# GestaltCogTeam/STEP

Hardware: AMD Instinct MI355X
Metric: training windows/sec on PEMS04, horizon-12 MAE parity, 1/2/4/8 MI355X (higher is better)
Workload: dtype f16 (TSFormer Q/K/weights) + bf16 (P, V, GraphWaveNet / graph-learner GEMMs) operands, f32 accumulate

## Files before the change

### include/step_hip.h

```cpp
#ifndef STEP_HIP_H
#define STEP_HIP_H

#include <stdint.h>

#ifdef __cplusplus
extern "C" {
#endif

const char* step_last_error(void);
int step_abi_version(void);

typedef struct StepGemm {
    int M, N, K, batch;
    const void* A; long sam, sak, sab; int a_bf16;
    const void* B; long sbk, sbn, sbb; int b_bf16;
    float* C; long ldc, scn, scb;
    float alpha;
    int accumulate;
    const float* bias; int relu;
    int splitk;
    int a_kblk; long a_kstride;
    int b_kblk; long b_kstride;
    int b_nblk; long b_nstride;
    int c_nblk; long c_nstride;
    const float* a_kscale; const float* a_kshift; int a_kperiod;
    int batch0; long sab1, sbb1, scb1;
    int compute_bf16;
    float* a_rowsum;
    const float *c_nscale, *c_nshift, *c_mvec;
    int c_nperiod;
    float* splitk_ws; long splitk_ws_floats;
} StepGemm;
int step_gemm(const StepGemm* g, void* stream);

#define STEP_ENC_F16 1
#define STEP_ENC_ALWAYS_RESHIFT 2
#define STEP_ENC_RANGE_FLAG 4
#define STEP_ENC_WORKGROUPS(n) (((n) & 0xffff) << 8)
int step_tsformer_encode(const float* series, int S, int L, const void* wpack, long wpack_bytes,
                         int depth, int flags, uint16_t* hidden_bf16, float* hidden_f32, float* last_f32,
                         float* sqnorm_part, float dropout_p, const uint64_t* drop_pool, long pool_words, uint64_t seed,
                         unsigned int* fallback_count, void* stream);
int step_dropout_pool_fill(uint64_t* pool, long words, float dropout_p, uint64_t seed, void* stream);
long step_tsformer_dropout_words(int L, int depth);

int step_pack_long_history(const float* x, int B, int L, int N, int C, int ch, float* out, void* stream);
int step_gather_windows(const float* data, int T, int N, int C, int ch, const long* t0, int B, int L, int H,
                        float* long_series, float* hist, float* fut, void* stream);

long step_knn_workspace_bytes(int B, int N, int F);
int step_knn_graph(const uint16_t* hidden, const float* sqnorm_part, int B, int N, int F, int k_total,
                   float* sim, float* adj, void* work, long work_bytes, void* stream);
int step_topk_mask(const float* sim, int B, int N, int k_total, float* adj, void* work, long work_bytes,
                   void* stream);

typedef struct StepDglParams {
    float *conv1_w, *conv1_b;
    float *conv2_w, *conv2_b;
    float *fc_w, *fc_b;
    float *bn1_w, *bn1_b, *bn1_rm, *bn1_rv;
    float *bn2_w, *bn2_b, *bn2_rm, *bn2_rv;
    float *bn3_w, *bn3_b, *bn3_rm, *bn3_rv;
    float *fc_out_w, *fc_out_b;
    float *fc_cat_w, *fc_cat_b;
    int gemm_bf16;
} StepDglParams;

long step_dgl_global_saved_floats(int N, int T);
long step_dgl_global_work_floats(int N, int T, int backward);
int step_dgl_global_forward(const float* series_nt, int N, int T, const StepDglParams* p, int training,
                            float momentum, float* saved, float* work, float* g, void* stream);
int step_dgl_global_backward(const float* series_nt, int N, int T, const StepDglParams* p, const float* saved,
                             const float* dg, float* work, const StepDglParams* grads, void* stream);
#define STEP_DGL_FRESH_FC_GRAD 16
int step_dgl_global_backward_phase(const float* series_nt, int N, int T, const StepDglParams* p, const float* saved,
                             const float* dg, float* work, const StepDglParams* grads, int phase, void* stream);

typedef struct StepDglShard { int own1; double count1, count2; } StepDglShard;
int step_dgl_global_forward_shard(const float* series_slice, int N, int Ts, const StepDglParams* p, int training, float momentum,
                                  float* saved, float* work, double* sums, float* g, const StepDglShard* shard, int phase,
                                  void* stream);
int step_dgl_global_backward_shard(const float* series_slice, int N, int Ts, const StepDglParams* p, const float* saved,
                                   const float* dg, float* work, const StepDglParams* grads, const StepDglShard* shard, int phase,
                                   void* stream);
// ... 162 lines not shown
```

### step_amd/_lib.py

```python
import ctypes
import os

import torch

_HERE = os.path.dirname(os.path.abspath(__file__))
LIB_PATH = os.environ.get("STEP_HIP_LIB") or os.path.join(_HERE, "libstep_hip.so")

_vp, _i, _l, _f, _u64 = ctypes.c_void_p, ctypes.c_int, ctypes.c_long, ctypes.c_float, ctypes.c_uint64


class StepGemm(ctypes.Structure):
    _fields_ = [("M", _i), ("N", _i), ("K", _i), ("batch", _i),
                ("A", _vp), ("sam", _l), ("sak", _l), ("sab", _l), ("a_bf16", _i),
                ("B", _vp), ("sbk", _l), ("sbn", _l), ("sbb", _l), ("b_bf16", _i),
                ("C", _vp), ("ldc", _l), ("scn", _l), ("scb", _l),
                ("alpha", _f), ("accumulate", _i), ("bias", _vp), ("relu", _i), ("splitk", _i),
                ("a_kblk", _i), ("a_kstride", _l), ("b_kblk", _i), ("b_kstride", _l),
                ("b_nblk", _i), ("b_nstride", _l), ("c_nblk", _i), ("c_nstride", _l),
                ("a_kscale", _vp), ("a_kshift", _vp), ("a_kperiod", _i),
                ("batch0", _i), ("sab1", _l), ("sbb1", _l), ("scb1", _l), ("compute_bf16", _i), ("a_rowsum", _vp), ("c_nscale", _vp), ("c_nshift", _vp), ("c_mvec", _vp),
                ("c_nperiod", _i), ("splitk_ws", _vp), ("splitk_ws_floats", _l)]


class StepDglParams(ctypes.Structure):
    NAMES = ["conv1_w", "conv1_b", "conv2_w", "conv2_b", "fc_w", "fc_b",
             "bn1_w", "bn1_b", "bn1_rm", "bn1_rv", "bn2_w", "bn2_b", "bn2_rm", "bn2_rv",
             "bn3_w", "bn3_b", "bn3_rm", "bn3_rv", "fc_out_w", "fc_out_b", "fc_cat_w", "fc_cat_b"]
    _fields_ = [(n, _vp) for n in NAMES] + [("gemm_bf16", _i)]


class StepGwnetParams(ctypes.Structure):
    _fields_ = [("nodevec1", _vp), ("nodevec2", _vp), ("start_w", _vp), ("start_b", _vp),
                ("filter_w", _vp * 8), ("filter_b", _vp * 8), ("gate_w", _vp * 8), ("gate_b", _vp * 8),
                ("skip_w", _vp * 8), ("skip_b", _vp * 8),
                ("bn_w", _vp * 8), ("bn_b", _vp * 8), ("bn_rm", _vp * 8), ("bn_rv", _vp * 8),
                ("gconv_w", _vp * 8), ("gconv_b", _vp * 8),
                ("fc_his0_w", _vp), ("fc_his0_b", _vp), ("fc_his2_w", _vp), ("fc_his2_b", _vp),
                ("end1_w", _vp), ("end1_b", _vp), ("end2_w", _vp), ("end2_b", _vp), ("gemm_bf16", _i)]


_PD = ctypes.POINTER(StepDglParams)


class StepDynState(ctypes.Structure):
    _fields_ = [("seed_xor", ctypes.c_uint64), ("adam_step", ctypes.c_int32), ("lr", _f), ("gsl_coef", _f), ("reserved", _f)]


class StepDglShard(ctypes.Structure):
    _fields_ = [("own1", ctypes.c_int), ("count1", ctypes.c_double), ("count2", ctypes.c_double)]


_PS = ctypes.POINTER(StepDglShard)
_PG = ctypes.POINTER(StepGwnetParams)

_SIGS = {
    "step_last_error": (ctypes.c_char_p, []),
    "step_abi_version": (_i, []),
    "step_gemm": (_i, [ctypes.POINTER(StepGemm), _vp]),
    "step_tsformer_encode": (_i, [_vp, _i, _i, _vp, _l, _i, _i, _vp, _vp, _vp, _vp, _f, _vp, _l, _u64, _vp, _vp]),
    "step_dropout_pool_fill": (_i, [_vp, _l, _f, _u64, _vp]),
    "step_tsformer_dropout_words": (_l, [_i, _i]),
    "step_gather_windows": (_i, [_vp, _i, _i, _i, _i, _vp, _i, _i, _i, _vp, _vp, _vp, _vp]),
    "step_pack_long_history": (_i, [_vp, _i, _i, _i, _i, _i, _vp, _vp]),
    "step_knn_workspace_bytes": (_l, [_i, _i, _i]),
    "step_knn_graph": (_i, [_vp, _vp, _i, _i, _i, _i, _vp, _vp, _vp, _l, _vp]),
    "step_topk_mask": (_i, [_vp, _i, _i, _i, _vp, _vp, _l, _vp]),
    "step_selftest_mfma": (_i, [_vp, _vp]),
    "step_streams_concurrent": (_i, [_vp, _vp, ctypes.POINTER(_i)]),
    "step_dgl_global_saved_floats": (_l, [_i, _i]),
    "step_dgl_global_work_floats": (_l, [_i, _i, _i]),
    "step_dgl_global_forward": (_i, [_vp, _i, _i, _PD, _i, _f, _vp, _vp, _vp, _vp]),
    "step_dgl_global_backward": (_i, [_vp, _i, _i, _PD, _vp, _vp, _vp, _PD, _vp]),
    "step_dgl_global_backward_phase": (_i, [_vp, _i, _i, _PD, _vp, _vp, _vp, _PD, _i, _vp]),
    "step_dgl_global_forward_shard": (_i, [_vp, _i, _i, _PD, _i, _f, _vp, _vp, _vp, _vp, _PS, _i, _vp]),
# ... 82 lines not shown

ABI_VERSION = 10
ENC_F16, ENC_ALWAYS_RESHIFT, ENC_RANGE_FLAG = 1, 2, 4
COMM_F32, COMM_F64, COMM_U8, COMM_ID_BYTES = 0, 1, 2, 128


def lib():
    global _lib
    if _lib is None:
        if not os.path.exists(LIB_PATH):
            raise RuntimeError(
                f"libstep_hip.so not found at {LIB_PATH}: build it with `python -m step_amd.build` "
                "(step_amd has no fallback path)")
        _lib = ctypes.CDLL(LIB_PATH)
        for name, (res, args) in _SIGS.items():
            fn = getattr(_lib, name)
            fn.restype = res
            fn.argtypes = args
        if _lib.step_abi_version() != ABI_VERSION:
            v = _lib.step_abi_version()
            _lib = None
            raise RuntimeError(f"libstep_hip.so has ABI version {v}, this package needs {ABI_VERSION}: rebuild with `python -m step_amd.build`")
    return _lib


def exported_symbols():
    return sorted(_SIGS)


def check(rc, what=""):
    if rc != 0:
        msg = lib().step_last_error().decode(errors="replace")
        raise RuntimeError(f"libstep_hip {what} failed (rc={rc}): {msg}")


def ptr(t):
    if t is None:
        return None
    assert t.is_cuda and t.is_contiguous(), "libstep_hip takes contiguous device tensors"
    return ctypes.c_void_p(t.data_ptr())


def stream():
    return ctypes.c_void_p(torch.cuda.current_stream().cuda_stream)


def call(name, *args):
    check(getattr(lib(), name)(*args), name)


def gemm(a, b, c, M, N, K, sam, sak, sbk, sbn, ldc, batch=1, sab=0, sbb=0, scb=0, scn=1, alpha=1.0,
         accumulate=0, bias=None, relu=False, splitk=1, a_off=0, b_off=0, c_off=0, a_k=(0, 0), b_k=(0, 0),
         b_n=(0, 0), c_n=(0, 0), a_kscale=None, a_kshift=None, a_kperiod=0, batch0=0, sab1=0, sbb1=0, scb1=0, compute_bf16=False, a_rowsum=None, c_nscale=None, c_nshift=None, c_mvec=None,
         c_nperiod=0, splitk_ws=None):
    g = StepGemm()
    g.M, g.N, g.K, g.batch = M, N, K, batch
    g.A = a.data_ptr() + a_off * a.element_size()
    g.sam, g.sak, g.sab, g.a_bf16 = sam, sak, sab, int(a.dtype == torch.bfloat16)
    g.B = b.data_ptr() + b_off * b.element_size()
    g.sbk, g.sbn, g.sbb, g.b_bf16 = sbk, sbn, sbb, int(b.dtype == torch.bfloat16)
    g.C = c.data_ptr() + c_off * 4
    g.ldc, g.scn, g.scb = ldc, scn, scb
    g.alpha, g.accumulate = alpha, accumulate
    g.bias = bias.data_ptr() if bias is not None else None
    g.relu, g.splitk = int(relu), splitk
    g.a_kblk, g.a_kstride = a_k
    g.b_kblk, g.b_kstride = b_k
    g.b_nblk, g.b_nstride = b_n
    g.c_nblk, g.c_nstride = c_n
    g.batch0, g.sab1, g.sbb1, g.scb1 = batch0, sab1, sbb1, scb1
    g.compute_bf16 = int(compute_bf16)
    g.a_rowsum = ptr(a_rowsum) if a_rowsum is not None else None
    g.c_nscale, g.c_nshift, g.c_mvec = (ptr(c_nscale) if c_nscale is not None else None, ptr(c_nshift) if c_nshift is not None else None,
                                         ptr(c_mvec) if c_mvec is not None else None)
    g.c_nperiod = c_nperiod
    if splitk_ws is not None:
        g.splitk_ws, g.splitk_ws_floats = ptr(splitk_ws), splitk_ws.numel()
    if a_kscale is not None:
        g.a_kscale, g.a_kshift, g.a_kperiod = a_kscale.data_ptr(), a_kshift.data_ptr(), a_kperiod
    check(lib().step_gemm(ctypes.byref(g), stream()), "step_gemm")
```

### step_amd/csrc/common.h

```cpp
#pragma once
#include "../../include/step_hip.h"
#include <hip/hip_runtime.h>
#include <stdint.h>
#include <stdio.h>
#include <string.h>

#define STEP_OK 0
#define STEP_ERR_ARG 1
#define STEP_ERR_HIP 2

void step_set_error(const char* fmt, ...);
int step_raise_lds_once(const void* kernel, int bytes, const char* what);

#define STEP_REQUIRE(cond, ...)                 \
    do {                                        \
        if (!(cond)) {                          \
            step_set_error(__VA_ARGS__);        \
            return STEP_ERR_ARG;                \
        }                                       \
    } while (0)

#define STEP_LAUNCH_CHECK(name)                                                   \
    do {                                                                          \
        hipError_t e_ = hipGetLastError();                                        \
// ... 26 lines not shown
    return f32_to_bf16_bits(lo) | (f32_to_bf16_bits(hi) << 16);
}
__device__ __forceinline__ float bf16_bits_to_f32(uint32_t b) { return __uint_as_float(b << 16); }

typedef __attribute__((ext_vector_type(8))) float f32x8;
__device__ __forceinline__ bf16x8 pack8(const float* v) {
    f32x8 t;
#pragma unroll
    for (int j = 0; j < 8; ++j) t[j] = v[j];
    return __builtin_convertvector(t, bf16x8);
}

__device__ __forceinline__ float wave_sum(float v) {
#pragma unroll
    for (int o = 32; o > 0; o >>= 1) v += __shfl_xor(v, o, 64);
    return v;
}
__device__ __forceinline__ float wave_max(float v) {
#pragma unroll
    for (int o = 32; o > 0; o >>= 1) v = fmaxf(v, __shfl_xor(v, o, 64));
    return v;
}

#ifndef STEP_PHILOX_MUL64
#define STEP_PHILOX_MUL64 1
#endif
__device__ __forceinline__ void philox4x32(uint32_t c0, uint32_t c1, uint32_t c2, uint32_t c3,
                                           uint32_t k0, uint32_t k1, uint32_t out[4]) {
#pragma unroll
    for (int r = 0; r < 10; ++r) {
#if STEP_PHILOX_MUL64
        const uint64_t p0 = (uint64_t)0xD2511F53u * c0, p1 = (uint64_t)0xCD9E8D57u * c2;
        const uint32_t hi0 = (uint32_t)(p0 >> 32), lo0 = (uint32_t)p0, hi1 = (uint32_t)(p1 >> 32), lo1 = (uint32_t)p1;
#else
        uint32_t hi0 = __umulhi(0xD2511F53u, c0), lo0 = 0xD2511F53u * c0;
        uint32_t hi1 = __umulhi(0xCD9E8D57u, c2), lo1 = 0xCD9E8D57u * c2;
#endif
        uint32_t n0 = hi1 ^ c1 ^ k0, n1 = lo1, n2 = hi0 ^ c3 ^ k1, n3 = lo0;
        c0 = n0; c1 = n1; c2 = n2; c3 = n3;
        k0 += 0x9E3779B9u; k1 += 0xBB67AE85u;
    }
    out[0] = c0; out[1] = c1; out[2] = c2; out[3] = c3;
}
__device__ __forceinline__ float u32_to_unit(uint32_t x) { return (float)(x >> 8) * (1.0f / 16777216.0f); }

struct GemmColAffine { float cs, csh; const float* mvec; };
__device__ __forceinline__ GemmColAffine gemm_col_affine(const StepGemm& g, int gn) {
    GemmColAffine a = {1.f, 0.f, nullptr};
    if (g.c_nscale) { const int c = gn / g.c_nperiod; a.cs = g.c_nscale[c]; a.csh = g.c_nshift[c]; a.mvec = g.c_mvec; }
    return a;
}

__device__ __forceinline__ void gemm_store_tile(const f32x16& acc, float* col, int mb, int M, long ldc, float alpha, int accumulate,
                                                float bv, int relu, GemmColAffine ca = GemmColAffine{1.f, 0.f, nullptr}) {
    float val[16];
#pragma unroll
    for (int e = 0; e < 16; ++e) {
        const int gm = mb + (e & 3) + 8 * (e >> 2);
        val[e] = alpha * acc[e] * ca.cs;
        if (ca.mvec) val[e] += ca.csh * (gm < M ? ca.mvec[gm] : 0.f);
    }
    if (accumulate == 2) {
#pragma unroll
        for (int e = 0; e < 16; ++e) {
            const int gm = mb + (e & 3) + 8 * (e >> 2);
            if (gm < M) atomicAdd(col + (long)gm * ldc, val[e]);
        }
    } else if (accumulate == 1) {
        float old[16];
#pragma unroll
        for (int e = 0; e < 16; ++e) {
            const int gm = mb + (e & 3) + 8 * (e >> 2);
            old[e] = gm < M ? col[(long)gm * ldc] : 0.f;
        }
#pragma unroll
        for (int e = 0; e < 16; ++e) {
            const int gm = mb + (e & 3) + 8 * (e >> 2);
            float v = val[e] + old[e] + bv;
            if (relu) v = fmaxf(v, 0.f);
            if (gm < M) col[(long)gm * ldc] = v;
        }
    } else {
#pragma unroll
        for (int e = 0; e < 16; ++e) {
            const int gm = mb + (e & 3) + 8 * (e >> 2);
            float v = val[e] + bv;
            if (relu) v = fmaxf(v, 0.f);
            if (gm < M) col[(long)gm * ldc] = v;
        }
    }
}
```

### step_amd/csrc/dgl.hip

```cpp
#include "common.h"
#include "step_internal.h"

namespace {

constexpr int KW = 10;
constexpr int EMB = 100;

template <int CI, int CO, int TPT>
__global__ __launch_bounds__(256) void conv_relu_fwd_kernel(const float* __restrict__ in, const float* __restrict__ w,
                                                            const float* __restrict__ b, const float* __restrict__ in_sc,
                                                            const float* __restrict__ in_sh, float* __restrict__ out,
                                                            float* __restrict__ partial, int Tin, int stat_limit) {
    __shared__ __attribute__((aligned(16))) float ws[CI * KW * CO];
    __shared__ float red[4][2 * CO];
    const int tid = threadIdx.x, n = blockIdx.y;
    const int Tout = Tin - (KW - 1);
    for (int e = tid; e < CI * KW * CO; e += 256) {
        int co = e % CO, k = (e / CO) % KW, ci = e / (CO * KW);
        ws[e] = w[(co * CI + ci) * KW + k];
    }
    __syncthreads();
    const int t0 = (blockIdx.x * 256 + tid) * TPT;
    float acc[CO][TPT];
#pragma unroll
    for (int co = 0; co < CO; ++co)
#pragma unroll
        for (int j = 0; j < TPT; ++j) acc[co][j] = b[co];
    if (t0 < Tout) {
#pragma unroll 1
        for (int ci = 0; ci < CI; ++ci) {
            const float* src = in + ((long)n * CI + ci) * Tin + t0;
            const float sc = in_sc ? in_sc[ci] : 1.f, sh = in_sh ? in_sh[ci] : 0.f;
            float x[TPT + KW - 1];
#pragma unroll
            for (int q = 0; q < TPT + KW - 1; ++q) x[q] = (t0 + q < Tin) ? src[q] * sc + sh : 0.f;
#pragma unroll
            for (int k = 0; k < KW; ++k) {
                const float* wk = ws + (ci * KW + k) * CO;
#pragma unroll
                for (int co = 0; co < CO; ++co) {
                    const float wv = wk[co];
#pragma unroll
                    for (int j = 0; j < TPT; ++j) acc[co][j] += wv * x[k + j];
                }
            }
        }
    }
    float s1[CO], s2[CO];
#pragma unroll
    for (int co = 0; co < CO; ++co) {
        s1[co] = 0.f; s2[co] = 0.f;
        float* dst = out + ((long)n * CO + co) * Tout + t0;
#pragma unroll
        for (int j = 0; j < TPT; ++j) {
            if (t0 + j < Tout) {
                float v = fmaxf(acc[co][j], 0.f);
                dst[j] = v;
                if (t0 + j < stat_limit) { s1[co] += v; s2[co] += v * v; }
            }
        }
    }
    const int lane = tid & 63, wave = tid >> 6;
#pragma unroll
    for (int co = 0; co < CO; ++co) {
        float a = wave_sum(s1[co]), q = wave_sum(s2[co]);
        if (lane == 0) { red[wave][co] = a; red[wave][CO + co] = q; }
    }
    __syncthreads();
    if (tid < 2 * CO)
        partial[((long)blockIdx.y * gridDim.x + blockIdx.x) * (2 * CO) + tid] = red[0][tid] + red[1][tid] + red[2][tid] + red[3][tid];
}

__global__ __launch_bounds__(256) void bn_finalize_kernel(const float* __restrict__ partial, int nblk, int C, double count,
                                                          const float* __restrict__ gamma, const float* __restrict__ beta,
                                                          float* __restrict__ rmean, float* __restrict__ rvar, int training,
                                                          float momentum, float* __restrict__ stat) {
    __shared__ double r1[256], r2[256];
    const int c = blockIdx.x, tid = threadIdx.x;
    double mean, var;
    if (training) {
        double a = 0.0, q = 0.0;
        for (int i = tid; i < nblk; i += 256) { a += partial[(long)i * 2 * C + c]; q += partial[(long)i * 2 * C + C + c]; }
        r1[tid] = a; r2[tid] = q;
        __syncthreads();
        for (int s = 128; s > 0; s >>= 1) {
            if (tid < s) { r1[tid] += r1[tid + s]; r2[tid] += r2[tid + s]; }
            __syncthreads();
        }
        mean = r1[0] / count;
        var = fmax(r2[0] / count - mean * mean, 0.0);
        if (tid == 0) {
            rmean[c] = (1.f - momentum) * rmean[c] + momentum * (float)mean;
            rvar[c] = (1.f - momentum) * rvar[c] + momentum * (float)(var * count / fmax(count - 1.0, 1.0));
        }
    } else {
        mean = rmean[c];
        var = rvar[c];
    }
    if (tid == 0) {
        float rstd = (float)(1.0 / sqrt(var + 1e-5));
        float sc = gamma[c] * rstd;
        stat[c] = sc;
        stat[C + c] = beta[c] - (float)mean * sc;
        stat[2 * C + c] = (float)mean;
        stat[3 * C + c] = rstd;
    }
}

__global__ __launch_bounds__(256) void bn_sums_kernel(const float* __restrict__ partial, int nblk, int C, double* __restrict__ sums) {
    __shared__ double r1[256], r2[256];
    const int c = blockIdx.x, tid = threadIdx.x;
    double a = 0.0, q = 0.0;
    for (int i = tid; i < nblk; i += 256) { a += partial[(long)i * 2 * C + c]; q += partial[(long)i * 2 * C + C + c]; }
    r1[tid] = a; r2[tid] = q;
    __syncthreads();
    for (int s = 128; s > 0; s >>= 1) {
        if (tid < s) { r1[tid] += r1[tid + s]; r2[tid] += r2[tid + s]; }
        __syncthreads();
    }
    if (tid == 0) { sums[c] = r1[0]; sums[C + c] = r2[0]; }
}
__global__ __launch_bounds__(256) void bn_sums_sliced_kernel(const float* __restrict__ partial, int nblk, int C, double* __restrict__ sums) {
    __shared__ double r1[256], r2[256];
    const int c = blockIdx.x, tid = threadIdx.x;
    const int per = (nblk + gridDim.y - 1) / gridDim.y, beg = blockIdx.y * per, end = min(nblk, beg + per);
    double a = 0.0, q = 0.0;
    for (int i = beg + tid; i < end; i += 256) { a += partial[(long)i * 2 * C + c]; q += partial[(long)i * 2 * C + C + c]; }
    r1[tid] = a; r2[tid] = q;
    __syncthreads();
    for (int s = 128; s > 0; s >>= 1) {
        if (tid < s) { r1[tid] += r1[tid + s]; r2[tid] += r2[tid + s]; }
        __syncthreads();
    }
    if (tid == 0) { unsafeAtomicAdd(sums + c, r1[0]); unsafeAtomicAdd(sums + C + c, r2[0]); }
}
__global__ void bn_finalize_sums_kernel(const double* __restrict__ sums, int C, double count, const float* __restrict__ gamma,
                                        const float* __restrict__ beta, float* __restrict__ rmean, float* __restrict__ rvar,
                                        int training, float momentum, float* __restrict__ stat) {
    const int c = threadIdx.x;
    if (c >= C) return;
    double mean, var;
    if (training) {
        mean = sums[c] / count;
        var = fmax(sums[C + c] / count - mean * mean, 0.0);
        rmean[c] = (1.f - momentum) * rmean[c] + momentum * (float)mean;
        rvar[c] = (1.f - momentum) * rvar[c] + momentum * (float)(var * count / fmax(count - 1.0, 1.0));
    } else {
        mean = rmean[c]; var = rvar[c];
    }
    const float rstd = (float)(1.0 / sqrt(var + 1e-5));
    const float sc = gamma[c] * rstd;
    stat[c] = sc; stat[C + c] = beta[c] - (float)mean * sc; stat[2 * C + c] = (float)mean; stat[3 * C + c] = rstd;
}

__global__ __launch_bounds__(256) void fc_post_bn3_kernel(float* __restrict__ gpre, const float* __restrict__ bias, int N,
                                                          const float* __restrict__ gamma, const float* __restrict__ beta,
                                                          float* __restrict__ rmean, float* __restrict__ rvar, int training,
                                                          float momentum, float* __restrict__ stat, float* __restrict__ g) {
    __shared__ double r1[256], r2[256];
    const int j = blockIdx.x, tid = threadIdx.x;
    const float bj = bias[j];
    double a = 0.0, q = 0.0;
    for (int n = tid; n < N; n += 256) {
        float v = gpre[(long)n * EMB + j] + bj;
        gpre[(long)n * EMB + j] = v;
        v = fmaxf(v, 0.f);
        a += v; q += (double)v * v;
    }
    r1[tid] = a; r2[tid] = q;
    __syncthreads();
    for (int s = 128; s > 0; s >>= 1) {
        if (tid < s) { r1[tid] += r1[tid + s]; r2[tid] += r2[tid + s]; }
        __syncthreads();
    }
    double mean, var;
    if (training) {
        mean = r1[0] / N;
        var = fmax(r2[0] / N - mean * mean, 0.0);
        if (tid == 0) {
            rmean[j] = (1.f - momentum) * rmean[j] + momentum * (float)mean;
            rvar[j] = (1.f - momentum) * rvar[j] + momentum * (float)(var * N / fmax((double)N - 1.0, 1.0));
        }
    } else {
        mean = rmean[j]; var = rvar[j];
    }
    const float rstd = (float)(1.0 / sqrt(var + 1e-5));
    if (tid == 0) { stat[2 * EMB + j] = (float)mean; stat[3 * EMB + j] = rstd; }
    const float sc = gamma[j] * rstd, sh = beta[j] - (float)mean * sc;
    for (int n = tid; n < N; n += 256) g[(long)n * EMB + j] = fmaxf(gpre[(long)n * EMB + j], 0.f) * sc + sh;
}

__global__ __launch_bounds__(256) void bn3_relu_bwd_kernel(const float* __restrict__ dg, const float* __restrict__ gpre, int N,
                                                           const float* __restrict__ gamma, const float* __restrict__ stat,
                                                           float* __restrict__ dgamma, float* __restrict__ dbeta,
                                                           float* __restrict__ dbias, float* __restrict__ dgpre,
                                                           float* __restrict__ dgpreT, float* __restrict__ colsum) {
    __shared__ double r1[256], r2[256];
    const int j = blockIdx.x, tid = threadIdx.x;
    const float mean = stat[2 * EMB + j], rstd = stat[3 * EMB + j];
    double a = 0.0, q = 0.0;
    for (int n = tid; n < N; n += 256) {
        float d = dg[(long)n * EMB + j];
        float xh = (fmaxf(gpre[(long)n * EMB + j], 0.f) - mean) * rstd;
        a += d; q += (double)d * xh;
    }
    r1[tid] = a; r2[tid] = q;
    __syncthreads();
    for (int s = 128; s > 0; s >>= 1) {
        if (tid < s) { r1[tid] += r1[tid + s]; r2[tid] += r2[tid + s]; }
        __syncthreads();
    }
    const float m1 = (float)(r1[0] / N), m2 = (float)(r2[0] / N);
    const float k = gamma[j] * rstd;
    __syncthreads();
    double sb = 0.0;
    for (int n = tid; n < N; n += 256) {
        float pre = gpre[(long)n * EMB + j];
        float xh = (fmaxf(pre, 0.f) - mean) * rstd;
        float dh = k * (dg[(long)n * EMB + j] - m1 - xh * m2);
        float v = pre > 0.f ? dh : 0.f;
        dgpre[(long)n * EMB + j] = v;
        dgpreT[(long)j * N + n] = v;
        sb += v;
    }
    if (tid == 0) { dgamma[j] += (float)r2[0]; dbeta[j] += (float)r1[0]; }
    __syncthreads();
    r1[tid] = sb;
    __syncthreads();
    for (int s = 128; s > 0; s >>= 1) {
        if (tid < s) r1[tid] += r1[tid + s];
        __syncthreads();
    }
    if (tid == 0) { dbias[j] += (float)r1[0]; colsum[j] = (float)r1[0]; }
}

template <int C>
__global__ __launch_bounds__(256) void bn_bwd_reduce_kernel(const float* __restrict__ dy, const float* __restrict__ x,
                                                            const float* __restrict__ stat, int Tlen, float* __restrict__ partial) {
    __shared__ float red[4][2];
    const int n = blockIdx.z, c = blockIdx.y, tid = threadIdx.x;
    const float mean = stat[2 * C + c], rstd = stat[3 * C + c];
    const long base = ((long)n * C + c) * Tlen;
    float a = 0.f, q = 0.f;
    for (int t = blockIdx.x * 1024 + tid; t < min(Tlen, (int)(blockIdx.x + 1) * 1024); t += 256) {
        float d = dy[base + t];
        a += d; q += d * ((x[base + t] - mean) * rstd);
    }
    a = wave_sum(a); q = wave_sum(q);
    if ((tid & 63) == 0) { red[tid >> 6][0] = a; red[tid >> 6][1] = q; }
    __syncthreads();
    if (tid < 2) {
// ... 377 lines not shown
#pragma unroll
        for (int c = 0; c < 16; ++c) { acc += v[c] * st2[16 + c]; v[c] *= st2[c]; }
        uint4* dst = wp + ((long)o * T2 + t) * 2;
        dst[0] = make_uint4(pack_bf16x2(v[0], v[1]), pack_bf16x2(v[2], v[3]), pack_bf16x2(v[4], v[5]), pack_bf16x2(v[6], v[7]));
        dst[1] = make_uint4(pack_bf16x2(v[8], v[9]), pack_bf16x2(v[10], v[11]), pack_bf16x2(v[12], v[13]), pack_bf16x2(v[14], v[15]));
    }
    acc = wave_sum(acc);
    if ((tid & 63) == 0) red[tid >> 6] = acc;
    __syncthreads();
    if (tid == 0) atomicAdd(&shiftdot[o], red[0] + red[1] + red[2] + red[3]);
}
__global__ void gpre_init_kernel(float* __restrict__ gpre, const float* __restrict__ shiftdot, long n) {
    const long i = (long)blockIdx.x * 256 + threadIdx.x;
    if (i < n) gpre[i] = shiftdot[i % EMB];
}
__global__ __launch_bounds__(256) void fc_unpermute_kernel(const float* __restrict__ graw, const float* __restrict__ fc_w,
                                                           const float* __restrict__ st2, const float* __restrict__ colsum,
                                                           float* __restrict__ dfc_w, float* __restrict__ dots_o, int T2, int overwrite) {
    __shared__ float red[4][32];
    const int o = blockIdx.y, t = blockIdx.x * 256 + threadIdx.x, tid = threadIdx.x;
    const float cso = colsum[o];
    float d[32];
#pragma unroll
    for (int i = 0; i < 32; ++i) d[i] = 0.f;
    if (t < T2) {
        const float4* src = (const float4*)(graw + ((long)o * T2 + t) * 16);
        const float4 g0 = src[0], g1 = src[1], g2 = src[2], g3 = src[3];
        const float g[16] = {g0.x, g0.y, g0.z, g0.w, g1.x, g1.y, g1.z, g1.w, g2.x, g2.y, g2.z, g2.w, g3.x, g3.y, g3.z, g3.w};
        float w[16], old[16];
#pragma unroll
        for (int c = 0; c < 16; ++c) { const long idx = ((long)o * 16 + c) * T2 + t; w[c] = fc_w[idx]; old[c] = overwrite ? 0.f : dfc_w[idx]; }
#pragma unroll
        for (int c = 0; c < 16; ++c) {
            dfc_w[((long)o * 16 + c) * T2 + t] = old[c] + st2[c] * g[c] + st2[16 + c] * cso;
            d[2 * c] = w[c] * g[c]; d[2 * c + 1] = w[c] * cso;
        }
    }
#pragma unroll
    for (int i = 0; i < 32; ++i) {
        const float v = wave_sum(d[i]);
        if ((tid & 63) == 0) red[tid >> 6][i] = v;
    }
    __syncthreads();
    if (tid < 32) atomicAdd(&dots_o[o * 32 + tid], red[0][tid] + red[1][tid] + red[2][tid] + red[3][tid]);
}
__global__ void dots_reduce_kernel(const float* __restrict__ dots_o, float* __restrict__ dots) {
    const int i = threadIdx.x;
    if (i >= 32) return;
    double a = 0.0;
    for (int o = 0; o < EMB; ++o) a += dots_o[o * 32 + i];
    dots[i] = (float)a;
}

static bool dgl_channels_last(const StepDglParams* p) {
    const char* e = getenv("STEP_DGL_F32_STORAGE");
    return p->gemm_bf16 && !(e && e[0] == '1');
}

static bool dgl_legacy_bn_backward() {
    const char* e = getenv("STEP_DGL_LEGACY_BN");
    return e && e[0] == '1';
}

extern "C" long step_dgl_global_saved_floats(int N, int T) {
    long T1 = T - 9, T2 = T - 18;
    return (long)N * 8 * T1 + (long)N * 16 * T2 + (long)N * EMB + 4 * 8 + 4 * 16 + 4 * EMB + (long)EMB * 16 * T2 + 128;
}
static long fc_splitk_ws_floats(int N, int T2) {
    const int splits = step_gemm_auto_splitk(N, EMB, 16 * T2, 1);
    return splits > 1 ? (long)splits * N * EMB + 4 : 0;
}
extern "C" long step_dgl_global_work_floats(int N, int T, int backward) {
    long T1 = T - 9, T2 = T - 18;
    long nb1 = (long)N * cdiv(T1, 1024), nb2 = (long)N * cdiv(T2, 1024);
    long part = (nb1 > nb2 ? nb1 : nb2) * 32 + 64;
    if (!backward) return part + dgl_conv2_pack_floats() + 64 + fc_splitk_ws_floats(N, (int)T2);
    return part + (long)N * 16 * T2 + (long)N * 8 * T1 + (long)EMB * 16 * T2 + 2L * N * EMB + DGL_SMALL + dgl_conv2_wgrad_scratch_floats(N, (int)T1);
}

static float* saved_wp(float* saved, int N, int T) {
    long T1 = T - 9, T2 = T - 18;
    return saved + (long)N * 8 * T1 + (long)N * 16 * T2 + (long)N * EMB + 4 * 8 + 4 * 16 + 4 * EMB;
}
static void carve_saved(float* saved, int N, int T, float** a1, float** a2, float** gpre, float** st1, float** st2, float** st3) {
    long T1 = T - 9, T2 = T - 18;
    *a1 = saved; saved += (long)N * 8 * T1;
    *a2 = saved; saved += (long)N * 16 * T2;
    *gpre = saved; saved += (long)N * EMB;
    *st1 = saved; saved += 4 * 8;
    *st2 = saved; saved += 4 * 16;
    *st3 = saved;
}

static int dgl_bn_stats(const float* partial, int nblk, int C, double count, const float* gamma, const float* beta, float* rm, float* rv,
                        int training, float momentum, float* stat, double* sums, hipStream_t st) {
    if (nblk < 8192) {
        bn_finalize_kernel<<<C, 256, 0, st>>>(partial, nblk, C, count, gamma, beta, rm, rv, training, momentum, stat);
    } else {
        if (hipMemsetAsync(sums, 0, 2 * C * sizeof(double), st) != hipSuccess) { step_set_error("memset failed"); return STEP_ERR_HIP; }
        bn_sums_sliced_kernel<<<dim3(C, 32), 256, 0, st>>>(partial, nblk, C, sums);
        bn_finalize_sums_kernel<<<1, 64, 0, st>>>(sums, C, count, gamma, beta, rm, rv, training, momentum, stat);
    }
    STEP_LAUNCH_CHECK("bn_stats");
    return STEP_OK;
}

static int dgl_global_forward_impl(const float* series_nt, int N, int T, const StepDglParams* p, int training, float momentum,
                                   float* saved, float* work, double* sums, float* g, const StepDglShard* shard, int phase,
                                   hipStream_t st) {
    const int T1 = T - 9, T2 = T - 18;
    float *a1, *a2, *gpre, *st1, *st2, *st3;
    carve_saved(saved, N, T, &a1, &a2, &gpre, &st1, &st2, &st3);
    float* partial = work;
    const bool all = phase == 0;
    const double count1 = shard ? shard->count1 : (double)N * T1, count2 = shard ? shard->count2 : (double)N * T2;
    const bool cl = dgl_channels_last(p);
    const long part_floats = ((long)N * cdiv(T1, 1024) > (long)N * cdiv(T2, 1024) ? (long)N * cdiv(T1, 1024) : (long)N * cdiv(T2, 1024)) * 32 + 64;
    double* own_sums = (double*)(work + part_floats + dgl_conv2_pack_floats());
    float* wp = saved_wp(saved, N, T);
    float* shiftdot = wp + (long)EMB * 16 * T2;
    if (all || phase == 1) {
        int nblk;
        if (cl) {
            STEP_TRY(dgl_conv1_fwd_cl(series_nt, p->conv1_w, p->conv1_b, a1, partial, N, T, shard ? shard->own1 : T1, &nblk, st));
        } else {
            dim3 grid(cdiv(T1, 256 * 4), N);
            conv_relu_fwd_kernel<1, 8, 4><<<grid, 256, 0, st>>>(series_nt, p->conv1_w, p->conv1_b, nullptr, nullptr, a1, partial, T,
                                                                shard ? shard->own1 : T1);
            STEP_LAUNCH_CHECK("conv1");
            nblk = grid.x * grid.y;
        }
        if (shard) bn_sums_kernel<<<8, 256, 0, st>>>(partial, nblk, 8, sums);
        else STEP_TRY(dgl_bn_stats(partial, nblk, 8, count1, p->bn1_w, p->bn1_b, p->bn1_rm, p->bn1_rv, training, momentum, st1, own_sums, st));
        STEP_LAUNCH_CHECK("bn1");
    }
    if (all || phase == 2) {
        if (shard) bn_finalize_sums_kernel<<<1, 64, 0, st>>>(sums, 8, count1, p->bn1_w, p->bn1_b, p->bn1_rm, p->bn1_rv, training, momentum, st1);
        int nblk;
        if (cl) {
            STEP_TRY(dgl_conv2_fwd_cl(a1, p->conv2_w, p->conv2_b, st1, st1 + 8, a2, partial, N, T1, &nblk,
                                      work + part_floats, st));
        } else if (p->gemm_bf16) {
            STEP_TRY(dgl_conv2_fwd_mfma(a1, p->conv2_w, p->conv2_b, st1, st1 + 8, a2, partial, N, T1, &nblk, st));
        } else {
            dim3 grid(cdiv(T2, 256 * 4), N);
            conv_relu_fwd_kernel<8, 16, 4><<<grid, 256, 0, st>>>(a1, p->conv2_w, p->conv2_b, st1, st1 + 8, a2, partial, T1, T2);
            STEP_LAUNCH_CHECK("conv2");
            nblk = grid.x * grid.y;
        }
        if (shard) bn_sums_kernel<<<16, 256, 0, st>>>(partial, nblk, 16, sums + 16);
        else STEP_TRY(dgl_bn_stats(partial, nblk, 16, count2, p->bn2_w, p->bn2_b, p->bn2_rm, p->bn2_rv, training, momentum, st2, own_sums, st));
        STEP_LAUNCH_CHECK("bn2");
    }
    if (all || phase == 3) {
        if (shard) bn_finalize_sums_kernel<<<1, 64, 0, st>>>(sums + 16, 16, count2, p->bn2_w, p->bn2_b, p->bn2_rm, p->bn2_rv, training, momentum, st2);
        const long K = 16L * T2;
        StepGemm gm = gemm_desc(N, EMB, (int)K, a2, K, 1, p->fc_w, 1, K, gpre, EMB);
        if (cl) {
            if (hipMemsetAsync(shiftdot, 0, 128 * sizeof(float), st) != hipSuccess) { step_set_error("memset failed"); return STEP_ERR_HIP; }
            fc_prep_kernel<<<dim3(cdiv(T2, 256), EMB), 256, 0, st>>>(p->fc_w, st2, (uint4*)wp, shiftdot, T2);
            gpre_init_kernel<<<cdiv((long)N * EMB, 256), 256, 0, st>>>(gpre, shiftdot, (long)N * EMB);
            STEP_LAUNCH_CHECK("fc_prep");
            gm.a_bf16 = 1;
            gm.B = wp; gm.b_bf16 = 1;
        } else {
            if (hipMemsetAsync(gpre, 0, (size_t)N * EMB * sizeof(float), st) != hipSuccess) { step_set_error("memset failed"); return STEP_ERR_HIP; }
            gm.a_kscale = st2; gm.a_kshift = st2 + 16; gm.a_kperiod = T2;
        }
        gm.accumulate = 2;
        gm.splitk = -1;
        gm.compute_bf16 = p->gemm_bf16;
        if (fc_splitk_ws_floats(N, T2) > 0) {
            float* ws = work + part_floats + dgl_conv2_pack_floats() + 64;
            gm.splitk_ws = (float*)(((uintptr_t)ws + 15) & ~(uintptr_t)15);
            gm.splitk_ws_floats = fc_splitk_ws_floats(N, T2) - 4;
        }
        STEP_TRY(step_gemm_launch(gm, st));
    }
    if (all || phase == 4) {
        fc_post_bn3_kernel<<<EMB, 256, 0, st>>>(gpre, p->fc_b, N, p->bn3_w, p->bn3_b, p->bn3_rm, p->bn3_rv, training, momentum, st3, g);
        STEP_LAUNCH_CHECK("fc_post_bn3");
    }
    return STEP_OK;
}

extern "C" int step_dgl_global_forward(const float* series_nt, int N, int T, const StepDglParams* p, int training,
                                       float momentum, float* saved, float* work, float* g, void* stream) {
    STEP_REQUIRE(series_nt && p && saved && work && g && N > 0 && T > 18, "dgl_global_forward: bad arguments");
    return dgl_global_forward_impl(series_nt, N, T, p, training, momentum, saved, work, nullptr, g, nullptr, 0, (hipStream_t)stream);
}

extern "C" int step_dgl_global_forward_shard(const float* series_slice, int N, int Ts, const StepDglParams* p, int training,
                                             float momentum, float* saved, float* work, double* sums, float* g,
                                             const StepDglShard* shard, int phase, void* stream) {
    STEP_REQUIRE(series_slice && p && saved && work && sums && g && shard && N > 0 && Ts > 18 && phase >= 1 && phase <= 4,
                 "dgl_global_forward_shard: bad arguments");
    STEP_REQUIRE(shard->own1 > 0 && shard->own1 <= Ts - 9 && shard->count1 > 0 && shard->count2 > 0, "dgl_global_forward_shard: bad shard");
    return dgl_global_forward_impl(series_slice, N, Ts, p, training, momentum, saved, work, sums, g, shard, phase, (hipStream_t)stream);
}

extern "C" long step_dgl_global_offset(int N, int T, int item) {
    const long T1 = T - 9, T2 = T - 18;
    if (item == 0) return 0;
    if (item == 1) return (long)N * 8 * T1;
    if (item == 2) return (long)N * 8 * T1 + (long)N * 16 * T2;
    const long nb1 = (long)N * cdiv(T1, 1024), nb2 = (long)N * cdiv(T2, 1024);
    const long coef = (nb1 > nb2 ? nb1 : nb2) * 32 + 64 + (long)N * 16 * T2 + (long)N * 8 * T1 + (long)EMB * 16 * T2 + 2L * N * EMB;
    if (item == 10) return coef + 256;
    if (item == 11) return coef + 320;
    return -1;
}

static int dgl_global_backward_impl(const float* series_nt, int N, int T, const StepDglParams* p, const float* saved, const float* dg,
                                    float* work, const StepDglParams* grads, const StepDglShard* shard, int phase, void* stream);

extern "C" int step_dgl_global_backward(const float* series_nt, int N, int T, const StepDglParams* p, const float* saved,
                                        const float* dg, float* work, const StepDglParams* grads, void* stream) {
    return step_dgl_global_backward_phase(series_nt, N, T, p, saved, dg, work, grads, 0, stream);
}

extern "C" int step_dgl_global_backward_phase(const float* series_nt, int N, int T, const StepDglParams* p, const float* saved,
                                              const float* dg, float* work, const StepDglParams* grads, int phase, void* stream) {
    STEP_REQUIRE(series_nt && p && saved && dg && work && grads && N > 0 && T > 18 && (phase & ~STEP_DGL_FRESH_FC_GRAD) >= 0 &&
                 (phase & ~STEP_DGL_FRESH_FC_GRAD) <= 2, "dgl_global_backward: bad arguments");
    return dgl_global_backward_impl(series_nt, N, T, p, saved, dg, work, grads, nullptr, phase, stream);
}

extern "C" int step_dgl_global_backward_shard(const float* series_slice, int N, int Ts, const StepDglParams* p, const float* saved,
                                              const float* dg, float* work, const StepDglParams* grads, const StepDglShard* shard,
                                              int phase, void* stream) {
    const int ph = phase & ~STEP_DGL_FRESH_FC_GRAD;
    STEP_REQUIRE(series_slice && p && saved && dg && work && grads && shard && N > 0 && Ts > 18 && (ph == 1 || ph == 3 || ph == 4),
                 "dgl_global_backward_shard: bad arguments");
    STEP_REQUIRE(p->gemm_bf16 && Ts - 18 >= 128, "dgl_global_backward_shard: needs the bf16 contraction mode and a slice of >= 128 conv2 columns");
    return dgl_global_backward_impl(series_slice, N, Ts, p, saved, dg, work, grads, shard, phase, stream);
}

static int dgl_global_backward_impl(const float* series_nt, int N, int T, const StepDglParams* p, const float* saved, const float* dg,
                                    float* work, const StepDglParams* grads, const StepDglShard* shard, int phase, void* stream) {
    const int fresh_fc = (phase & STEP_DGL_FRESH_FC_GRAD) ? 1 : 0;
    phase &= ~STEP_DGL_FRESH_FC_GRAD;
    const bool do_fc = phase == 0 || phase == 1, do_mid = phase == 0 || phase == 2 || phase == 3, do_tail = phase == 0 || phase == 2 || phase == 4;
    hipStream_t st = (hipStream_t)stream;
    const int T1 = T - 9, T2 = T - 18;
    const long K = 16L * T2;
    float *a1, *a2, *gpre, *st1, *st2, *st3;
    carve_saved((float*)saved, N, T, &a1, &a2, &gpre, &st1, &st2, &st3);
    long nb1 = (long)N * cdiv(T1, 1024), nb2 = (long)N * cdiv(T2, 1024);
    float* partial = work;
    float* d_a2 = work + (nb1 > nb2 ? nb1 : nb2) * 32 + 64;
    float* d_a1 = d_a2 + (long)N * 16 * T2;
    float* wraw = d_a1 + (long)N * 8 * T1;
    float* dgpre = wraw + (long)EMB * K;
    float* dgpreT = dgpre + (long)N * EMB;
    float* coef = dgpreT + (long)N * EMB;
    float* dots = coef + 256;
    float* graw = coef + 320;
    float* wg_scratch = coef + DGL_SMALL;
    const bool fuse2 = T2 >= 128 && (shard || !dgl_legacy_bn_backward());
    const double count1 = shard ? shard->count1 : (double)N * T1, count2 = shard ? shard->count2 : (double)N * T2;
    if (dgl_channels_last(p)) {
        const float* wp = saved_wp((float*)saved, N, T);
        float* dots_o = coef + 256 + 64 + 1344;
        float* colsum = coef + 128;
        if (do_fc) {
            bn3_relu_bwd_kernel<<<EMB, 256, 0, st>>>(dg, gpre, N, p->bn3_w, st3, grads->bn3_w, grads->bn3_b, grads->fc_b, dgpre, dgpreT, colsum);
            STEP_LAUNCH_CHECK("bn3_bwd");
            StepGemm gm = gemm_desc(EMB, (int)K, N, dgpre, 1, EMB, a2, K, 1, wraw, K);
            gm.b_bf16 = 1;
            gm.compute_bf16 = 1;
            STEP_TRY(step_gemm_launch(gm, st));
            if (hipMemsetAsync(dots_o, 0, EMB * 32 * sizeof(float), st) != hipSuccess) { step_set_error("memset failed"); return STEP_ERR_HIP; }
            fc_unpermute_kernel<<<dim3(cdiv(T2, 256), EMB), 256, 0, st>>>(wraw, p->fc_w, st2, colsum, grads->fc_w, dots_o, T2, fresh_fc);
            dots_reduce_kernel<<<1, 64, 0, st>>>(dots_o, dots);
            STEP_LAUNCH_CHECK("fc_unpermute");
        }
        if (do_mid) {
            bn2_fused_coef_kernel<<<1, 64, 0, st>>>(dots, st2, p->bn2_w, count2, grads->bn2_w, grads->bn2_b, coef);
            STEP_LAUNCH_CHECK("bn2_fused_coef");
            StepGemm gm = gemm_desc(N, (int)K, EMB, dgpre, EMB, 1, wp, K, 1, d_a2, K);
            gm.b_bf16 = 1;
            gm.compute_bf16 = 1;
            GemmFused fu = {nullptr, nullptr, a2, coef, st2, 16, T2, GEMM_FUSED_INTERLEAVED};
            STEP_TRY(step_gemm_launch_fused(gm, fu, st));
            STEP_TRY(dgl_conv2_wgrad_cl(d_a2, a1, wg_scratch, graw, N, T1, st));
        }
        if (do_tail) {
            STEP_TRY(dgl_conv2_wgrad_finish(graw, p->conv2_w, st1, p->bn1_w, p->bn1_b, count1, grads->conv2_w, grads->conv2_b, grads->bn1_w,
                                            grads->bn1_b, coef + 64, 1, st));
            STEP_TRY(dgl_conv2_dgrad_cl(d_a2, p->conv2_w, st1, d_a1, N, T1, a1, coef + 64, st1, shard ? shard->own1 : T1, wraw, st));
            STEP_TRY(dgl_conv1_wgrad_cl(d_a1, series_nt, wg_scratch, grads->conv1_w, grads->conv1_b, N, T, st));
        }
        return STEP_OK;
    }
    if (do_fc) {
        float* colsum = coef + 128;
        bn3_relu_bwd_kernel<<<EMB, 256, 0, st>>>(dg, gpre, N, p->bn3_w, st3, grads->bn3_w, grads->bn3_b, grads->fc_b, dgpre, dgpreT, colsum);
        STEP_LAUNCH_CHECK("bn3_bwd");
        {
            StepGemm gm = gemm_desc(EMB, (int)K, N, dgpre, 1, EMB, a2, K, 1, grads->fc_w, K);
            gm.accumulate = fresh_fc ? 0 : 1;
            gm.c_nscale = st2; gm.c_nshift = st2 + 16; gm.c_nperiod = T2; gm.c_mvec = colsum;
            gm.compute_bf16 = p->gemm_bf16;
            if (fuse2) {
                if (hipMemsetAsync(dots, 0, 32 * sizeof(float), st) != hipSuccess) { step_set_error("memset failed"); return STEP_ERR_HIP; }
                GemmFused fu = {p->fc_w, dots, nullptr, nullptr, nullptr, 16, T2};
                STEP_TRY(step_gemm_launch_fused(gm, fu, st));
            } else {
                STEP_TRY(step_gemm_launch(gm, st));
            }
        }
    }
    if (!do_mid && !do_tail) return STEP_OK;
    if (do_mid) {
        StepGemm gm = gemm_desc(N, (int)K, EMB, dgpreT, 1, N, p->fc_w, K, 1, d_a2, K);
        if (p->gemm_bf16 || fuse2) { gm.A = dgpre; gm.sam = EMB; gm.sak = 1; }
        gm.compute_bf16 = p->gemm_bf16;
        if (fuse2) {
            bn2_fused_coef_kernel<<<1, 64, 0, st>>>(dots, st2, p->bn2_w, count2, grads->bn2_w, grads->bn2_b, coef);
            STEP_LAUNCH_CHECK("bn2_fused_coef");
            GemmFused fu = {nullptr, nullptr, a2, coef, st2, 16, T2};
            STEP_TRY(step_gemm_launch_fused(gm, fu, st));
        } else {
            STEP_TRY(step_gemm_launch(gm, st));
        }
    }
    if (do_mid && !fuse2) {
        dim3 grid(cdiv(T2, 1024), 16, N);
        bn_bwd_reduce_kernel<16><<<grid, 256, 0, st>>>(d_a2, a2, st2, T2, partial);
        STEP_LAUNCH_CHECK("bn2_bwd_reduce");
        bn_bwd_finalize_kernel<<<16, 256, 0, st>>>(partial, (int)nb2, 16, (double)N * T2, p->bn2_w, st2, grads->bn2_w, grads->bn2_b, coef);
        STEP_LAUNCH_CHECK("bn2_bwd_finalize");
        bn_bwd_apply_kernel<16><<<grid, 256, 0, st>>>(d_a2, a2, st2, coef, T2);
        STEP_LAUNCH_CHECK("bn2_bwd_apply");
    }
    const bool fuse1 = p->gemm_bf16 && (shard || !dgl_legacy_bn_backward());
    if (fuse1) {
        if (do_mid) STEP_TRY(dgl_conv2_wgrad_xhat_mfma(d_a2, a1, st1, wg_scratch, graw, N, T1, st));
        if (!do_tail) return STEP_OK;
        STEP_TRY(dgl_conv2_wgrad_finish(graw, p->conv2_w, st1, p->bn1_w, p->bn1_b, count1, grads->conv2_w, grads->conv2_b, grads->bn1_w,
                                        grads->bn1_b, coef + 64, 0, st));
        STEP_TRY(dgl_conv2_dgrad_mfma(d_a2, p->conv2_w, d_a1, N, T1, a1, coef + 64, st1, shard ? shard->own1 : T1, st));
    } else if (p->gemm_bf16) {
        STEP_TRY(dgl_conv2_wgrad_mfma(d_a2, a1, st1, st1 + 8, wg_scratch, grads->conv2_w, grads->conv2_b, N, T1, st));
        STEP_TRY(dgl_conv2_dgrad_mfma(d_a2, p->conv2_w, d_a1, N, T1, nullptr, nullptr, nullptr, T1, st));
    } else {
        conv_bwd_weight_kernel<8, 16><<<N, 256, 0, st>>>(d_a2, a1, st1, st1 + 8, grads->conv2_w, grads->conv2_b, T1);
        STEP_LAUNCH_CHECK("conv2_bwd_weight");
        conv_bwd_data_kernel<8, 16, 4><<<dim3(cdiv(T1, 1024), N), 256, 0, st>>>(d_a2, p->conv2_w, d_a1, T1);
        STEP_LAUNCH_CHECK("conv2_bwd_data");
// ... 103 lines not shown
```

### step_amd/csrc/dgl_conv_mfma.hip

```cpp
#include "common.h"
#include "step_internal.h"

namespace {

constexpr int KW = 10, CI = 8, CO = 16, C1_ = 8;
constexpr int FW_TT = 1024;

__device__ __forceinline__ uint32_t cvt2(float a, float b) {
    uint32_t r;
    asm("v_cvt_pk_bf16_f32 %0, %1, %2" : "=v"(r) : "v"(a), "v"(b));
    return r;
}
__device__ __forceinline__ bf16x8 as_frag(uint4 v) { return __builtin_bit_cast(bf16x8, v); }

__global__ __launch_bounds__(256) void conv2_fwd_mfma_kernel(const float* __restrict__ a1, const float* __restrict__ w,
                                                             const float* __restrict__ b, const float* __restrict__ sc,
                                                             const float* __restrict__ sh, float* __restrict__ a2,
                                                             float* __restrict__ partial, int T1) {
    __shared__ uint4 xs[FW_TT + 16];
    __shared__ float red[4][2 * CO];
    const int tid = threadIdx.x, lane = tid & 63, wave = tid >> 6, n = blockIdx.y;
    const int T2 = T1 - (KW - 1), t0 = blockIdx.x * FW_TT;
    const int ln = lane & 15, q = lane >> 4;

// ... 376 lines not shown
    {
        const int tb = blockIdx.x * 1024;
        const float* xr = x + (long)n * T + tb;
        for (int i = tid; i < 1024 + 16; i += 256) xs[i] = tb + i < T ? xr[i] : 0.f;
    }
    __syncthreads();
    const int t0 = (blockIdx.x * 256 + tid) * 4;
    float s1[C1_], s2[C1_];
#pragma unroll
    for (int c = 0; c < C1_; ++c) { s1[c] = 0.f; s2[c] = 0.f; }
    if (t0 < T1) {
        float xv[16];
#pragma unroll
        for (int q4 = 0; q4 < 4; ++q4) {
            const float4 v4 = *(const float4*)(xs + 4 * tid + 4 * q4);
            xv[4 * q4] = v4.x; xv[4 * q4 + 1] = v4.y; xv[4 * q4 + 2] = v4.z; xv[4 * q4 + 3] = v4.w;
        }
        float acc[4][C1_];
#pragma unroll
        for (int j = 0; j < 4; ++j)
#pragma unroll
            for (int c = 0; c < C1_; ++c) acc[j][c] = b[c];
#pragma unroll
        for (int k = 0; k < KW; ++k)
#pragma unroll
            for (int c = 0; c < C1_; ++c) {
                const float wv = ws[k][c];
#pragma unroll
                for (int j = 0; j < 4; ++j) acc[j][c] += wv * xv[k + j];
            }
#pragma unroll
        for (int j = 0; j < 4; ++j) {
            if (t0 + j >= T1) break;
            float v[C1_];
#pragma unroll
            for (int c = 0; c < C1_; ++c) {
                v[c] = fmaxf(acc[j][c], 0.f);
                if (t0 + j < stat_limit) { s1[c] += v[c]; s2[c] += v[c] * v[c]; }
            }
            a1h[(long)n * T1 + t0 + j] = make_uint4(cvt2(v[0], v[1]), cvt2(v[2], v[3]), cvt2(v[4], v[5]), cvt2(v[6], v[7]));
        }
    }
    const int lane = tid & 63, wave = tid >> 6;
#pragma unroll
    for (int c = 0; c < C1_; ++c) {
        const float a = wave_sum(s1[c]), q = wave_sum(s2[c]);
        if (lane == 0) { red[wave][c] = a; red[wave][C1_ + c] = q; }
    }
    __syncthreads();
    if (tid < 2 * C1_)
        partial[((long)blockIdx.y * gridDim.x + blockIdx.x) * (2 * C1_) + tid] = red[0][tid] + red[1][tid] + red[2][tid] + red[3][tid];
}

__global__ void conv2_pack_kernel(const float* __restrict__ w, const float* __restrict__ b, const float* __restrict__ sc,
                                  const float* __restrict__ sh, uint4* __restrict__ pack) {
    const int lane = threadIdx.x & 63, s = threadIdx.x >> 6, ln = lane & 15, q = lane >> 4;
    float v[8];
    if (s < 3) {
        const int kk = 4 * s + q;
#pragma unroll
        for (int ci = 0; ci < CI; ++ci) v[ci] = kk < KW ? w[(ln * CI + ci) * KW + kk] * sc[ci] : 0.f;
    } else {
        const int kk = 2 * (s - 3) + (q >> 1), c0 = 8 * (q & 1);
#pragma unroll
        for (int j = 0; j < 8; ++j) v[j] = ln < CI ? w[((c0 + j) * CI + ln) * KW + kk] * sc[ln] : 0.f;
    }
    pack[s * 64 + lane] = make_uint4(cvt2(v[0], v[1]), cvt2(v[2], v[3]), cvt2(v[4], v[5]), cvt2(v[6], v[7]));
    if (threadIdx.x < CO) {
        float a = b[threadIdx.x];
        for (int ci = 0; ci < CI; ++ci) {
            float ws = 0.f;
            for (int kk = 0; kk < KW; ++kk) ws += w[(threadIdx.x * CI + ci) * KW + kk];
            a += ws * sh[ci];
        }
        ((float*)(pack + 8 * 64))[threadIdx.x] = a;
    }
}

__global__ __launch_bounds__(256) void conv2_fwd_cl_kernel(const uint4* __restrict__ a1h, const uint4* __restrict__ pack,
                                                           uint2* __restrict__ a2h, float* __restrict__ partial, int T1) {
    __shared__ uint4 xs[FW_TT + 16];
    __shared__ float red[4][2 * CO];
    const int tid = threadIdx.x, lane = tid & 63, wave = tid >> 6, n = blockIdx.y;
    const int T2 = T1 - (KW - 1), t0 = blockIdx.x * FW_TT;
    const int ln = lane & 15, q = lane >> 4;
    for (int tt = tid; tt < FW_TT + 16; tt += 256) {
        const int t = t0 + tt;
        xs[tt] = t < T1 ? a1h[(long)n * T1 + t] : make_uint4(0u, 0u, 0u, 0u);
    }
    bf16x8 wf[3];
#pragma unroll
    for (int s = 0; s < 3; ++s) wf[s] = as_frag(pack[s * 64 + lane]);
    float bias[4];
#pragma unroll
    for (int e = 0; e < 4; ++e) bias[e] = ((const float*)(pack + 8 * 64))[4 * q + e];
    __syncthreads();
    float s1[4] = {0.f, 0.f, 0.f, 0.f}, s2[4] = {0.f, 0.f, 0.f, 0.f};
    for (int tile = wave; tile < FW_TT / 16; tile += 4) {
        const int tb = tile * 16;
        if (t0 + tb >= T2) break;
        f32x4 acc = {0.f, 0.f, 0.f, 0.f};
#pragma unroll
        for (int s = 0; s < 3; ++s) acc = __builtin_amdgcn_mfma_f32_16x16x32_bf16(wf[s], as_frag(xs[tb + ln + 4 * s + q]), acc, 0, 0, 0);
        const int t = t0 + tb + ln;
        if (t < T2) {
            float v[4];
#pragma unroll
            for (int e = 0; e < 4; ++e) { v[e] = fmaxf(acc[e] + bias[e], 0.f); s1[e] += v[e]; s2[e] += v[e] * v[e]; }
            a2h[((long)n * T2 + t) * 4 + q] = make_uint2(cvt2(v[0], v[1]), cvt2(v[2], v[3]));
        }
    }
#pragma unroll
    for (int e = 0; e < 4; ++e) {
#pragma unroll
        for (int o = 1; o < 16; o <<= 1) { s1[e] += __shfl_xor(s1[e], o, 64); s2[e] += __shfl_xor(s2[e], o, 64); }
        if (ln == 0) { red[wave][4 * q + e] = s1[e]; red[wave][CO + 4 * q + e] = s2[e]; }
    }
    __syncthreads();
    if (tid < 2 * CO)
        partial[((long)blockIdx.y * gridDim.x + blockIdx.x) * (2 * CO) + tid] = red[0][tid] + red[1][tid] + red[2][tid] + red[3][tid];
}

__global__ __launch_bounds__(256) void conv2_dgrad_cl_kernel(const uint4* __restrict__ dz2h, const uint4* __restrict__ pack,
                                                             uint2* __restrict__ dz1h, int T1,
                                                             const uint2* __restrict__ a1h, const float* __restrict__ coef,
                                                             const float* __restrict__ stat, int own) {
    __shared__ uint4 zs[FW_TT + 16][2];
    const int tid = threadIdx.x, lane = tid & 63, wave = tid >> 6, n = blockIdx.y;
    const int T2 = T1 - (KW - 1), t0 = blockIdx.x * FW_TT;
// ... 249 lines not shown
    return (long)N * cdiv(T2, WG_SC * WG_PASSES) * WG_OUT;
}

int dgl_conv2_wgrad_mfma(const float* dz, const float* a1, const float* sc, const float* sh, float* scratch, float* dw, float* db, int N,
                         int T1, hipStream_t st) {
    const int T2 = T1 - (KW - 1);
    dim3 grid(cdiv(T2, WG_SC * WG_PASSES), N);
    conv2_wgrad_mfma_kernel<<<grid, 256, 0, st>>>(dz, a1, sc, sh, scratch, T1, 0);
    STEP_LAUNCH_CHECK("conv2_wgrad_mfma");
    conv_wgrad_reduce_kernel<<<dim3(cdiv(WG_OUT, 64), wgrad_slices(grid.x * grid.y)), 256, 0, st>>>(scratch, grid.x * grid.y, WG_OUT, CO * CI * KW, dw, db);
    STEP_LAUNCH_CHECK("conv2_wgrad_reduce");
    return STEP_OK;
}

int dgl_conv2_wgrad_xhat_mfma(const float* dz, const float* a1, const float* stat1, float* scratch, float* graw, int N, int T1,
                              hipStream_t st) {
    const int T2 = T1 - (KW - 1);
    dim3 grid(cdiv(T2, WG_SC * WG_PASSES), N);
    if (hipMemsetAsync(graw, 0, WG_OUT * sizeof(float), st) != hipSuccess) { step_set_error("memset failed"); return STEP_ERR_HIP; }
    conv2_wgrad_mfma_kernel<<<grid, 256, 0, st>>>(dz, a1, stat1, nullptr, scratch, T1, 1);
    STEP_LAUNCH_CHECK("conv2_wgrad_mfma(xhat)");
    conv_wgrad_reduce_kernel<<<dim3(cdiv(WG_OUT, 64), wgrad_slices(grid.x * grid.y)), 256, 0, st>>>(scratch, grid.x * grid.y, WG_OUT, CO * CI * KW, graw, graw + CO * CI * KW);
    STEP_LAUNCH_CHECK("conv2_wgrad_reduce");
    return STEP_OK;
}
int dgl_conv2_wgrad_finish(const float* graw, const float* w, const float* stat1, const float* gamma1, const float* beta1, double count,
                           float* dw, float* db, float* dgamma1, float* dbeta1, float* coef1, int raw, hipStream_t st) {
    conv2_wgrad_finish_kernel<<<1, 256, 0, st>>>(graw, w, stat1, gamma1, beta1, count, dw, db, dgamma1, dbeta1, coef1, raw);
    STEP_LAUNCH_CHECK("conv2_wgrad_finish");
    return STEP_OK;
}

int dgl_conv1_wgrad_mfma(const float* dz, const float* x, float* scratch, float* dw, float* db, int N, int T, hipStream_t st) {
    const int T1 = T - (KW - 1);
    dim3 grid(cdiv(T1, WG_SC * WG_PASSES), N);
    conv1_wgrad_mfma_kernel<<<grid, 256, 0, st>>>(dz, x, scratch, T);
    STEP_LAUNCH_CHECK("conv1_wgrad_mfma");
    conv_wgrad_reduce_kernel<<<dim3(cdiv(W1_OUT, 64), wgrad_slices(grid.x * grid.y)), 256, 0, st>>>(scratch, grid.x * grid.y, W1_OUT, C1 * KW, dw, db);
    STEP_LAUNCH_CHECK("conv1_wgrad_reduce");
    return STEP_OK;
}

int dgl_conv1_fwd_cl(const float* x, const float* w, const float* b, void* a1h, float* partial, int N, int T, int stat_limit, int* nblk,
                     hipStream_t st) {
    const int T1 = T - (KW - 1);
    dim3 grid(cdiv(T1, 1024), N);
    conv1_fwd_cl_kernel<<<grid, 256, 0, st>>>(x, w, b, (uint4*)a1h, partial, T, stat_limit);
    STEP_LAUNCH_CHECK("conv1_fwd_cl");
    *nblk = grid.x * grid.y;
    return STEP_OK;
}
long dgl_conv2_pack_floats() { return 8 * 64 * 4 + 16; }
int dgl_conv2_fwd_cl(const void* a1h, const float* w, const float* b, const float* sc, const float* sh, void* a2h, float* partial, int N,
                     int T1, int* nblk, float* pack, hipStream_t st) {
    const int T2 = T1 - (KW - 1);
    dim3 grid(cdiv(T2, FW_TT), N);
    conv2_pack_kernel<<<1, 512, 0, st>>>(w, b, sc, sh, (uint4*)pack);
    conv2_fwd_cl_kernel<<<grid, 256, 0, st>>>((const uint4*)a1h, (const uint4*)pack, (uint2*)a2h, partial, T1);
    STEP_LAUNCH_CHECK("conv2_fwd_cl");
    *nblk = grid.x * grid.y;
    return STEP_OK;
}
int dgl_conv2_dgrad_cl(const void* dz2h, const float* w, const float* sc, void* dz1h, int N, int T1, const void* a1h, const float* coef,
                       const float* stat, int own, float* pack, hipStream_t st) {
    conv2_pack_kernel<<<1, 512, 0, st>>>(w, w, sc, sc, (uint4*)pack);
    conv2_dgrad_cl_kernel<<<dim3(cdiv(T1, FW_TT), N), 256, 0, st>>>((const uint4*)dz2h, (const uint4*)pack, (uint2*)dz1h, T1, (const uint2*)a1h, coef, stat, own);
    STEP_LAUNCH_CHECK("conv2_dgrad_cl");
    return STEP_OK;
}
int dgl_conv2_wgrad_cl(const void* dz2h, const void* a1h, float* scratch, float* graw, int N, int T1, hipStream_t st) {
    const int T2 = T1 - (KW - 1);
    dim3 grid(cdiv(T2, WG_SC * WG_PASSES), N);
    if (hipMemsetAsync(graw, 0, WG_OUT * sizeof(float), st) != hipSuccess) { step_set_error("memset failed"); return STEP_ERR_HIP; }
    conv2_wgrad_cl_kernel<<<grid, 256, 0, st>>>((const uint4*)dz2h, (const uint4*)a1h, scratch, T1);
    STEP_LAUNCH_CHECK("conv2_wgrad_cl");
    conv_wgrad_reduce_kernel<<<dim3(cdiv(WG_OUT, 64), wgrad_slices(grid.x * grid.y)), 256, 0, st>>>(scratch, grid.x * grid.y, WG_OUT, CO * CI * KW, graw, graw + CO * CI * KW);
    STEP_LAUNCH_CHECK("conv2_wgrad_reduce");
    return STEP_OK;
}
int dgl_conv1_wgrad_cl(const void* dz1h, const float* x, float* scratch, float* dw, float* db, int N, int T, hipStream_t st) {
    const int T1 = T - (KW - 1);
    dim3 grid(cdiv(T1, WG_SC * WG_PASSES), N);
    conv1_wgrad_cl_kernel<<<grid, 256, 0, st>>>((const uint4*)dz1h, x, scratch, T);
    STEP_LAUNCH_CHECK("conv1_wgrad_cl");
    conv_wgrad_reduce_kernel<<<dim3(cdiv(W1_OUT, 64), wgrad_slices(grid.x * grid.y)), 256, 0, st>>>(scratch, grid.x * grid.y, W1_OUT, C1 * KW, dw, db);
    STEP_LAUNCH_CHECK("conv1_wgrad_reduce");
    return STEP_OK;
}
```

### step_amd/csrc/gemm.hip

```cpp
#include "common.h"
#include "step_internal.h"

namespace {

constexpr int BK = 32;

template <typename T>
__device__ __forceinline__ float ld_elem(const void* p, long idx) {
    if constexpr (sizeof(T) == 2) {
        return bf16_bits_to_f32(((const uint16_t*)p)[idx]);
    } else {
        return ((const float*)p)[idx];
    }
}

template <int BM, int BN, int WM, int WN, typename TA, typename TB>
__global__ __launch_bounds__(256) void gemm_f32mfma_kernel(StepGemm g) {
    constexpr int TM = BM / WM / 32;
    constexpr int TN = BN / WN / 32;
    constexpr int LDA = BM + 4;
    constexpr int LDB = BN + 4;
    __shared__ __attribute__((aligned(16))) float As[BK * LDA];
    __shared__ __attribute__((aligned(16))) float Bs[BK * LDB];

// ... 133 lines not shown
            const int e4 = tid + r * 256;
            if (b_kc) {
                const int kk = (e4 % (BK / 4)) * 4, nn = e4 / (BK / 4);
#pragma unroll
                for (int i = 0; i < 4; ++i) Bs[(kk + i) * LDB + nn] = rb[r][i];
            } else {
                const int nn = (e4 % (BN / 4)) * 4, kk = e4 / (BN / 4);
                *(float4*)&Bs[kk * LDB + nn] = make_float4(rb[r][0], rb[r][1], rb[r][2], rb[r][3]);
            }
        }
    };

    f32x16 acc[TM][TN];
#pragma unroll
    for (int i = 0; i < TM; ++i)
#pragma unroll
        for (int j = 0; j < TN; ++j)
#pragma unroll
            for (int e = 0; e < 16; ++e) acc[i][j][e] = 0.f;

    const int li = lane & 31, lk = lane >> 5;
    if (kbeg < kend) {
        load_tiles(kbeg);
        for (int k0 = kbeg; k0 < kend; k0 += BK) {
            __syncthreads();
            store_tiles();
            __syncthreads();
            if (k0 + BK < kend) load_tiles(k0 + BK);
#pragma unroll
            for (int kk = 0; kk < BK; kk += 2) {
                float a[TM], b[TN];
#pragma unroll
                for (int i = 0; i < TM; ++i) a[i] = As[(kk + lk) * LDA + wr * (TM * 32) + i * 32 + li];
#pragma unroll
                for (int j = 0; j < TN; ++j) b[j] = Bs[(kk + lk) * LDB + wc * (TN * 32) + j * 32 + li];
#pragma unroll
                for (int i = 0; i < TM; ++i)
#pragma unroll
                    for (int j = 0; j < TN; ++j)
                        acc[i][j] = __builtin_amdgcn_mfma_f32_32x32x2f32(a[i], b[j], acc[i][j], 0, 0, 0);
            }
        }
    }

    float* Cb = g.C + (long)i0 * g.scb + (long)i1 * g.scb1;
#pragma unroll
    for (int i = 0; i < TM; ++i)
#pragma unroll
        for (int j = 0; j < TN; ++j) {
            int gn = n0 + wc * (TN * 32) + j * 32 + li;
            if (gn >= g.N) continue;
            const float bv = (g.bias != nullptr) ? g.bias[gn] : 0.f;
            const long ni = g.c_nblk ? (long)(gn / g.c_nblk) * g.c_nstride + (gn % g.c_nblk) : (long)gn;
            gemm_store_tile(acc[i][j], Cb + ni * g.scn, m0 + wr * (TM * 32) + i * 32 + 4 * lk, g.M, g.ldc, g.alpha, g.accumulate, bv, g.relu, gemm_col_affine(g, gn));
        }
}

struct DirectArgs {
    int tiles_m, tiles_n;
    int a_sh, a_mask, b_sh, b_mask, bn_sh, bn_mask, cn_sh, cn_mask;
    int a_vec, b_vec;
};

template <typename TA, typename TB>
__global__ __launch_bounds__(256) void gemm_direct_kernel(StepGemm g, DirectArgs d) {
    const int lane = threadIdx.x & 63;
    const int wave = __builtin_amdgcn_readfirstlane(threadIdx.x >> 6);
    const long tile = (long)blockIdx.x * 4 + wave;
    const long per_batch = (long)d.tiles_m * d.tiles_n;
    if (tile >= per_batch * g.batch) return;
    const int zb = (int)(tile / per_batch);
    const int tr = (int)(tile % per_batch);
    const int m0 = (tr / d.tiles_n) * 32, n0 = (tr % d.tiles_n) * 32;
    const int li = lane & 31, lk = lane >> 5;
    const int i0 = g.batch0 ? zb % g.batch0 : zb, i1 = g.batch0 ? zb / g.batch0 : 0;
    const TA* Ab = (const TA*)g.A + (long)i0 * g.sab + (long)i1 * g.sab1;
    const TB* Bb = (const TB*)g.B + (long)i0 * g.sbb + (long)i1 * g.sbb1;
    const int gm = m0 + li, gn = n0 + li;
    const bool m_ok = gm < g.M, n_ok = gn < g.N;
    const int K = g.K;
    const int sak = (int)g.sak, sbk = (int)g.sbk;
    const int a_row = m_ok ? (int)((long)gm * g.sam) : 0;
    const int b_col = n_ok ? (int)((((long)(gn >> d.bn_sh)) * g.b_nstride + (gn & d.bn_mask)) * g.sbn) : 0;
    const int a_lane = a_row + 4 * lk * sak;
    const int b_lane = b_col + 4 * lk * sbk;

    auto ldA = [&](const TA* p, int off) -> float {
        if constexpr (sizeof(TA) == 2) return bf16_bits_to_f32(((const uint16_t*)p)[off]); else return p[off];
    };
    auto ldB = [&](const TB* p, int off) -> float {
        if constexpr (sizeof(TB) == 2) return bf16_bits_to_f32(((const uint16_t*)p)[off]); else return p[off];
    };
    auto load_a = [&](int k0, float (&v)[4]) {
        const TA* pu = Ab + (long)(((k0 >> d.a_sh) * (int)g.a_kstride + (k0 & d.a_mask)) * sak);
        if (sizeof(TA) == 4 && d.a_vec) {
            float4 t = *(const float4*)((const float*)pu + a_lane);
            v[0] = t.x; v[1] = t.y; v[2] = t.z; v[3] = t.w;
        } else {
#pragma unroll
            for (int j = 0; j < 4; ++j) v[j] = ldA(pu, a_lane + j * sak);
        }
    };
    auto load_b = [&](int k0, float (&v)[4]) {
        const TB* pu = Bb + (long)(((k0 >> d.b_sh) * (int)g.b_kstride + (k0 & d.b_mask)) * sbk);
        if (sizeof(TB) == 4 && d.b_vec) {
            float4 t = *(const float4*)((const float*)pu + b_lane);
            v[0] = t.x; v[1] = t.y; v[2] = t.z; v[3] = t.w;
// ... 19 lines not shown
            const int gkc = gk < K ? gk : 0;
            const long ki = (long)(gkc >> d.b_sh) * g.b_kstride + (gkc & d.b_mask);
            float x = ldB(Bb, b_col + (int)(ki * sbk));
            v[j] = gk < K ? x : 0.f;
        }
    };

    constexpr int G = 3, CH = 8 * G;
    f32x16 acc, acc2;
#pragma unroll
    for (int e = 0; e < 16; ++e) { acc[e] = 0.f; acc2[e] = 0.f; }
    const int kfull = K / CH * CH;
    if (kfull > 0) {
        float a[G][4], b[G][4], an[G][4], bn[G][4];
#pragma unroll
        for (int q = 0; q < G; ++q) { load_a(8 * q, a[q]); load_b(8 * q, b[q]); }
        for (int k0 = 0; k0 < kfull; k0 += CH) {
            const int kn = k0 + CH;
            if (kn < kfull) {
#pragma unroll
                for (int q = 0; q < G; ++q) { load_a(kn + 8 * q, an[q]); load_b(kn + 8 * q, bn[q]); }
            }
#pragma unroll
            for (int q = 0; q < G; ++q)
#pragma unroll
                for (int j = 0; j < 4; j += 2) {
                    acc = __builtin_amdgcn_mfma_f32_32x32x2f32(m_ok ? a[q][j] : 0.f, n_ok ? b[q][j] : 0.f, acc, 0, 0, 0);
                    acc2 = __builtin_amdgcn_mfma_f32_32x32x2f32(m_ok ? a[q][j + 1] : 0.f, n_ok ? b[q][j + 1] : 0.f, acc2, 0, 0, 0);
                }
            if (kn < kfull) {
#pragma unroll
                for (int q = 0; q < G; ++q)
#pragma unroll
                    for (int j = 0; j < 4; ++j) { a[q][j] = an[q][j]; b[q][j] = bn[q][j]; }
            }
        }
    }
    for (int k0 = kfull; k0 < K; k0 += 8) {
        float a[4], b[4];
        load_a_tail(k0, a); load_b_tail(k0, b);
#pragma unroll
        for (int j = 0; j < 4; j += 2) {
            acc = __builtin_amdgcn_mfma_f32_32x32x2f32(m_ok ? a[j] : 0.f, n_ok ? b[j] : 0.f, acc, 0, 0, 0);
            acc2 = __builtin_amdgcn_mfma_f32_32x32x2f32(m_ok ? a[j + 1] : 0.f, n_ok ? b[j + 1] : 0.f, acc2, 0, 0, 0);
        }
    }
#pragma unroll
    for (int e = 0; e < 16; ++e) acc[e] += acc2[e];

    float* Cb = g.C + (long)i0 * g.scb + (long)i1 * g.scb1;
    if (!n_ok) return;
    const float bv = (g.bias != nullptr) ? g.bias[gn] : 0.f;
    const long ni = (long)(gn >> d.cn_sh) * g.c_nstride + (gn & d.cn_mask);
    gemm_store_tile(acc, Cb + ni * g.scn, m0 + 4 * lk, g.M, g.ldc, g.alpha, g.accumulate, bv, g.relu, gemm_col_affine(g, gn));
}

static bool pow2(int x) { return x > 0 && (x & (x - 1)) == 0; }
static int ilog2(int x) { int s = 0; while ((1 << s) < x) ++s; return s; }

bool direct_eligible(const StepGemm& g) {
    if (g.K > 1024 || g.a_kscale) return false;
    if (g.sak == 1 || g.sbk == 1) return false;
    if ((g.a_kblk && (!pow2(g.a_kblk) || g.a_kblk < 8)) || (g.b_kblk && (!pow2(g.b_kblk) || g.b_kblk < 8))) return false;
    if ((g.b_nblk && !pow2(g.b_nblk)) || (g.c_nblk && !pow2(g.c_nblk))) return false;
    const long lim = 1L << 30;
    if ((long)g.M * (g.sam < 0 ? -g.sam : g.sam) + (long)g.K * g.sak >= lim) return false;
    if ((long)g.N * (g.sbn < 0 ? -g.sbn : g.sbn) * (g.b_nblk ? g.b_nstride / g.b_nblk + 1 : 1) + (long)g.K * g.sbk >= lim) return false;
    return true;
}

int launch_direct(const StepGemm& g, hipStream_t st) {
    DirectArgs d;
    d.tiles_m = cdiv(g.M, 32); d.tiles_n = cdiv(g.N, 32);
    auto sm = [](int blk, int& sh, int& mask) { if (blk) { sh = ilog2(blk); mask = blk - 1; } else { sh = 31; mask = 0x7fffffff; } };
    sm(g.a_kblk, d.a_sh, d.a_mask); sm(g.b_kblk, d.b_sh, d.b_mask); sm(g.b_nblk, d.bn_sh, d.bn_mask); sm(g.c_nblk, d.cn_sh, d.cn_mask);
    d.a_vec = !g.a_bf16 && g.sak == 1 && (g.sam % 4 == 0) && (g.sab % 4 == 0) && (((uintptr_t)g.A & 15) == 0) &&
              (g.a_kblk == 0 || g.a_kstride % 4 == 0) && (g.sab1 % 4 == 0);
    d.b_vec = !g.b_bf16 && g.sbk == 1 && (g.sbn % 4 == 0) && (g.sbb % 4 == 0) && (((uintptr_t)g.B & 15) == 0) &&
              (g.b_kblk == 0 || g.b_kstride % 4 == 0) && (g.b_nblk == 0 || g.b_nstride % 4 == 0) && (g.sbb1 % 4 == 0);
    const long waves = (long)d.tiles_m * d.tiles_n * g.batch;
    dim3 grid((unsigned)((waves + 3) / 4));
    if (g.a_bf16 && g.b_bf16) gemm_direct_kernel<uint16_t, uint16_t><<<grid, 256, 0, st>>>(g, d);
    else if (g.a_bf16) gemm_direct_kernel<uint16_t, float><<<grid, 256, 0, st>>>(g, d);
    else if (g.b_bf16) gemm_direct_kernel<float, uint16_t><<<grid, 256, 0, st>>>(g, d);
    else gemm_direct_kernel<float, float><<<grid, 256, 0, st>>>(g, d);
    STEP_LAUNCH_CHECK("step_gemm(direct)");
    return STEP_OK;
}

template <int BM, int BN, int WM, int WN>
int launch(const StepGemm& g, hipStream_t st) {
    dim3 grid(cdiv(g.N, BN), cdiv(g.M, BM), g.batch * g.splitk);
    if (g.a_bf16 && g.b_bf16)
        gemm_f32mfma_kernel<BM, BN, WM, WN, uint16_t, uint16_t><<<grid, 256, 0, st>>>(g);
    else if (g.a_bf16)
        gemm_f32mfma_kernel<BM, BN, WM, WN, uint16_t, float><<<grid, 256, 0, st>>>(g);
    else if (g.b_bf16)
        gemm_f32mfma_kernel<BM, BN, WM, WN, float, uint16_t><<<grid, 256, 0, st>>>(g);
    else
        gemm_f32mfma_kernel<BM, BN, WM, WN, float, float><<<grid, 256, 0, st>>>(g);
    STEP_LAUNCH_CHECK("step_gemm");
    return STEP_OK;
}

}

int step_gemm_rowsum_separate(StepGemm* g, hipStream_t st) {
    if (!g->a_rowsum) return STEP_OK;
    STEP_REQUIRE(g->sam == 1 && g->a_kblk == 0, "step_gemm: a_rowsum on the general kernels needs an m-contiguous A without k remap");
    STEP_TRY(step_colsum_launch((const float*)g->A, g->K, g->M, g->sak, g->a_rowsum, st));
    g->a_rowsum = nullptr;
    return STEP_OK;
}

int step_gemm_launch(StepGemm g, hipStream_t st) {
    STEP_REQUIRE(g.M > 0 && g.N > 0 && g.K >= 0 && g.batch > 0, "step_gemm: bad sizes M=%d N=%d K=%d batch=%d", g.M, g.N, g.K, g.batch);
    STEP_REQUIRE(g.A && g.B && g.C, "step_gemm: null operand");
    if (g.scn == 0) g.scn = 1;
    if (g.a_rowsum)
        STEP_REQUIRE(g.batch == 1 && g.alpha == 1.f && !g.a_bf16 && !g.a_kscale, "step_gemm: a_rowsum needs batch 1, alpha 1, f32 A without affine");
    if (g.c_nscale)
        STEP_REQUIRE(g.c_nshift && g.c_mvec && g.c_nperiod > 0, "step_gemm: c_nscale needs c_nshift, c_mvec and a positive c_nperiod");
    if (g.compute_bf16) return step_gemm_bf16_launch(g, st);
    {
        const int rc = step_gemm_f32_fast_launch(g, st);
        if (rc != -1) return rc;
    }
    STEP_TRY(step_gemm_rowsum_separate(&g, st));
    if (g.splitk < 0 && direct_eligible(g)) g.splitk = 1;
    if (g.splitk < 0) {
        STEP_REQUIRE(g.accumulate == 2, "step_gemm: automatic split-K needs accumulate==2");
        const int bm = (g.N <= 32 && g.M > 64) ? 128 : (g.M <= 32 && g.N > 64) ? 32 : (g.M <= 64 || g.N <= 64) ? 64 : 128;
        const int bn = (g.N <= 32 && g.M > 64) ? 32 : (g.M <= 32 && g.N > 64) ? 128 : (g.M <= 64 || g.N <= 64) ? 64 : 128;
        long tiles = (long)cdiv(g.M, bm) * cdiv(g.N, bn) * g.batch;
        long want = (768 + tiles - 1) / tiles;
        long maxs = cdiv(g.K, BK) / 2;
        g.splitk = (int)(want < 1 ? 1 : (want > maxs ? (maxs < 1 ? 1 : maxs) : want));
    }
    if (g.splitk < 1) g.splitk = 1;
    if (g.splitk == 1 && direct_eligible(g)) return launch_direct(g, st);
    if (g.splitk > 1) {
        STEP_REQUIRE(g.accumulate == 2, "step_gemm: split-K needs accumulate==2 (atomic) and a pre-zeroed/accumulating C");
    }
    STEP_REQUIRE(!(g.accumulate == 2 && (g.bias || g.relu)), "step_gemm: bias/relu epilogue not available with atomic accumulate");
    if (g.N <= 32 && g.M > 64) return launch<128, 32, 4, 1>(g, st);
    if (g.M <= 32 && g.N > 64) return launch<32, 128, 1, 4>(g, st);
    if (g.M <= 64 || g.N <= 64) return launch<64, 64, 2, 2>(g, st);
    long tiles128 = (long)cdiv(g.M, 128) * cdiv(g.N, 128) * g.batch * g.splitk;
    if (tiles128 < 256) return launch<64, 64, 2, 2>(g, st);
    return launch<128, 128, 2, 2>(g, st);
}

int step_gemm_launch_fused(StepGemm g, const GemmFused& fused, hipStream_t st) {
    STEP_REQUIRE(g.M > 0 && g.N > 0 && g.K >= 0 && g.batch == 1 && g.A && g.B && g.C, "step_gemm(fused): bad descriptor");
    STEP_REQUIRE(fused.channels > 0 && fused.period > 0 && (long)fused.channels * fused.period == g.N, "step_gemm(fused): N != channels * period");
    if (g.scn == 0) g.scn = 1;
    if (g.splitk < 1) g.splitk = 1;
    if (g.c_nscale) STEP_REQUIRE(g.c_nshift && g.c_mvec && g.c_nperiod == fused.period, "step_gemm(fused): column affine must use the same period");
    if (g.compute_bf16) return step_gemm_bf16_launch(g, st, &fused);
    const int rc = step_gemm_f32_fast_launch(g, st, &fused);
    if (rc == -1) { step_set_error("step_gemm(fused): operands do not qualify for the staged path"); return STEP_ERR_ARG; }
    return rc;
}

extern "C" int step_gemm(const StepGemm* g, void* stream) {
    STEP_REQUIRE(g != nullptr, "step_gemm: null descriptor");
    return step_gemm_launch(*g, (hipStream_t)stream);
}
```

### step_amd/csrc/gemm_bf16.hip

```cpp
#include "common.h"
#include "step_internal.h"

namespace {

constexpr int BK = 32;
constexpr int PITCH = BK * 2 + 16;

typedef __attribute__((ext_vector_type(4))) float f32x4v;
typedef __attribute__((ext_vector_type(4))) __bf16 bf16x4;

typedef __attribute__((ext_vector_type(2))) float f32x2v;
typedef __attribute__((ext_vector_type(2))) __bf16 bf16x2v;
__device__ __forceinline__ uint32_t pack2(float a, float b) {
    uint32_t r;
    asm("v_cvt_pk_bf16_f32 %0, %1, %2" : "=v"(r) : "v"(a), "v"(b));
    return r;
}
__device__ __forceinline__ uint2 pack4(float a, float b, float c, float d) { return make_uint2(pack2(a, b), pack2(c, d)); }
__device__ __forceinline__ uint2 pack4(const float (&v)[4]) { return pack4(v[0], v[1], v[2], v[3]); }
__device__ __forceinline__ uint16_t bf16_of(float x) {
    return __builtin_bit_cast(uint16_t, (__bf16)x);
}
template <typename T>
__device__ __forceinline__ float ld1(const void* p, long idx) {
// ... 132 lines not shown
            const int e4 = tid + r * 256;
            if (b_kc) {
                const int kk = (e4 % (BK / 4)) * 4, nn = e4 / (BK / 4);
                *(uint2*)(Bs + nn * PITCH + kk * 2) = pack4(rb[r]);
            } else {
                const int nn = (e4 % (BN / 4)) * 4, kk = e4 / (BN / 4);
#pragma unroll
                for (int i = 0; i < 4; ++i) *(uint16_t*)(Bs + (nn + i) * PITCH + kk * 2) = bf16_of(rb[r][i]);
            }
        }
    };

    f32x16 acc[TM][TN];
#pragma unroll
    for (int i = 0; i < TM; ++i)
#pragma unroll
        for (int j = 0; j < TN; ++j)
#pragma unroll
            for (int e = 0; e < 16; ++e) acc[i][j][e] = 0.f;

    const int r = lane & 31, h = lane >> 5;
    if (kbeg < kend) {
        load_tiles(kbeg);
        for (int k0 = kbeg; k0 < kend; k0 += BK) {
            __syncthreads();
            store_tiles();
            __syncthreads();
            if (k0 + BK < kend) load_tiles(k0 + BK);
#pragma unroll
            for (int ks = 0; ks < BK / 16; ++ks) {
                bf16x8 a[TM], b[TN];
#pragma unroll
                for (int i = 0; i < TM; ++i) a[i] = *(const bf16x8*)(As + (wr * (TM * 32) + i * 32 + r) * PITCH + ks * 32 + h * 16);
#pragma unroll
                for (int j = 0; j < TN; ++j) b[j] = *(const bf16x8*)(Bs + (wc * (TN * 32) + j * 32 + r) * PITCH + ks * 32 + h * 16);
#pragma unroll
                for (int i = 0; i < TM; ++i)
#pragma unroll
                    for (int j = 0; j < TN; ++j)
                        acc[i][j] = __builtin_amdgcn_mfma_f32_32x32x16_bf16(a[i], b[j], acc[i][j], 0, 0, 0);
            }
        }
    }

    float* Cb = g.C + (long)i0 * g.scb + (long)i1 * g.scb1;
#pragma unroll
    for (int i = 0; i < TM; ++i)
#pragma unroll
        for (int j = 0; j < TN; ++j) {
            const int gn = n0 + wc * (TN * 32) + j * 32 + r;
            if (gn >= g.N) continue;
            const float bv = (g.bias != nullptr) ? g.bias[gn] : 0.f;
            const long ni = g.c_nblk ? (long)(gn / g.c_nblk) * g.c_nstride + (gn % g.c_nblk) : (long)gn;
            gemm_store_tile(acc[i][j], Cb + ni * g.scn, m0 + wr * (TM * 32) + i * 32 + 4 * h, g.M, g.ldc, g.alpha, g.accumulate, bv, g.relu, gemm_col_affine(g, gn));
        }
}


enum { KC_F32 = 0, KC_BF16 = 1, MC_F32 = 2, MC_BF16 = 3 };
constexpr int FBK = 64;
constexpr int FPITCH = FBK * 2 + 8;
constexpr int FPITCH32 = FBK * 4 + 16;

struct FastArgs {
    const GemmKSeg* ktab;
    int ktab_per;
    int a_klog, b_klog, b_nlog;
    int xcd_swizzle;
    int wide_store;
    int m_fast;
    long split_stride;
    GemmFused fu;
};

static int wide_store_ok(const StepGemm& g, bool force = false) {
    return g.accumulate != 2 && !g.a_rowsum && g.c_nblk == 0 && g.scn == 1 && g.N % 4 == 0 && g.ldc % 4 == 0 && g.scb % 4 == 0 &&
           g.scb1 % 4 == 0 && ((uintptr_t)g.C & 15) == 0 && (force || (long)g.M * g.N * g.batch >= (4L << 20));
}

__device__ __forceinline__ long remap(int i, int lg, long stride) {
    return (long)(i >> lg) * stride + (i & ((1 << lg) - 1));
}

template <int MODE, int BR>
struct Stage {
    static constexpr int NV = MODE == KC_F32 ? BR * FBK / 4 / 256 : (MODE == KC_BF16 ? BR * FBK / 8 / 256 : (MODE == MC_F32 ? BR * FBK / 16 / 256 : (BR * FBK / 32 + 255) / 256));
    static constexpr int NR = (MODE == MC_F32 || MODE == MC_BF16) ? NV * 4 : NV;
    float f[NR][4];
};

template <int MODE, int BR>
__device__ __forceinline__ void stage_load(Stage<MODE, BR>& s, const char* base, int row0, int rows, long srow, long sk, int k0,
                                           int kend, int klog, long kstride, int rlog, long rstride, int tid) {
    if constexpr (MODE == KC_F32) {
#pragma unroll
        for (int r = 0; r < s.NV; ++r) {
            const int e = tid + r * 256;
            const int k = k0 + (e % (FBK / 4)) * 4, row = row0 + e / (FBK / 4);
            const bool ok = row < rows && k < kend;
            const long off = ok ? remap(row, rlog, rstride) * srow + remap(k, klog, kstride) : 0;
            const float4 t = *(const float4*)((const float*)base + off);
            s.f[r][0] = t.x; s.f[r][1] = t.y; s.f[r][2] = t.z; s.f[r][3] = t.w;
        }
    } else if constexpr (MODE == KC_BF16) {
#pragma unroll
        for (int r = 0; r < s.NV; ++r) {
            const int e = tid + r * 256;
            const int k = k0 + (e % (FBK / 8)) * 8, row = row0 + e / (FBK / 8);
            const bool ok = row < rows && k < kend;
            const long off = ok ? remap(row, rlog, rstride) * srow + remap(k, klog, kstride) : 0;
            const float4 t = *(const float4*)((const uint16_t*)base + off);
            s.f[r][0] = t.x; s.f[r][1] = t.y; s.f[r][2] = t.z; s.f[r][3] = t.w;
        }
    } else if constexpr (MODE == MC_BF16) {
#pragma unroll
        for (int r = 0; r < s.NV; ++r) {
            const int e = tid + r * 256;
            const int row = row0 + (e % (BR / 8)) * 8, kb = k0 + (e / (BR / 8)) * 4;
#pragma unroll
            for (int j = 0; j < 4; ++j) {
                const bool ok = row < rows && kb + j < kend && e < BR * FBK / 32;
                const long off = ok ? (long)row * srow + remap(kb + j, klog, kstride) * sk : 0;
                const float4 t = *(const float4*)((const uint16_t*)base + off);
                s.f[r * 4 + j][0] = t.x; s.f[r * 4 + j][1] = t.y; s.f[r * 4 + j][2] = t.z; s.f[r * 4 + j][3] = t.w;
            }
        }
    } else {
#pragma unroll
        for (int r = 0; r < s.NV; ++r) {
            const int e = tid + r * 256;
// ... 441 lines not shown
                        v[i] = x[i] > 0.f ? kk[j] * (v[i] - m1[j] - (x[i] - mu[j]) * m2r[j]) : 0.f;
                    }
                }
                float4 r4 = make_float4(v[0], v[1], v[2], v[3]);
                if (g.accumulate == 1) { r4.x += o4[u].x; r4.y += o4[u].y; r4.z += o4[u].z; r4.w += o4[u].w; }
                *(float4*)(Cb + off[u]) = r4;
            }
        }
        if (fu.dotw) {
            float q4[4] = {dw[0], dm[0], dw[1], dm[1]};
#pragma unroll
            for (int i = 0; i < 4; ++i) q4[i] = wave_sum(q4[i]);
            if (lane == 0) { fred[wave][0] = q4[0]; fred[wave][1] = q4[1]; fred[wave][2] = q4[2]; fred[wave][3] = q4[3]; }
            __syncthreads();
            if (tid < 4) {
                const int c = c_lo + (tid >> 1);
                if (c < C) atomicAdd(fu.dots + 2 * c + (tid & 1), fred[0][tid] + fred[1][tid] + fred[2][tid] + fred[3][tid]);
            }
        }
        return;
    }
    if constexpr (BM * (BN + 4) * 4 <= 2 * BUF)
    if (fa.wide_store) {
        constexpr int TP = BN + 4;
        static_assert(BM * TP * 4 <= 2 * BUF, "staging tile must fit in the operand buffers");
        float* tile = (float*)lds;
        __syncthreads();
#pragma unroll
        for (int i = 0; i < TM; ++i)
#pragma unroll
            for (int j = 0; j < TN; ++j) {
                const int cn = wc * (TN * 32) + j * 32 + r, gn = n0 + cn;
                const GemmColAffine ca = gemm_col_affine(g, gn < g.N ? gn : 0);
                const float bv = (g.bias != nullptr && gn < g.N) ? g.bias[gn] : 0.f;
#pragma unroll
                for (int e = 0; e < 16; ++e) {
                    const int rm = wr * (TM * 32) + i * 32 + 4 * h + (e & 3) + 8 * (e >> 2), gm = m0 + rm;
                    float v = g.alpha * acc[i][j][e] * ca.cs + bv;
                    if (ca.mvec) v += ca.csh * (gm < g.M ? ca.mvec[gm] : 0.f);
                    tile[rm * TP + cn] = v;
                }
            }
        __syncthreads();
        constexpr int PIECES = BM * BN / 4;
#pragma unroll 4
        for (int pc = tid; pc < PIECES; pc += 256) {
            const int rm = pc / (BN / 4), c4 = (pc % (BN / 4)) * 4;
            const int gm = m0 + rm, gn = n0 + c4;
            if (gm >= g.M || gn >= g.N) continue;
            float4 v = *(const float4*)(tile + rm * TP + c4);
            float4* dst = (float4*)(Cb + (long)gm * g.ldc + gn);
            if (g.accumulate == 1) { const float4 o = *dst; v.x += o.x; v.y += o.y; v.z += o.z; v.w += o.w; }
            if (g.relu) { v.x = fmaxf(v.x, 0.f); v.y = fmaxf(v.y, 0.f); v.z = fmaxf(v.z, 0.f); v.w = fmaxf(v.w, 0.f); }
            *dst = v;
        }
        return;
    }
#pragma unroll
    for (int i = 0; i < TM; ++i)
#pragma unroll
        for (int j = 0; j < TN; ++j) {
            const int gn = n0 + wc * (TN * 32) + j * 32 + r;
            const int mb = m0 + wr * (TM * 32) + i * 32 + 4 * h;
            if (gn == ones_row) gemm_store_tile(acc[i][j], g.a_rowsum, mb, g.M, 1, g.alpha, 2, 0.f, 0);
            if (gn >= g.N) continue;
            const float bv = (g.bias != nullptr) ? g.bias[gn] : 0.f;
            const long ni = g.c_nblk ? (long)(gn / g.c_nblk) * g.c_nstride + (gn % g.c_nblk) : (long)gn;
            gemm_store_tile(acc[i][j], Cb + ni * g.scn, mb, g.M, g.ldc, g.alpha, g.accumulate, bv, g.relu, gemm_col_affine(g, gn));
        }
}

static int ilog2_exact(int v) {
    for (int l = 2; l < 31; ++l) if ((1 << l) == v) return l;
    return -2;
}

static int fast_mode(const void* base, int is_bf16, long srow, long sk, long sb0, long sb1, int kblk, long kstride, int rblk,
                     long rstride, int* klog, int* rlog) {
    const int vec = is_bf16 ? 8 : 4;
    if (((uintptr_t)base & 15) || sb0 % vec || sb1 % vec) return -1;
    *klog = 30; *rlog = 30;
    if (sk == 1) {
        if (srow % vec) return -1;
        if (kblk) { *klog = ilog2_exact(kblk); if (*klog < 0 || kblk % vec || kstride % vec) return -1; }
        if (rblk) { *rlog = ilog2_exact(rblk); if (*rlog < 0) return -1; }
        return is_bf16 ? KC_BF16 : KC_F32;
    }
    if (srow == 1 && is_bf16) {
        if (sk % 8 || kblk || rblk) return -1;
        return MC_BF16;
    }
    if (srow == 1 && !is_bf16) {
        if (sk % 4) return -1;
        if (kblk) { *klog = ilog2_exact(kblk); if (*klog < 0) return -1; }
        if (rblk) { *rlog = ilog2_exact(rblk); if (*rlog < 0 || rstride % 4) return -1; }
        return MC_F32;
    }
    return -1;
}

template <int BM, int BN, int AMODE>
int launch_fast_b(const StepGemm& g, const FastArgs& fa, int bmode, dim3 grid, hipStream_t st) {
    if (bmode == KC_F32) gemm_fast_kernel<BM, BN, AMODE, KC_F32, false><<<grid, 256, 0, st>>>(g, fa);
    else if (bmode == KC_BF16) gemm_fast_kernel<BM, BN, AMODE, KC_BF16, false><<<grid, 256, 0, st>>>(g, fa);
    else if (bmode == MC_F32) gemm_fast_kernel<BM, BN, AMODE, MC_F32, false><<<grid, 256, 0, st>>>(g, fa);
    else {
        if constexpr (AMODE != KC_BF16) gemm_fast_kernel<BM, BN, AMODE, MC_BF16, false><<<grid, 256, 0, st>>>(g, fa);
        else { step_set_error("step_gemm: an n-contiguous bf16 B operand needs an f32 A operand"); return STEP_ERR_ARG; }
    }
    STEP_LAUNCH_CHECK("step_gemm(bf16 fast)");
    return STEP_OK;
}
template <int BM, int BN>
int launch_fast(const StepGemm& g, const FastArgs& fa_in, int amode, int bmode, hipStream_t st) {
    dim3 grid(cdiv(g.N + (g.a_rowsum ? 1 : 0), BN), cdiv(g.M, BM), g.batch * g.splitk);
    FastArgs fa = fa_in;
    fa.xcd_swizzle = grid.x >= 2 && (grid.y * grid.z) % 8 == 0 && (long)g.M * g.K * g.batch >= (8L << 20);
    if (amode == KC_F32) return launch_fast_b<BM, BN, KC_F32>(g, fa, bmode, grid, st);
    if (amode == KC_BF16) return launch_fast_b<BM, BN, KC_BF16>(g, fa, bmode, grid, st);
    return launch_fast_b<BM, BN, MC_F32>(g, fa, bmode, grid, st);
}
// ... 83 lines not shown
                            ((fused->flags & (GEMM_FUSED_FFN_FWD | GEMM_FUSED_MASKNZ | GEMM_FUSED_BF16OUT)) ? (g.accumulate == 0 && !fused->dotw && !fused->bnx && !g.c_nscale) :
                             (fused->flags & GEMM_FUSED_INTERLEAVED) ? (128 % fused->channels == 0 && fused->channels % 8 == 0 && g.N % 8 == 0 && g.ldc % 8 == 0 &&
                                                                       ((((uintptr_t)fused->bnx) | ((uintptr_t)g.C)) & 15) == 0 && !fused->dotw) : fused->period >= 128),
                            "step_gemm: the fused DGL epilogues need the staged path with a wide-store result (aligned dense C, period >= 128)");
    if (g.splitk < 0) {
        STEP_REQUIRE(g.accumulate == 2, "step_gemm: automatic split-K needs accumulate==2");
        g.splitk = auto_splitk(g.M, g.N, g.K, g.batch, fast);
    }
    if (g.splitk < 1) g.splitk = 1;
    if (g.splitk > 1) STEP_REQUIRE(g.accumulate == 2, "step_gemm: split-K needs accumulate==2");
    STEP_REQUIRE(!(g.accumulate == 2 && (g.bias || g.relu)), "step_gemm: bias/relu epilogue not available with atomic accumulate");
    long tiles128 = (long)cdiv(g.M, 128) * cdiv(g.N, 128) * g.batch * g.splitk;
    const bool big = g.M > 64 && g.N > 64 && tiles128 >= 512;
    static const bool use_ws = []() { const char* e = getenv("STEP_GEMM_SPLITK_WS"); return !e || atoi(e) != 0; }();
    const StepGemm orig = g;
    bool ws_reduce = false;
    if (use_ws && fast && !fused && g.splitk > 1 && g.splitk_ws && !g.c_nblk && !g.c_nscale && (((uintptr_t)g.splitk_ws) & 15) == 0 &&
        (long)g.M * g.N * g.batch * g.splitk <= g.splitk_ws_floats) {
        const long mn = (long)g.M * g.N;
        ws_reduce = true;
        fa.split_stride = mn * g.batch;
        g.C = g.splitk_ws; g.ldc = g.N; g.scn = 1; g.accumulate = 0;
        g.scb = mn; g.scb1 = (long)g.batch0 * mn;
        fa.wide_store = wide_store_ok(g, true);
    }
    auto finish = [&](int rc) -> int {
        if (rc != STEP_OK || !ws_reduce) return rc;
        const long total = (long)orig.M * orig.N * orig.batch;
        const int chunk = 16;
        dim3 grid((unsigned)((total + 255) / 256), (unsigned)cdiv(orig.splitk, chunk));
        splitk_reduce_kernel<<<grid, 256, 0, st>>>(orig.splitk_ws, orig.splitk, chunk, (long)orig.M * orig.N, orig.N, orig.batch, orig.batch0, orig.C,
                                                  orig.ldc, orig.scn ? orig.scn : 1, orig.scb, orig.scb1);
        STEP_LAUNCH_CHECK("step_gemm(split-K reduce)");
        return STEP_OK;
    };
    if (fast && fused) return big ? launch_fast_fused<128, 128>(g, fa, amode, bmode, st) : launch_fast_fused<64, 64>(g, fa, amode, bmode, st);
    static const bool hop128 = []() { const char* e = getenv("STEP_GEMM_HOP128"); return !e || atoi(e) != 0; }();
    if (hop128 && fast && !big && amode == KC_BF16 && bmode == KC_BF16 && g.M >= 2048 && g.N >= 256 && tiles128 >= 256)
        return finish(launch_fast<128, 128>(g, fa, amode, bmode, st));
    static const int tall_m = []() { const char* e = getenv("STEP_GEMM_TALL_M"); return e ? atoi(e) : 1024; }();
    if (fast && !big && bmode != MC_BF16 && g.M >= tall_m && g.N > 64) {
        const long t = (long)cdiv(g.M, 128) * cdiv(g.N, 64) * g.batch * g.splitk;
        if (t >= 256) return finish(launch_fast<128, 64>(g, fa, amode, bmode, st));
    }
    if (fast) return finish(big ? launch_fast<128, 128>(g, fa, amode, bmode, st) : launch_fast<64, 64>(g, fa, amode, bmode, st));
    STEP_TRY(step_gemm_rowsum_separate(&g, st));
    if (big) return launch_bf16<128, 128>(g, st);
    return launch_bf16<64, 64>(g, st);
}

int step_gemm_segmented_launch(StepGemm g, const GemmKSeg* ktab, int ktab_per, hipStream_t st) {
    STEP_REQUIRE(g.M > 0 && g.N > 0 && g.K > 0 && g.K % 32 == 0 && g.K / 32 <= GEMM_KSEG_MAX && ktab && g.A && g.B && g.C && g.batch >= 1,
                 "step_gemm(segmented): bad descriptor");
    STEP_REQUIRE(g.accumulate != 2 && !g.bias && !g.relu && !g.a_rowsum && !g.a_kscale && g.scn <= 1 && !g.c_nblk,
                 "step_gemm(segmented): plain store / += only");
    STEP_REQUIRE((((uintptr_t)g.A | (uintptr_t)g.B) & 15) == 0, "step_gemm(segmented): 16-byte aligned bases");
    g.scn = 1; g.splitk = 1;
    if (g.batch0 == 0) g.batch0 = g.batch;
    FastArgs fa;
    memset(&fa, 0, sizeof(fa));
    fa.ktab = ktab; fa.ktab_per = ktab_per;
    fa.a_klog = fa.b_klog = fa.b_nlog = 30;
    fa.wide_store = 0;
    const long tiles128 = (long)cdiv(g.M, 128) * cdiv(g.N, 128) * g.batch;
    if (g.M > 64 && g.N > 64 && tiles128 >= 256) {
        dim3 grid(cdiv(g.N, 128), cdiv(g.M, 128), g.batch);
        if (g.compute_bf16) gemm_fast_kernel<128, 128, KC_F32, KC_F32, false, true><<<grid, 256, 0, st>>>(g, fa);
        else { dim3 g64(cdiv(g.N, 64), cdiv(g.M, 64), g.batch); gemm_fast_kernel<64, 64, KC_F32, KC_F32, true, true><<<g64, 256, 0, st>>>(g, fa); }
    } else {
        dim3 grid(cdiv(g.N, 64), cdiv(g.M, 64), g.batch);
        if (g.compute_bf16) gemm_fast_kernel<64, 64, KC_F32, KC_F32, false, true><<<grid, 256, 0, st>>>(g, fa);
        else gemm_fast_kernel<64, 64, KC_F32, KC_F32, true, true><<<grid, 256, 0, st>>>(g, fa);
    }
    STEP_LAUNCH_CHECK("step_gemm(segmented)");
    return STEP_OK;
}

int step_gemm_f32_fast_launch(StepGemm g, hipStream_t st, const GemmFused* fused) {
    if (g.a_bf16 || g.b_bf16) return -1;
    FastArgs fa;
    memset(&fa, 0, sizeof(fa));
    if (fused) fa.fu = *fused;
    int dummy;
    const int amode = fast_mode(g.A, 0, g.sam, g.sak, g.sab, g.sab1, g.a_kblk, g.a_kstride, 0, 0, &fa.a_klog, &dummy);
    const int bmode = fast_mode(g.B, 0, g.sbn, g.sbk, g.sbb, g.sbb1, g.b_kblk, g.b_kstride, g.b_nblk, g.b_nstride, &fa.b_klog, &fa.b_nlog);
    if (amode < 0 || bmode < 0 || amode == MC_BF16 || bmode == MC_BF16 || (g.a_kscale && (amode != KC_F32 || g.a_kperiod < FBK))) return -1;
    fa.wide_store = wide_store_ok(g, fused != nullptr);
    if (fused && !(fa.wide_store && !g.bias && !g.relu && g.batch == 1 && g.splitk <= 1 && fused->period >= 128)) return -1;
    if (g.splitk < 0) {
        STEP_REQUIRE(g.accumulate == 2, "step_gemm: automatic split-K needs accumulate==2");
        long tiles = (long)cdiv(g.M, 64) * cdiv(g.N, 64) * g.batch;
        long want = (512 + tiles - 1) / tiles;
        long maxs = cdiv(g.K, FBK) / 2;
        g.splitk = (int)(want < 1 ? 1 : (want > maxs ? (maxs < 1 ? 1 : maxs) : want));
    }
    if (g.splitk < 1) g.splitk = 1;
    if (g.splitk > 1) STEP_REQUIRE(g.accumulate == 2, "step_gemm: split-K needs accumulate==2");
    STEP_REQUIRE(!(g.accumulate == 2 && (g.bias || g.relu)), "step_gemm: bias/relu epilogue not available with atomic accumulate");
    if (fused) return launch_fast_f32_fused(g, fa, amode, bmode, st);
    return launch_fast_f32(g, fa, amode, bmode, st);
}
```

### step_amd/csrc/gwnet.hip

```cpp
#include "common.h"
#include "step_internal.h"
#include <vector>

namespace {

constexpr int C = 32, CAT = 224, CS = 256, CE = 512, OUT = 12, NL = 8, HID = 96;
constexpr int TIN[NL] = {13, 12, 10, 9, 7, 6, 4, 3};
constexpr int DIL[NL] = {1, 2, 1, 2, 1, 2, 1, 2};
constexpr int TOUT[NL] = {12, 10, 9, 7, 6, 4, 3, 1};

__global__ void start_conv_kernel(const float* __restrict__ hist, int B, int N, int Cin, const float* __restrict__ w,
                                  const float* __restrict__ b, float* __restrict__ x0) {
    long idx = (long)blockIdx.x * 256 + threadIdx.x;
    long total = (long)B * N * 13 * C;
    if (idx >= total) return;
    int c = idx % C, t = (idx / C) % 13;
    long bn = idx / (C * 13);
    int n = bn % N, bb = bn / N;
    float v = b[c];
    if (t >= 1) {
        const float* src = hist + (((long)bb * 12 + (t - 1)) * N + n) * Cin;
        v += w[c * 2] * src[0] + w[c * 2 + 1] * src[1];
    }
    x0[idx] = v;
}
__global__ __launch_bounds__(256) void start_conv_bwd_kernel(const float* __restrict__ hist, int B, int N, int Cin,
                                                             const float* __restrict__ dx0, float* __restrict__ dw,
                                                             float* __restrict__ db) {
    __shared__ float red[8][96];
    const int c = threadIdx.x & 31;
    const int sub = threadIdx.x >> 5;
    long npos = (long)B * N * 13;
    float a0 = 0.f, a1 = 0.f, ab = 0.f;
    for (long p = (long)blockIdx.x * 8 + sub; p < npos; p += (long)gridDim.x * 8) {
        int t = p % 13;
        long bn = p / 13;
        int n = bn % N, bb = bn / N;
        float d = dx0[p * C + c];
        ab += d;
        if (t >= 1) {
            const float* src = hist + (((long)bb * 12 + (t - 1)) * N + n) * Cin;
            a0 += d * src[0]; a1 += d * src[1];
        }
    }
    red[sub][c] = a0; red[sub][32 + c] = a1; red[sub][64 + c] = ab;
    __syncthreads();
    if (threadIdx.x < 96) {
        float s = 0.f;
#pragma unroll
        for (int r = 0; r < 8; ++r) s += red[r][threadIdx.x];
        const int cc = threadIdx.x & 31, kind = threadIdx.x >> 5;
        if (kind == 2) atomicAdd(&db[cc], s); else atomicAdd(&dw[cc * 2 + kind], s);
    }
}

__global__ __launch_bounds__(256) void row_sums_kernel(const float* __restrict__ A, int N, float* __restrict__ rs, float* __restrict__ cs_init) {
    __shared__ float red[4];
    const long row = blockIdx.x;
    float s = 0.f;
    for (int j = threadIdx.x; j < N; j += 256) s += A[row * N + j];
    s = wave_sum(s);
    if ((threadIdx.x & 63) == 0) red[threadIdx.x >> 6] = s;
    __syncthreads();
    if (threadIdx.x == 0) { rs[row] = 1.f + red[0] + red[1] + red[2] + red[3]; cs_init[row] = 1.f; }
}
__global__ __launch_bounds__(256) void col_sums_kernel(const float* __restrict__ A, int N, float* __restrict__ cs) {
    __shared__ float red[4][64];
    const int b = blockIdx.z;
    const int j = blockIdx.x * 64 + (threadIdx.x & 63), w = threadIdx.x >> 6;
    const int per = (N + gridDim.y - 1) / gridDim.y, ibeg = blockIdx.y * per, iend = min(N, ibeg + per);
    float s = 0.f;
    if (j < N)
        for (int i = ibeg + w; i < iend; i += 4) s += A[((long)b * N + i) * N + j];
    red[w][threadIdx.x & 63] = s;
    __syncthreads();
    if (w == 0 && j < N) atomicAdd(&cs[(long)b * N + j], red[0][threadIdx.x] + red[1][threadIdx.x] + red[2][threadIdx.x] + red[3][threadIdx.x]);
}
__global__ __launch_bounds__(256) void rw_build_kernel(const float* __restrict__ A, int N, const float* __restrict__ rs,
                                                       const float* __restrict__ cs, float* __restrict__ Pf, float* __restrict__ Pb,
                                                       float* __restrict__ PfT, float* __restrict__ PbT) {
    __shared__ float tile[32][33];
    const int b = blockIdx.z, i0 = blockIdx.y * 32, j0 = blockIdx.x * 32;
    const int tx = threadIdx.x & 31, ty = threadIdx.x >> 5;
    const long base = (long)b * N * N;
    for (int r = ty; r < 32; r += 8) {
        int i = i0 + r, j = j0 + tx;
        float a = (i < N && j < N) ? A[base + (long)i * N + j] : 0.f;
        tile[r][tx] = a;
        if (i < N && j < N) {
            const float v = a + (i == j ? 1.f : 0.f);
            Pf[base + (long)i * N + j] = v / rs[(long)b * N + i];
            PbT[base + (long)i * N + j] = v / cs[(long)b * N + j];
        }
    }
    __syncthreads();
    for (int r = ty; r < 32; r += 8) {
        int j = j0 + r, i = i0 + tx;
        if (i < N && j < N) {
            const float v = tile[tx][r] + (i == j ? 1.f : 0.f);
            Pb[base + (long)j * N + i] = v / cs[(long)b * N + j];
            PfT[base + (long)j * N + i] = v / rs[(long)b * N + i];
        }
    }
}
__global__ void replicate_adp_kernel(const float* __restrict__ Pa, int N, int B, float* __restrict__ P2, float* __restrict__ PT2) {
    long idx = (long)blockIdx.x * 256 + threadIdx.x;
    if (idx >= (long)N * N) return;
    int i = idx / N, j = idx % N;
    float v = Pa[idx], vt = Pa[(long)j * N + i];
    for (int b = 0; b < B; ++b) { P2[(long)b * N * N + idx] = v; PT2[(long)b * N * N + idx] = vt; }
}
__global__ void stacks_to_bf16_kernel(const float* __restrict__ P, const float* __restrict__ PT, long rows, int N, int N8,
                                      uint16_t* __restrict__ P16, uint16_t* __restrict__ PT16) {
    long idx = (long)blockIdx.x * 256 + threadIdx.x;
    if (idx >= rows * (N8 / 2)) return;
    const long row = idx / (N8 / 2);
    const int j = (int)(idx % (N8 / 2)) * 2;
    const float* src = blockIdx.y ? PT : P;
    uint16_t* dst = blockIdx.y ? PT16 : P16;
    const float a = j < N ? src[row * N + j] : 0.f, b = j + 1 < N ? src[row * N + j + 1] : 0.f;
    typedef __attribute__((ext_vector_type(2))) float f2;
    typedef __attribute__((ext_vector_type(2))) __bf16 b2;
    f2 t = {a, b};
    *(uint32_t*)(dst + row * N8 + j) = __builtin_bit_cast(uint32_t, __builtin_convertvector(t, b2));
}
__global__ __launch_bounds__(256) void slots_to_bf16T_kernel(const float* __restrict__ cat, int slot0, int sstep, int B, int N, int T, int N8,
                                                             uint16_t* __restrict__ XT) {
    __shared__ float tile[64][33];
    const int v0 = blockIdx.x * 64, t = blockIdx.y, src = blockIdx.z / B, b = blockIdx.z % B;
    const int slot = slot0 + sstep * src;
    const int c = threadIdx.x & 31, r = threadIdx.x >> 5;
    for (int i = r; i < 64; i += 8) {
        const int v = v0 + i;
        tile[i][c] = v < N ? cat[(((long)b * N + v) * T + t) * CAT + slot * C + c] : 0.f;
    }
    __syncthreads();
    const int cc = threadIdx.x >> 3, g8 = (threadIdx.x & 7) * 8;
    if (v0 + g8 < N8) {
        float v8[8];
#pragma unroll
        for (int j = 0; j < 8; ++j) v8[j] = tile[g8 + j][cc];
        *(bf16x8*)(XT + (((long)blockIdx.z * T + t) * C + cc) * N8 + v0 + g8) = pack8(v8);
    }
}
__global__ void sum_batches_kernel(const float* __restrict__ x, long n, int B, float* __restrict__ out) {
    long idx = (long)blockIdx.x * 256 + threadIdx.x;
    if (idx >= n) return;
    float s = 0.f;
    for (int b = 0; b < B; ++b) s += x[(long)b * n + idx];
    out[idx] = s;
}
__global__ __launch_bounds__(256) void row_dot_kernel(const float* __restrict__ dP, const float* __restrict__ P, int N,
                                                      float* __restrict__ out) {
    __shared__ float red[4];
    const long row = blockIdx.x;
    float s = 0.f;
    for (int j = threadIdx.x; j < N; j += 256) s += dP[row * N + j] * P[row * N + j];
    s = wave_sum(s);
    if ((threadIdx.x & 63) == 0) red[threadIdx.x >> 6] = s;
    __syncthreads();
    if (threadIdx.x == 0) out[row] = red[0] + red[1] + red[2] + red[3];
}
__global__ __launch_bounds__(256) void rw_bwd_kernel(const float* __restrict__ dPf, const float* __restrict__ dPb, int N,
                                                     const float* __restrict__ rs, const float* __restrict__ cs,
                                                     const float* __restrict__ rf, const float* __restrict__ rb, float* __restrict__ dA) {
    __shared__ float tile[32][33];
    const int b = blockIdx.z, i0 = blockIdx.y * 32, j0 = blockIdx.x * 32;
    const int tx = threadIdx.x & 31, ty = threadIdx.x >> 5;
    const long base = (long)b * N * N;
    for (int r = ty; r < 32; r += 8) {
        int j = j0 + r, i = i0 + tx;
        tile[r][tx] = (i < N && j < N) ? (dPb[base + (long)j * N + i] - rb[(long)b * N + j]) / cs[(long)b * N + j] : 0.f;
    }
    __syncthreads();
    for (int r = ty; r < 32; r += 8) {
        int i = i0 + r, j = j0 + tx;
        if (i < N && j < N)
            dA[base + (long)i * N + j] = (dPf[base + (long)i * N + j] - rf[(long)b * N + i]) / rs[(long)b * N + i] + tile[tx][r];
    }
}
__global__ __launch_bounds__(256) void softmax_relu_rows_kernel(const float* __restrict__ M, int N, float* __restrict__ P) {
    __shared__ float red[4];
    const long row = blockIdx.x;
    float mx = 0.f;
    for (int j = threadIdx.x; j < N; j += 256) mx = fmaxf(mx, M[row * N + j]);
    mx = wave_max(mx);
    if ((threadIdx.x & 63) == 0) red[threadIdx.x >> 6] = mx;
    __syncthreads();
    mx = fmaxf(fmaxf(red[0], red[1]), fmaxf(red[2], red[3]));
    __syncthreads();
    float s = 0.f;
    for (int j = threadIdx.x; j < N; j += 256) s += __expf(fmaxf(M[row * N + j], 0.f) - mx);
    s = wave_sum(s);
    if ((threadIdx.x & 63) == 0) red[threadIdx.x >> 6] = s;
    __syncthreads();
    const float inv = 1.f / (red[0] + red[1] + red[2] + red[3]);
    for (int j = threadIdx.x; j < N; j += 256) P[row * N + j] = __expf(fmaxf(M[row * N + j], 0.f) - mx) * inv;
}
__global__ void softmax_relu_bwd_kernel(const float* __restrict__ M, const float* __restrict__ P, const float* __restrict__ dP,
                                        const float* __restrict__ rdot, int N, float* __restrict__ dM) {
    long idx = (long)blockIdx.x * 256 + threadIdx.x;
    if (idx >= (long)N * N) return;
    int i = idx / N;
    dM[idx] = M[idx] > 0.f ? P[idx] * (dP[idx] - rdot[i]) : 0.f;
}

struct GatePtrs { float *wf[8], *bf[8], *wg[8], *bg[8]; };
struct SkipPtrs { float *w[8], *b[8]; };
struct MixPtrs { const float* w[7]; };
__global__ __launch_bounds__(256) void pack_weights_kernel(GatePtrs P, SkipPtrs K, MixPtrs M, float* __restrict__ wcat_all,
                                                           float* __restrict__ wcatT_all, float* __restrict__ bcat_all,
                                                           float* __restrict__ wskip, float* __restrict__ bsum, float* __restrict__ wmixT) {
    const int blk = blockIdx.x, tid = threadIdx.x;
    if (blk < 128) {
        const int L = blk >> 4;
        const int idx = (blk & 15) * 256 + tid;
        const int o = idx / 64, k = idx % 64;
        const float v = (o < 32 ? P.wf[L] : P.wg[L])[(((o & 31) * 32) + (k & 31)) * 2 + (k >> 5)];
        wcat_all[L * 4096 + idx] = v;
        wcatT_all[L * 4096 + k * 64 + o] = v;
        if (idx < 64) bcat_all[L * 64 + idx] = idx < 32 ? P.bf[L][idx] : P.bg[L][idx - 32];
    } else if (blk < 384) {
        const int o = blk - 128, k = tid;
        wskip[o * CS + k] = K.w[k >> 5][o * C + (k & 31)];
        if (o == 0) {
            float sum = 0.f;
#pragma unroll
            for (int i = 0; i < 8; ++i) sum += K.b[i][k];
            bsum[k] = sum;
        }
    } else {
        const int L = (blk - 384) / 28;
        const int idx = ((blk - 384) % 28) * 256 + tid;
        const int c = idx / CAT, j = idx % CAT;
        wmixT[L * (C * CAT) + j * C + c] = M.w[L][idx];
    }
}
__global__ void unpack_gate_grad_kernel(const float* __restrict__ dwcat_all, const float* __restrict__ dbcat_all, GatePtrs G) {
    const int L = blockIdx.y;
    const float* dwcat = dwcat_all + L * 4096;
    const float* dbcat = dbcat_all + L * 64;
    float *dwf = G.wf[L], *dbf = G.bf[L], *dwg = G.wg[L], *dbg = G.bg[L];
    int idx = blockIdx.x * 256 + threadIdx.x;
    if (idx < 64 * 64) {
        int o = idx / 64, k = idx % 64;
        float* dst = o < 32 ? dwf : dwg;
        dst[(((o & 31) * 32) + (k & 31)) * 2 + (k >> 5)] += dwcat[idx];
    }
    if (idx < 64) { if (idx < 32) dbf[idx] += dbcat[idx]; else dbg[idx - 32] += dbcat[idx]; }
}
struct XIn { const float* src; const float* stat; };

__device__ __forceinline__ void load8h(const float* chunk, int h, float* v) {
    const float4 a = *(const float4*)(chunk + 4 * h), b = *(const float4*)(chunk + 8 + 4 * h);
    v[0] = a.x; v[1] = a.y; v[2] = a.z; v[3] = a.w; v[4] = b.x; v[5] = b.y; v[6] = b.z; v[7] = b.w;
}
__device__ __forceinline__ void load8q(const float* chunk, int g, float* v) {
    const float4 a = *(const float4*)(chunk + 4 * g), b = *(const float4*)(chunk + 16 + 4 * g);
    v[0] = a.x; v[1] = a.y; v[2] = a.z; v[3] = a.w; v[4] = b.x; v[5] = b.y; v[6] = b.z; v[7] = b.w;
}
__device__ __forceinline__ void store8h(float* chunk, int h, const float* v) {
    *(float4*)(chunk + 4 * h) = make_float4(v[0], v[1], v[2], v[3]);
    *(float4*)(chunk + 8 + 4 * h) = make_float4(v[4], v[5], v[6], v[7]);
}
__device__ __forceinline__ int chan8h(int q, int h, int j) { return 16 * q + 4 * h + (j & 3) + 8 * (j >> 2); }

// ... 327 lines not shown
    if (!yprev) return;
    red[jg][c] = s1; red[jg][32 + c] = s2;
    __syncthreads();
    if (threadIdx.x < 64) {
        float a = 0.f;
#pragma unroll
        for (int r = 0; r < 8; ++r) a += red[r][threadIdx.x];
        bsum[threadIdx.x] = a;
    }
    __syncthreads();
    add_block_sums(sums, bsum);
}

__global__ void im2col_kernel(XIn x, long BN, int Tin, int Tout, int dil, float* __restrict__ xcat) {
    long idx = (long)blockIdx.x * 256 + threadIdx.x;
    if (idx >= BN * Tout * 64) return;
    int k = idx % 64, t = (idx / 64) % Tout;
    long bn = idx / (64L * Tout);
    float v = x.src[(bn * Tin + t + (k >> 5) * dil) * C + (k & 31)];
    if (x.stat) v = v * x.stat[k & 31] + x.stat[32 + (k & 31)];
    xcat[idx] = v;
}
__global__ void unpack_skip_grad_kernel(const float* __restrict__ dwskip, SkipPtrs G) {
    const int o = blockIdx.x, k = threadIdx.x;
    G.w[k >> 5][o * C + (k & 31)] += dwskip[o * CS + k];
}
__global__ void head_combine_kernel(const float* __restrict__ skip, const float* __restrict__ h2, long n, float* __restrict__ xh) {
    long idx = (long)blockIdx.x * 256 + threadIdx.x;
    if (idx >= n) return;
    xh[idx] = fmaxf(skip[idx] + h2[idx], 0.f);
}
struct MPtr8 { float* p[8]; };
__global__ void add_to8_kernel(MPtr8 dst, const float* __restrict__ v, int n) {
    int i = blockIdx.x * 256 + threadIdx.x;
    if (i >= n) return;
    const float x = v[i];
#pragma unroll
    for (int k = 0; k < 8; ++k) dst.p[k][i] += x;
}
__global__ void relu_bwd_kernel(float* __restrict__ d, const float* __restrict__ y, long n) {
    long idx = (long)blockIdx.x * 256 + threadIdx.x;
    if (idx < n && !(y[idx] > 0.f)) d[idx] = 0.f;
}

__global__ __launch_bounds__(256) void rowsum_mod_kernel(const float* __restrict__ x, int cols, int mod, float* __restrict__ out) {
    __shared__ float red[4];
    const long row = blockIdx.x;
    float s = 0.f;
    for (int j = threadIdx.x; j < cols; j += 256) s += x[row * cols + j];
    s = wave_sum(s);
    if ((threadIdx.x & 63) == 0) red[threadIdx.x >> 6] = s;
    __syncthreads();
    if (threadIdx.x == 0) atomicAdd(&out[row % mod], red[0] + red[1] + red[2] + red[3]);
}

constexpr int ADJ_NSEG = 2 * (12 + 10 + 9 + 7 + 6 + 4 + 3);
struct AdjOffsets { long cat[NL - 1], dcat[NL - 1]; };
__global__ void adj_ktab_kernel(AdjOffsets o, int N, GemmKSeg* __restrict__ tab) {
    const int j = threadIdx.x, s = blockIdx.x;
    if (j >= ADJ_NSEG) return;
    constexpr int tout[NL - 1] = {12, 10, 9, 7, 6, 4, 3};
    int i = 0, rem = j >> 1;
    while (rem >= tout[i]) { rem -= tout[i]; ++i; }
    const int t = rem, pair = j & 1, T = tout[i];
    GemmKSeg g;
    g.a_off = o.cat[i] + (long)t * CAT + (pair == 0 ? (1 + 2 * s) * C : 0);
    g.b_off = o.dcat[i] + (long)t * CAT + (pair == 0 ? (2 + 2 * s) * C : (1 + 2 * s) * C);
    g.a_rs = g.b_rs = T * CAT;
    g.a_bs = g.b_bs = (long)N * T * CAT;
    tab[s * ADJ_NSEG + j] = g;
}

inline dim3 g1(long n) { return dim3((unsigned)((n + 255) / 256)); }

struct Carver {
    float* base;
    long used = 0;
    explicit Carver(float* b) : base(b) {}
    float* take(long n) {
        float* p = base ? base + used : nullptr;
        used += (n + 3) & ~3L;
        return p;
    }
};

static inline int n8(int N) { return (N + 7) & ~7; }
static inline bool hop_transposed_operand(int N) {
    static const int min_n = []() { const char* e = getenv("STEP_HOP_XT_MIN_N"); return e ? atoi(e) : 768; }();
    return N >= min_n;
}

struct Saved {
    float *x0, *cat[NL], *tf[NL], *sg[NL], *y[NL], *mask[NL], *bnstat[NL], *zlast;
    float *Pstk, *PTstk, *Pa, *Madp, *rs, *cs;
    uint16_t *P16, *PT16;
    float *skip, *h1, *h2, *xh, *e1;
    long total;
};
Saved carve_saved(float* base, int B, int N, bool dropout) {
    Carver cv(base);
    Saved s;
    const long BN = (long)B * N;
    s.x0 = cv.take(BN * TIN[0] * C);
    s.zlast = cv.take(BN * CS);
    for (int i = 0; i < NL; ++i) {
        s.cat[i] = cv.take(BN * TOUT[i] * CAT);
        s.tf[i] = cv.take(BN * TOUT[i] * C);
        s.sg[i] = cv.take(BN * TOUT[i] * C);
        s.y[i] = i < NL - 1 ? cv.take(BN * TOUT[i] * C) : nullptr;
        s.mask[i] = (i < NL - 1 && dropout) ? cv.take(BN * TOUT[i] * C) : nullptr;
        s.bnstat[i] = cv.take(128);
    }
    s.Pstk = cv.take(3L * B * N * N);
    s.PTstk = cv.take(3L * B * N * N);
    s.P16 = (uint16_t*)cv.take(3L * B * N * n8(N) / 2);
    s.PT16 = (uint16_t*)cv.take(3L * B * N * n8(N) / 2);
    s.Pa = cv.take((long)N * N);
    s.Madp = cv.take((long)N * N);
    s.rs = cv.take(BN);
    s.cs = cv.take(BN);
    s.skip = cv.take(BN * CS);
    s.h1 = cv.take(BN * CE);
    s.h2 = cv.take(BN * CS);
// ... 107 lines not shown
    g.scb = (long)N * T * CAT; g.scb1 = (long)dstep * C;
    g.b_nblk = C; g.b_nstride = CAT; g.c_nblk = C; g.c_nstride = CAT;
    g.accumulate = dstep == 0 ? 2 : 1;
    g.compute_bf16 = bf16;
    return step_gemm_launch(g, st);
}
}

extern "C" long step_gwnet_saved_floats(int B, int N, int dropout) { return carve_saved(nullptr, B, N, dropout != 0).total; }
extern "C" long step_gwnet_work_floats(int B, int N, int backward) { return carve_work(nullptr, B, N, backward != 0).total; }
extern "C" long step_gwnet_saved_offset(int B, int N, int dropout, int item, int layer) {
    Saved s = carve_saved((float*)16, B, N, dropout != 0);
    float* p = item == 0 ? s.mask[layer] : item == 1 ? s.y[layer] : s.bnstat[layer];
    return p ? (long)(p - (float*)16) : -1;
}

template <bool BF16>
static int gwnet_layers_forward(const StepGwnetParams* p, const Saved& S, const Work& W, int B, int N, bool training, float drop_p,
                                uint64_t seed, float momentum, bool dead_bn7, const StepDynState* dyn, hipStream_t st,
                                bool first_tcn_only = false, bool skip_first_tcn = false) {
    const long BN = (long)B * N;
    for (int i = 0; i < (first_tcn_only ? 1 : NL); ++i) {
        const int Tin = TIN[i], Tout = TOUT[i], dil = DIL[i];
        const long npos = BN * Tout;
        BnFwd bn = {nullptr, nullptr, nullptr, nullptr, training ? 1 : 0, momentum, nullptr, (double)BN * Tin, nullptr};
        if (i > 0) {
            bn.gamma = p->bn_w[i - 1]; bn.beta = p->bn_b[i - 1]; bn.rm = p->bn_rm[i - 1]; bn.rv = p->bn_rv[i - 1];
            bn.stat = S.bnstat[i - 1]; bn.sums = W.acc64 + (long)(i - 1) * NCOPY * 64;
        }
        if (!(i == 0 && skip_first_tcn)) {
            tcn_fwd_kernel<BF16><<<(unsigned)cdiv(npos, 128), 256, 0, st>>>(i == 0 ? S.x0 : S.y[i - 1], bn, npos, Tin, Tout, dil, W.wcat + i * 4096,
                                                                            W.bcat + i * 64, S.tf[i], S.sg[i], S.cat[i], S.zlast, i);
            STEP_LAUNCH_CHECK("tcn_fwd");
        }
        if (first_tcn_only) break;
        if (i == NL - 1 && !(dead_bn7 && training)) break;
        STEP_TRY(nconv_fwd3(S.Pstk, S.PT16, S.cat[i], 0, 0, 1, B, N, Tout, BF16, W.xT, st));
        STEP_TRY(nconv_fwd3(S.Pstk, S.PT16, S.cat[i], 1, 2, 2, B, N, Tout, BF16, W.xT, st));
        const XIn xin = {i == 0 ? S.x0 : S.y[i - 1], i == 0 ? nullptr : S.bnstat[i - 1]};
        const bool dead = i == NL - 1;
        mix_fwd_kernel<BF16><<<(unsigned)cdiv(npos, 64), 256, 0, st>>>(S.cat[i], p->gconv_w[i], p->gconv_b[i], xin, npos, Tin, Tout, dil, drop_p,
                                                                       (uint32_t)seed, (uint32_t)(seed >> 32), (uint32_t)i, dead ? W.m7 : S.mask[i],
                                                                       dead ? W.y7 : S.y[i], W.acc64 + (long)i * NCOPY * 64, dyn);
        STEP_LAUNCH_CHECK("mix_fwd");
        if (dead) {
            const BnFwd b7 = {p->bn_w[i], p->bn_b[i], p->bn_rm[i], p->bn_rv[i], 1, momentum, S.bnstat[i], (double)npos, W.acc64 + (long)i * NCOPY * 64};
            bn_stats_only_kernel<<<1, 64, 0, st>>>(b7);
            STEP_LAUNCH_CHECK("bn7_stats");
        }
    }
    return STEP_OK;
}

static int pack_weights(const StepGwnetParams* p, const Work& W, hipStream_t st) {
    GatePtrs gp;
    SkipPtrs sp;
    MixPtrs mp;
    for (int i = 0; i < NL; ++i) {
        gp.wf[i] = p->filter_w[i]; gp.bf[i] = p->filter_b[i]; gp.wg[i] = p->gate_w[i]; gp.bg[i] = p->gate_b[i];
        sp.w[i] = p->skip_w[i]; sp.b[i] = p->skip_b[i];
        if (i < NL - 1) mp.w[i] = p->gconv_w[i];
    }
    pack_weights_kernel<<<384 + 7 * 28, 256, 0, st>>>(gp, sp, mp, W.wcat, W.wcatT, W.bcat, W.wskip, W.bsum, W.wmixT);
    STEP_LAUNCH_CHECK("pack_weights");
    return STEP_OK;
}

extern "C" int step_gwnet_forward(const float* hist, int B, int N, int Cin, const float* hidden_last, const float* adj,
                                  const StepGwnetParams* p, int training, float dropout_p, uint64_t seed, float momentum,
                                  float* saved, float* work, float* pred, void* stream) {
    return step_gwnet_forward_phase(hist, B, N, Cin, hidden_last, adj, p, training, dropout_p, seed, momentum, saved, work, pred, 0, stream);
}

extern "C" int step_gwnet_forward_phase(const float* hist, int B, int N, int Cin, const float* hidden_last, const float* adj,
                                        const StepGwnetParams* p, int training, float dropout_p, uint64_t seed, float momentum,
                                        float* saved, float* work, float* pred, int phase, void* stream) {
    return step_gwnet_forward_phase_dyn(hist, B, N, Cin, hidden_last, adj, p, training, dropout_p, seed, momentum, saved, work, pred, phase, nullptr,
                                        stream);
}
extern "C" int step_gwnet_forward_phase_dyn(const float* hist, int B, int N, int Cin, const float* hidden_last, const float* adj,
                                            const StepGwnetParams* p, int training, float dropout_p, uint64_t seed, float momentum,
                                            float* saved, float* work, float* pred, int phase, const StepDynState* dyn, void* stream) {
    STEP_REQUIRE(p && saved && work && phase >= 0 && phase <= 6, "gwnet_forward: null argument / bad phase");
    const bool do_prep = phase == 0 || phase == 1 || phase == 5, do_layers = phase == 0 || phase == 1 || phase == 6;
    const bool do_his = phase == 0 || phase == 2 || phase == 3, do_head = phase == 0 || phase == 2 || phase == 4;
    STEP_REQUIRE(!do_prep || hist, "gwnet_forward: the layer phase needs hist");
    STEP_REQUIRE(!do_layers || adj, "gwnet_forward: the layer phase needs adj");
    STEP_REQUIRE(!do_his || hidden_last, "gwnet_forward: the fc_his phase needs hidden_last");
    STEP_REQUIRE(!do_head || pred, "gwnet_forward: the head phase needs pred");
    STEP_REQUIRE(B > 0 && N > 0 && Cin >= 2, "gwnet_forward: bad sizes B=%d N=%d C=%d", B, N, Cin);
    hipStream_t st = (hipStream_t)stream;
    const bool train = (training & 1) != 0;
    const bool use_drop = train && dropout_p > 0.f;
    Saved S = carve_saved(saved, B, N, use_drop);
    Work W = carve_work(work, B, N, false);
    const long BN = (long)B * N;
    const int allbf16 = p->gemm_bf16;

    const long NN = (long)N * N;
    const bool dead_bn7 = (training & 2) != 0;
    if (do_prep) {
        STEP_TRY(zero((float*)W.acc64, 2L * NL * NCOPY * 64, st));
        start_conv_kernel<<<g1(BN * 13 * C), 256, 0, st>>>(hist, B, N, Cin, p->start_w, p->start_b, S.x0);
        STEP_LAUNCH_CHECK("start_conv");
        {
            StepGemm g = gemm_desc(N, N, 10, p->nodevec1, 10, 1, p->nodevec2, N, 1, S.Madp, N);
            STEP_TRY(step_gemm_launch(g, st));
            softmax_relu_rows_kernel<<<N, 256, 0, st>>>(S.Madp, N, S.Pa);
            replicate_adp_kernel<<<g1(NN), 256, 0, st>>>(S.Pa, N, B, S.Pstk + 2 * B * NN, S.PTstk + 2 * B * NN);
            STEP_LAUNCH_CHECK("adp_softmax");
        }
        STEP_TRY(pack_weights(p, W, st));
        if (allbf16) STEP_TRY(gwnet_layers_forward<true>(p, S, W, B, N, train, use_drop ? dropout_p : 0.f, seed, momentum, dead_bn7, dyn, st, true, false));
        else STEP_TRY(gwnet_layers_forward<false>(p, S, W, B, N, train, use_drop ? dropout_p : 0.f, seed, momentum, dead_bn7, dyn, st, true, false));
    }
    if (do_layers) {
        row_sums_kernel<<<(unsigned)BN, 256, 0, st>>>(adj, N, S.rs, S.cs);
        {
            int slices = cdiv(512, cdiv(N, 64) * B);
            if (slices > cdiv(N, 64)) slices = cdiv(N, 64);
            if (slices < 1) slices = 1;
            col_sums_kernel<<<dim3(cdiv(N, 64), slices, B), 256, 0, st>>>(adj, N, S.cs);
        }
        rw_build_kernel<<<dim3(cdiv(N, 32), cdiv(N, 32), B), 256, 0, st>>>(adj, N, S.rs, S.cs, S.Pstk, S.Pstk + B * NN, S.PTstk,
                                                                           S.PTstk + B * NN);
        STEP_LAUNCH_CHECK("rw_build");
        if (p->gemm_bf16) {
            const long rows = 3L * B * N;
            stacks_to_bf16_kernel<<<dim3((unsigned)cdiv(rows * (n8(N) / 2), 256), 2), 256, 0, st>>>(S.Pstk, S.PTstk, rows, N, n8(N), S.P16,
                                                                                                   S.PT16);
            STEP_LAUNCH_CHECK("stacks_to_bf16");
        }
        if (allbf16) STEP_TRY(gwnet_layers_forward<true>(p, S, W, B, N, train, use_drop ? dropout_p : 0.f, seed, momentum, dead_bn7, dyn, st, false, true));
        else STEP_TRY(gwnet_layers_forward<false>(p, S, W, B, N, train, use_drop ? dropout_p : 0.f, seed, momentum, dead_bn7, dyn, st, false, true));
    }

    if (do_his) {
        StepGemm g = gemm_desc((int)BN, CE, HID, hidden_last, HID, 1, p->fc_his0_w, 1, HID, S.h1, CE);
        g.bias = p->fc_his0_b; g.relu = 1;
        g.compute_bf16 = allbf16; STEP_TRY(step_gemm_launch(g, st));
        StepGemm g2 = gemm_desc((int)BN, CS, CE, S.h1, CE, 1, p->fc_his2_w, 1, CE, S.h2, CS);
        g2.bias = p->fc_his2_b; g2.relu = 1;
        g2.compute_bf16 = allbf16; STEP_TRY(step_gemm_launch(g2, st));
    }
    if (do_head) {
        StepGemm gs = gemm_desc((int)BN, CS, CS, S.zlast, CS, 1, W.wskip, 1, CS, S.skip, CS);
        gs.bias = W.bsum;
        gs.compute_bf16 = allbf16; STEP_TRY(step_gemm_launch(gs, st));
        head_combine_kernel<<<g1(BN * CS), 256, 0, st>>>(S.skip, S.h2, BN * CS, S.xh);
        STEP_LAUNCH_CHECK("head_combine");
        StepGemm g3 = gemm_desc((int)BN, CE, CS, S.xh, CS, 1, p->end1_w, 1, CS, S.e1, CE);
        g3.bias = p->end1_b; g3.relu = 1;
        g3.compute_bf16 = allbf16; STEP_TRY(step_gemm_launch(g3, st));
        StepGemm g4 = gemm_desc(N, OUT, CE, S.e1, CE, 1, p->end2_w, 1, CE, pred, 1);
        g4.batch = B; g4.sab = (long)N * CE; g4.scb = (long)OUT * N; g4.scn = N;
        g4.bias = p->end2_b;
        g4.compute_bf16 = allbf16; STEP_TRY(step_gemm_launch(g4, st));
    }
    return STEP_OK;
}

template <bool BF16>
static int gwnet_layers_backward(const StepGwnetParams* p, const StepGwnetParams* grads, const Saved& S, const Work& W, int B, int N,
                                 float** dx0, hipStream_t st, AuxLane& lane, AuxLane& leaves, hipEvent_t* adj_done) {
    const long BN = (long)B * N;
    float* dx_next = nullptr;
    float* dxbuf[2] = {W.dxa, W.dxb};
    {
        AdjOffsets o;
        for (int i = 0; i < NL - 1; ++i) { o.cat[i] = S.cat[i] - S.cat[0]; o.dcat[i] = W.dcat[i] - W.dcat[0]; }
        adj_ktab_kernel<<<3, 128, 0, st>>>(o, N, W.ktab);
        STEP_LAUNCH_CHECK("adj_ktab");
    }
    static const bool adj_pieces = []() { const char* e = getenv("STEP_ADJ_PIECES"); return !(e && e[0] == '0'); }();
    bool adj_first = true;
    auto adj_piece = [&](int lo, int hi, hipStream_t on_stream) -> int {
        int seg0 = 0, nseg = 0;
        for (int i = 0; i < lo; ++i) seg0 += 2 * TOUT[i];
        for (int i = lo; i <= hi; ++i) nseg += 2 * TOUT[i];
        StepGemm g = gemm_desc(N, N, 32 * nseg, S.cat[0], 0, 1, W.dcat[0], 1, 0, W.dPstk, N);
        g.batch = 3 * B; g.batch0 = B;
        g.scb = (long)N * N; g.scb1 = (long)B * N * N;
        g.compute_bf16 = BF16;
        g.accumulate = adj_first ? 0 : 1;
        adj_first = false;
        return step_gemm_segmented_launch(g, W.ktab + seg0, ADJ_NSEG, on_stream);
    };
    for (int i = NL - 1; i >= 0; --i) {
        const int Tin = TIN[i], Tout = TOUT[i], dil = DIL[i];
        const long npos = BN * Tout;
        const float* cat = S.cat[i];
        if (i < NL - 1) {
            const BnBwd bn = {p->bn_w[i], S.bnstat[i], grads->bn_w[i], grads->bn_b[i], (double)npos, W.acc64 + (long)i * NCOPY * 64};
            mix_bwd_kernel<BF16><<<(unsigned)cdiv(npos, 128), 256, 0, st>>>(dx_next, S.y[i], bn, S.mask[i], W.wmixT + i * (C * CAT), npos, W.dres, W.dh[i],
                                                                            W.dcat[i]);
            STEP_LAUNCH_CHECK("mix_bwd");
            STEP_TRY(nconv_bwd_data3(S.PTstk, S.P16, W.dcat[i], 2, 1, 2, B, N, Tout, BF16, W.xT, st));
            STEP_TRY(nconv_bwd_data3(S.PTstk, S.P16, W.dcat[i], 1, 0, 0, B, N, Tout, BF16, W.xT, st));
            if (adj_pieces && i == 0) { STEP_TRY(adj_piece(0, 0, lane.fork())); *adj_done = lane.done(); }
        }
        float* dx = dxbuf[i & 1];
        tcn_bwd_kernel<BF16><<<(unsigned)cdiv(BN, TB_ROWS / Tout), 256, 0, st>>>(i < NL - 1 ? W.dcat[i] : nullptr, W.dskip, i, S.tf[i], S.sg[i],
                                                                                W.wcatT + i * 4096, i < NL - 1 ? W.dres : nullptr, BN, Tin, Tout, dil,
                                                                                W.dpre[i], dx, i > 0 ? S.y[i - 1] : nullptr,
                                                                                i > 0 ? S.bnstat[i - 1] : nullptr,
                                                                                i > 0 ? W.acc64 + (long)(i - 1) * NCOPY * 64 : nullptr);
        STEP_LAUNCH_CHECK("tcn_bwd");
        const XIn xin = {i == 0 ? S.x0 : S.y[i - 1], i == 0 ? nullptr : S.bnstat[i - 1]};
        hipEvent_t ev = leaves.on ? leaves.mark() : lane.mark();
        if (adj_pieces && i == 4) STEP_TRY(adj_piece(4, 6, lane.after(ev)));
        if (adj_pieces && i == 2) STEP_TRY(adj_piece(2, 3, lane.after(ev)));
        if (adj_pieces && i == 1) STEP_TRY(adj_piece(1, 1, lane.after(ev)));
        hipStream_t leaf = leaves.after(ev);
        if (i < NL - 1) {
            StepGemm gw = gemm_desc(C, CAT, (int)npos, W.dh[i], 1, C, cat, CAT, 1, grads->gconv_w[i], CAT);
            gw.accumulate = 2; gw.splitk = -1;
            gw.a_rowsum = grads->gconv_b[i];
            gw.compute_bf16 = BF16; STEP_TRY(step_gemm_launch(gw, leaf));
        }
        im2col_kernel<<<g1(npos * 64), 256, 0, leaf>>>(xin, BN, Tin, Tout, dil, W.xcat[i]);
        STEP_LAUNCH_CHECK("im2col");
        StepGemm gw = gemm_desc(64, 64, (int)npos, W.dpre[i], 1, 64, W.xcat[i], 64, 1, W.dwcat + i * 4096, 64);
        gw.accumulate = 2; gw.splitk = -1;
        gw.a_rowsum = W.dbcat + i * 64;
        gw.compute_bf16 = BF16; STEP_TRY(step_gemm_launch(gw, leaf));
        dx_next = dx;
    }
    *dx0 = dx_next;
    if (!adj_pieces) STEP_TRY(adj_piece(0, NL - 2, lane.fork()));
    return STEP_OK;
}

extern "C" int step_gwnet_backward(const float* hist, int B, int N, int Cin, const float* hidden_last, const StepGwnetParams* p,
                                   const float* saved, float* work, const float* dpred, const StepGwnetParams* grads,
                                   float* dadj, int dropout, void* aux_stream, void* leaf_stream, void* stream) {
    STEP_REQUIRE(hist && hidden_last && p && saved && work && dpred && grads && dadj, "gwnet_backward: null argument");
    STEP_REQUIRE(B > 0 && N > 0 && Cin >= 2, "gwnet_backward: bad sizes");
    hipStream_t st = (hipStream_t)stream;
    AuxLane lane(st, (hipStream_t)aux_stream);
    AuxLane leaves(st, leaf_stream ? (hipStream_t)leaf_stream : (hipStream_t)aux_stream, 64);
    Saved S = carve_saved((float*)saved, B, N, dropout != 0);
    Work W = carve_work(work, B, N, true);
    const long BN = (long)B * N;
    const int allbf16 = p->gemm_bf16;
    auto split_for = [](long) { return -1; };

    STEP_TRY(pack_weights(p, W, st));
    STEP_TRY(zero(W.dwcat, (long)((float*)W.acc64 - W.dwcat) + 2L * NL * NCOPY * 64, st));
    const long NN = (long)N * N;

    {
        StepGemm g = gemm_desc(N, CE, OUT, dpred, 1, N, p->end2_w, CE, 1, W.d_e1, CE);
        g.batch = B; g.sab = (long)OUT * N; g.scb = (long)N * CE;
        STEP_TRY(step_gemm_launch(g, st));
        relu_bwd_kernel<<<g1(BN * CE), 256, 0, st>>>(W.d_e1, S.e1, BN * CE);
        StepGemm gx = gemm_desc((int)BN, CS, CE, W.d_e1, CE, 1, p->end1_w, CS, 1, W.d_xh, CS);
        gx.compute_bf16 = allbf16; STEP_TRY(step_gemm_launch(gx, st));
        relu_bwd_kernel<<<g1(BN * CS), 256, 0, st>>>(W.d_xh, S.xh, BN * CS);
        {
            hipStream_t leaf = leaves.fork();
            StepGemm gz = gemm_desc((int)BN, CS, CS, W.d_xh, CS, 1, W.wskip, CS, 1, W.dskip, CS);
            gz.compute_bf16 = allbf16; STEP_TRY(step_gemm_launch(gz, st));
            {
                StepGemm gw = gemm_desc(OUT, CE, N, dpred, N, 1, S.e1, CE, 1, grads->end2_w, CE);
                gw.batch = B; gw.sab = (long)OUT * N; gw.sbb = (long)N * CE; gw.scb = 0; gw.accumulate = 2;
                STEP_TRY(step_gemm_launch(gw, leaf));
                rowsum_mod_kernel<<<B * OUT, 256, 0, leaf>>>(dpred, N, OUT, grads->end2_b);
                STEP_LAUNCH_CHECK("end2_bias_grad");
                StepGemm gw1 = gemm_desc(CE, CS, (int)BN, W.d_e1, 1, CE, S.xh, CS, 1, grads->end1_w, CS);
                gw1.accumulate = 2; gw1.splitk = split_for(BN);
                gw1.a_rowsum = grads->end1_b;
                gw1.compute_bf16 = allbf16; STEP_TRY(step_gemm_launch(gw1, leaf));
            }
            STEP_TRY(zero(W.bsum, CS, leaf));
            STEP_TRY(step_colsum_launch(W.d_xh, BN, CS, CS, W.bsum, leaf));
            MPtr8 gb;
            for (int i = 0; i < NL; ++i) gb.p[i] = grads->skip_b[i];
            add_to8_kernel<<<1, 256, 0, leaf>>>(gb, W.bsum, CS);
            StepGemm gws = gemm_desc(CS, CS, (int)BN, W.d_xh, 1, CS, S.zlast, CS, 1, W.dwskip, CS);
            gws.accumulate = 2; gws.splitk = split_for(BN);
            gws.compute_bf16 = allbf16; STEP_TRY(step_gemm_launch(gws, leaf));
            if (hipMemcpyAsync(W.d_h2, W.d_xh, (size_t)BN * CS * sizeof(float), hipMemcpyDeviceToDevice, leaf) != hipSuccess) {
                step_set_error("gwnet_backward: copy failed");
                return STEP_ERR_HIP;
            }
            relu_bwd_kernel<<<g1(BN * CS), 256, 0, leaf>>>(W.d_h2, S.h2, BN * CS);
            StepGemm gw2 = gemm_desc(CS, CE, (int)BN, W.d_h2, 1, CS, S.h1, CE, 1, grads->fc_his2_w, CE);
            gw2.accumulate = 2; gw2.splitk = split_for(BN);
            gw2.a_rowsum = grads->fc_his2_b;
            gw2.compute_bf16 = allbf16; STEP_TRY(step_gemm_launch(gw2, leaf));
            StepGemm gh1 = gemm_desc((int)BN, CE, CS, W.d_h2, CS, 1, p->fc_his2_w, CE, 1, W.d_h1, CE);
            gh1.compute_bf16 = allbf16; STEP_TRY(step_gemm_launch(gh1, leaf));
            relu_bwd_kernel<<<g1(BN * CE), 256, 0, leaf>>>(W.d_h1, S.h1, BN * CE);
            StepGemm gw0 = gemm_desc(CE, HID, (int)BN, W.d_h1, 1, CE, hidden_last, HID, 1, grads->fc_his0_w, HID);
            gw0.accumulate = 2; gw0.splitk = split_for(BN);
            gw0.a_rowsum = grads->fc_his0_b;
            gw0.compute_bf16 = allbf16; STEP_TRY(step_gemm_launch(gw0, leaf));
        }
    }

    float* dx0 = nullptr;
    hipEvent_t adj_done = nullptr;
    if (allbf16) STEP_TRY(gwnet_layers_backward<true>(p, grads, S, W, B, N, &dx0, st, lane, leaves, &adj_done));
    else STEP_TRY(gwnet_layers_backward<false>(p, grads, S, W, B, N, &dx0, st, lane, leaves, &adj_done));
    STEP_TRY(lane.wait_done(adj_done));
    static const bool tail_leaves = []() { const char* e = getenv("STEP_TAIL_LEAVES"); return !(e && e[0] == '0'); }();
    if (!tail_leaves) STEP_TRY(leaves.join());
    hipStream_t leaf = tail_leaves ? leaves.fork() : st;
    row_dot_kernel<<<(unsigned)BN, 256, 0, st>>>(W.dPstk, S.Pstk, N, W.rf);
    row_dot_kernel<<<(unsigned)BN, 256, 0, st>>>(W.dPstk + B * NN, S.Pstk + B * NN, N, W.rb);
    rw_bwd_kernel<<<dim3(cdiv(N, 32), cdiv(N, 32), B), 256, 0, st>>>(W.dPstk, W.dPstk + B * NN, N, S.rs, S.cs, W.rf, W.rb, dadj);
    STEP_LAUNCH_CHECK("rw_bwd");
    {
        GatePtrs gg;
        SkipPtrs sg;
        for (int i = 0; i < NL; ++i) {
            gg.wf[i] = grads->filter_w[i]; gg.bf[i] = grads->filter_b[i]; gg.wg[i] = grads->gate_w[i]; gg.bg[i] = grads->gate_b[i];
            sg.w[i] = grads->skip_w[i]; sg.b[i] = nullptr;
        }
        start_conv_bwd_kernel<<<128, 256, 0, leaf>>>(hist, B, N, Cin, dx0, grads->start_w, grads->start_b);
        STEP_LAUNCH_CHECK("start_conv_bwd");
        unpack_gate_grad_kernel<<<dim3(16, NL), 256, 0, leaf>>>(W.dwcat, W.dbcat, gg);
        unpack_skip_grad_kernel<<<CS, CS, 0, leaf>>>(W.dwskip, sg);
    }
    {
        float* rdot = W.y7;
        sum_batches_kernel<<<g1(NN), 256, 0, leaf>>>(W.dPstk + 2 * B * NN, NN, B, W.dPa);
        row_dot_kernel<<<N, 256, 0, leaf>>>(W.dPa, S.Pa, N, rdot);
        softmax_relu_bwd_kernel<<<g1(NN), 256, 0, leaf>>>(S.Madp, S.Pa, W.dPa, rdot, N, W.dM);
        STEP_LAUNCH_CHECK("adp_bwd");
        StepGemm g1_ = gemm_desc(N, 10, N, W.dM, N, 1, p->nodevec2, 1, N, grads->nodevec1, 10);
        g1_.accumulate = 1;
        STEP_TRY(step_gemm_launch(g1_, leaf));
        StepGemm g2_ = gemm_desc(10, N, N, p->nodevec1, 1, 10, W.dM, N, 1, grads->nodevec2, N);
        g2_.accumulate = 1;
        STEP_TRY(step_gemm_launch(g2_, leaf));
    }
    STEP_LAUNCH_CHECK("rw_bwd");
    return STEP_OK;
}
```

### step_amd/csrc/step_internal.h

```cpp
#pragma once
#include <hip/hip_runtime.h>
#include <vector>
#include "../../include/step_hip.h"

enum { GEMM_FUSED_INTERLEAVED = 1, GEMM_FUSED_FFN_FWD = 2, GEMM_FUSED_MASKNZ = 4, GEMM_FUSED_BF16OUT = 8 };
struct GemmFused {
    const float* dotw; float* dots;
    const float* bnx; const float* bncoef; const float* bnstat;
    int channels, period;
    int flags;
    const float* ffn_bias; const void* maskx; float p; unsigned seed_lo, seed_hi, site;
};

struct GemmKSeg { long a_off, b_off, a_bs, b_bs; int a_rs, b_rs; };
constexpr int GEMM_KSEG_MAX = 128;
int step_gemm_segmented_launch(StepGemm g, const GemmKSeg* ktab, int ktab_per, hipStream_t st);

int step_gemm_launch(StepGemm g, hipStream_t st);
int step_gemm_auto_splitk(int M, int N, int K, int batch);
int step_gemm_launch_fused(StepGemm g, const GemmFused& fused, hipStream_t st);
int step_gemm_bf16_launch(StepGemm g, hipStream_t st, const GemmFused* fused = nullptr);
int step_gemm_f32_fast_launch(StepGemm g, hipStream_t st, const GemmFused* fused = nullptr);

static inline StepGemm gemm_desc(int M, int N, int K, const float* A, long sam, long sak, const float* B, long sbk,
                                 long sbn, float* C, long ldc) {
    StepGemm g;
    memset(&g, 0, sizeof(g));
    g.M = M; g.N = N; g.K = K; g.batch = 1;
    g.A = A; g.sam = sam; g.sak = sak;
    g.B = B; g.sbk = sbk; g.sbn = sbn;
    g.C = C; g.ldc = ldc; g.scn = 1;
    g.alpha = 1.f; g.splitk = 1;
    return g;
}

int step_gemm_rowsum_separate(StepGemm* g, hipStream_t st);
int dgl_conv2_fwd_mfma(const float* a1, const float* w, const float* b, const float* sc, const float* sh, float* a2, float* partial,
                       int N, int T1, int* nblk, hipStream_t st);
int dgl_conv2_dgrad_mfma(const float* dz, const float* w, float* din, int N, int T1, const float* bnx, const float* coef, const float* stat,
                         int own, hipStream_t st);
int dgl_conv2_wgrad_xhat_mfma(const float* dz, const float* a1, const float* stat1, float* scratch, float* graw, int N, int T1, hipStream_t st);
int dgl_conv2_wgrad_finish(const float* graw, const float* w, const float* stat1, const float* gamma1, const float* beta1, double count,
                           float* dw, float* db, float* dgamma1, float* dbeta1, float* coef1, int raw, hipStream_t st);
int dgl_conv1_fwd_cl(const float* x, const float* w, const float* b, void* a1h, float* partial, int N, int T, int stat_limit, int* nblk,
                     hipStream_t st);
long dgl_conv2_pack_floats();
int dgl_conv2_fwd_cl(const void* a1h, const float* w, const float* b, const float* sc, const float* sh, void* a2h, float* partial, int N,
                     int T1, int* nblk, float* pack, hipStream_t st);
int dgl_conv2_dgrad_cl(const void* dz2h, const float* w, const float* sc, void* dz1h, int N, int T1, const void* a1h, const float* coef,
                       const float* stat, int own, float* pack, hipStream_t st);
int dgl_conv2_wgrad_cl(const void* dz2h, const void* a1h, float* scratch, float* graw, int N, int T1, hipStream_t st);
int dgl_conv1_wgrad_cl(const void* dz1h, const float* x, float* scratch, float* dw, float* db, int N, int T, hipStream_t st);
long dgl_conv2_wgrad_scratch_floats(int N, int T1);
int dgl_conv2_wgrad_mfma(const float* dz, const float* a1, const float* sc, const float* sh, float* scratch, float* dw, float* db, int N,
                         int T1, hipStream_t st);
int dgl_conv1_wgrad_mfma(const float* dz, const float* x, float* scratch, float* dw, float* db, int N, int T, hipStream_t st);
int step_colsum_launch(const float* x, long rows, int cols, long ld, float* out, hipStream_t st);

struct AuxLane {
    hipStream_t main, aux;
    bool on;
    int next = 0, base = 0;
    AuxLane(hipStream_t m, hipStream_t a, int base_ = 0) : main(m), aux(a), on(a != nullptr && a != m), base(base_) {}
    static hipEvent_t event(int k) {
        thread_local std::vector<hipEvent_t> pool[16];
        int dev = 0;
        (void)hipGetDevice(&dev);
        std::vector<hipEvent_t>& v = pool[dev & 15];
        while ((int)v.size() <= k) {
            hipEvent_t e;
            if (hipEventCreateWithFlags(&e, hipEventDisableTiming) != hipSuccess) return nullptr;
            v.push_back(e);
        }
        return v[k];
    }
    hipStream_t fork() {
        if (!on) return main;
        hipEvent_t e = event(base + (next++ & 63));
        if (!e || hipEventRecord(e, main) != hipSuccess || hipStreamWaitEvent(aux, e, 0) != hipSuccess) { on = false; return main; }
        return aux;
    }
    hipEvent_t mark() {
        if (!on) return nullptr;
        hipEvent_t e = event(base + (next++ & 63));
        if (!e || hipEventRecord(e, main) != hipSuccess) { on = false; return nullptr; }
        return e;
    }
    hipStream_t after(hipEvent_t e) {
        if (!on || !e) return main;
        if (hipStreamWaitEvent(aux, e, 0) != hipSuccess) { on = false; return main; }
        return aux;
    }
    hipEvent_t done() {
        if (!on) return nullptr;
        hipEvent_t e = event(base + (next++ & 63));
        if (!e || hipEventRecord(e, aux) != hipSuccess) return nullptr;
        return e;
    }
    int wait_done(hipEvent_t e) {
        if (!on) return STEP_OK;
        if (!e) return join();
        if (hipStreamWaitEvent(main, e, 0) != hipSuccess) { step_set_error("backward: stream join failed"); return STEP_ERR_HIP; }
        return STEP_OK;
    }
// ... 11 lines not shown
```

Baseline: 2378.

## Fold small kernels and memsets into neighbouring kernels across DGL and GWNet passes

Removes many small launches by merging them into adjacent kernels. Memsets move into BN finalize, bn3 backward and weight packing. ReLU backward becomes a mask applied in the GEMM store epilogue, and row and column sums plus the two row-dot kernels are merged. The bf16 stack conversion is folded into rw_build, and the BN1 finalize and dots/coef reductions are folded into conv2 and packing. An environment variable restores the old unfused path, and the change adds interface and buffer-layout complexity with some risk of subtle ordering bugs.

```diff
diff --git a/include/step_hip.h b/include/step_hip.h
--- a/include/step_hip.h
+++ b/include/step_hip.h
@@ -30,6 +30,7 @@
     const float *c_nscale, *c_nshift, *c_mvec;
     int c_nperiod;
     float* splitk_ws; long splitk_ws_floats;
+    const float* c_relu_mask;
 } StepGemm;
 int step_gemm(const StepGemm* g, void* stream);
 
diff --git a/step_amd/_lib.py b/step_amd/_lib.py
--- a/step_amd/_lib.py
+++ b/step_amd/_lib.py
@@ -19,7 +19,7 @@
                 ("b_nblk", _i), ("b_nstride", _l), ("c_nblk", _i), ("c_nstride", _l),
                 ("a_kscale", _vp), ("a_kshift", _vp), ("a_kperiod", _i),
                 ("batch0", _i), ("sab1", _l), ("sbb1", _l), ("scb1", _l), ("compute_bf16", _i), ("a_rowsum", _vp), ("c_nscale", _vp), ("c_nshift", _vp), ("c_mvec", _vp),
-                ("c_nperiod", _i), ("splitk_ws", _vp), ("splitk_ws_floats", _l)]
+                ("c_nperiod", _i), ("splitk_ws", _vp), ("splitk_ws_floats", _l), ("c_relu_mask", _vp)]
 
 
 class StepDglParams(ctypes.Structure):
@@ -208,7 +208,7 @@
 def gemm(a, b, c, M, N, K, sam, sak, sbk, sbn, ldc, batch=1, sab=0, sbb=0, scb=0, scn=1, alpha=1.0,
          accumulate=0, bias=None, relu=False, splitk=1, a_off=0, b_off=0, c_off=0, a_k=(0, 0), b_k=(0, 0),
          b_n=(0, 0), c_n=(0, 0), a_kscale=None, a_kshift=None, a_kperiod=0, batch0=0, sab1=0, sbb1=0, scb1=0, compute_bf16=False, a_rowsum=None, c_nscale=None, c_nshift=None, c_mvec=None,
-         c_nperiod=0, splitk_ws=None):
+         c_nperiod=0, splitk_ws=None, c_relu_mask=None):
     g = StepGemm()
     g.M, g.N, g.K, g.batch = M, N, K, batch
     g.A = a.data_ptr() + a_off * a.element_size()
@@ -234,4 +234,6 @@
         g.splitk_ws, g.splitk_ws_floats = ptr(splitk_ws), splitk_ws.numel()
     if a_kscale is not None:
         g.a_kscale, g.a_kshift, g.a_kperiod = a_kscale.data_ptr(), a_kshift.data_ptr(), a_kperiod
+    if c_relu_mask is not None:
+        g.c_relu_mask = c_relu_mask.data_ptr() + c_off * 4
     check(lib().step_gemm(ctypes.byref(g), stream()), "step_gemm")
diff --git a/step_amd/csrc/common.h b/step_amd/csrc/common.h
--- a/step_amd/csrc/common.h
+++ b/step_amd/csrc/common.h
@@ -102,8 +102,15 @@
 }
 
 __device__ __forceinline__ void gemm_store_tile(const f32x16& acc, float* col, int mb, int M, long ldc, float alpha, int accumulate,
-                                                float bv, int relu, GemmColAffine ca = GemmColAffine{1.f, 0.f, nullptr}) {
+                                                float bv, int relu, GemmColAffine ca = GemmColAffine{1.f, 0.f, nullptr},
+                                                const float* mcol = nullptr) {
     float val[16];
+    bool open[16];
+#pragma unroll
+    for (int e = 0; e < 16; ++e) {
+        const int gm = mb + (e & 3) + 8 * (e >> 2);
+        open[e] = mcol == nullptr || (gm < M && mcol[(long)gm * ldc] > 0.f);
+    }
 #pragma unroll
     for (int e = 0; e < 16; ++e) {
         const int gm = mb + (e & 3) + 8 * (e >> 2);
@@ -128,6 +135,7 @@
             const int gm = mb + (e & 3) + 8 * (e >> 2);
             float v = val[e] + old[e] + bv;
             if (relu) v = fmaxf(v, 0.f);
+            if (!open[e]) v = 0.f;
             if (gm < M) col[(long)gm * ldc] = v;
         }
     } else {
@@ -136,6 +144,7 @@
             const int gm = mb + (e & 3) + 8 * (e >> 2);
             float v = val[e] + bv;
             if (relu) v = fmaxf(v, 0.f);
+            if (!open[e]) v = 0.f;
             if (gm < M) col[(long)gm * ldc] = v;
         }
     }
diff --git a/step_amd/csrc/dgl.hip b/step_amd/csrc/dgl.hip
--- a/step_amd/csrc/dgl.hip
+++ b/step_amd/csrc/dgl.hip
@@ -74,9 +74,11 @@
 __global__ __launch_bounds__(256) void bn_finalize_kernel(const float* __restrict__ partial, int nblk, int C, double count,
                                                           const float* __restrict__ gamma, const float* __restrict__ beta,
                                                           float* __restrict__ rmean, float* __restrict__ rvar, int training,
-                                                          float momentum, float* __restrict__ stat) {
+                                                          float momentum, float* __restrict__ stat, float* __restrict__ zero_p, int zero_n) {
     __shared__ double r1[256], r2[256];
     const int c = blockIdx.x, tid = threadIdx.x;
+    if (zero_p && c == 0)
+        for (int i = tid; i < zero_n; i += 256) zero_p[i] = 0.f;
     double mean, var;
     if (training) {
         double a = 0.0, q = 0.0;
@@ -136,8 +138,10 @@
 }
 __global__ void bn_finalize_sums_kernel(const double* __restrict__ sums, int C, double count, const float* __restrict__ gamma,
                                         const float* __restrict__ beta, float* __restrict__ rmean, float* __restrict__ rvar,
-                                        int training, float momentum, float* __restrict__ stat) {
+                                        int training, float momentum, float* __restrict__ stat, float* __restrict__ zero_p, int zero_n) {
     const int c = threadIdx.x;
+    if (zero_p)
+        for (int i = c; i < zero_n; i += blockDim.x) zero_p[i] = 0.f;
     if (c >= C) return;
     double mean, var;
     if (training) {
@@ -194,9 +198,11 @@
                                                            const float* __restrict__ gamma, const float* __restrict__ stat,
                                                            float* __restrict__ dgamma, float* __restrict__ dbeta,
                                                            float* __restrict__ dbias, float* __restrict__ dgpre,
-                                                           float* __restrict__ dgpreT, float* __restrict__ colsum) {
+                                                           float* __restrict__ dgpreT, float* __restrict__ colsum,
+                                                           float* __restrict__ dots_o) {
     __shared__ double r1[256], r2[256];
     const int j = blockIdx.x, tid = threadIdx.x;
+    if (dots_o && tid < 32) dots_o[j * 32 + tid] = 0.f;
     const float mean = stat[2 * EMB + j], rstd = stat[3 * EMB + j];
     double a = 0.0, q = 0.0;
     for (int n = tid; n < N; n += 256) {
@@ -680,6 +686,32 @@
     dots[i] = (float)a;
 }
 
+__global__ __launch_bounds__(256) void dots_coef_kernel(const float* __restrict__ dots_o, float* __restrict__ dots, const float* __restrict__ stat,
+                                                        const float* __restrict__ gamma, double count, float* __restrict__ dgamma,
+                                                        float* __restrict__ dbeta, float* __restrict__ coef, float* __restrict__ graw, int nraw) {
+    constexpr int C = 16;
+    __shared__ float sd[32];
+    const int i = threadIdx.x;
+    if (i < 32) {
+        double a = 0.0;
+        for (int o = 0; o < EMB; ++o) a += dots_o[o * 32 + i];
+        sd[i] = (float)a;
+        dots[i] = sd[i];
+    }
+    for (int k = i; k < nraw; k += 256) graw[k] = 0.f;
+    __syncthreads();
+    if (i < C) {
+        const int c = i;
+        const float S1 = sd[2 * c + 1];
+        const float S2 = stat[3 * C + c] * (sd[2 * c] - stat[2 * C + c] * S1);
+        dgamma[c] += S2;
+        dbeta[c] += S1;
+        coef[c] = (float)(S1 / count);
+        coef[C + c] = (float)(S2 / count);
+        coef[2 * C + c] = gamma[c] * stat[3 * C + c];
+    }
+}
+
 static bool dgl_channels_last(const StepDglParams* p) {
     const char* e = getenv("STEP_DGL_F32_STORAGE");
     return p->gemm_bf16 && !(e && e[0] == '1');
@@ -692,7 +724,7 @@
 
 extern "C" long step_dgl_global_saved_floats(int N, int T) {
     long T1 = T - 9, T2 = T - 18;
-    return (long)N * 8 * T1 + (long)N * 16 * T2 + (long)N * EMB + 4 * 8 + 4 * 16 + 4 * EMB + (long)EMB * 16 * T2 + 128;
+    return (long)N * 8 * T1 + (long)N * 16 * T2 + (long)N * EMB + 4 * 8 + 4 * 16 + 4 * EMB + (long)EMB * 16 * T2 + 128 + dgl_conv2_pack_floats();
 }
 static long fc_splitk_ws_floats(int N, int T2) {
     const int splits = step_gemm_auto_splitk(N, EMB, 16 * T2, 1);
@@ -710,6 +742,7 @@
     long T1 = T - 9, T2 = T - 18;
     return saved + (long)N * 8 * T1 + (long)N * 16 * T2 + (long)N * EMB + 4 * 8 + 4 * 16 + 4 * EMB;
 }
+static float* saved_pack(float* saved, int N, int T) { return saved_wp(saved, N, T) + (long)EMB * 16 * (T - 18) + 128; }
 static void carve_saved(float* saved, int N, int T, float** a1, float** a2, float** gpre, float** st1, float** st2, float** st3) {
     long T1 = T - 9, T2 = T - 18;
     *a1 = saved; saved += (long)N * 8 * T1;
@@ -721,13 +754,13 @@
 }
 
 static int dgl_bn_stats(const float* partial, int nblk, int C, double count, const float* gamma, const float* beta, float* rm, float* rv,
-                        int training, float momentum, float* stat, double* sums, hipStream_t st) {
+                        int training, float momentum, float* stat, double* sums, hipStream_t st, float* zero_p = nullptr, int zero_n = 0) {
     if (nblk < 8192) {
-        bn_finalize_kernel<<<C, 256, 0, st>>>(partial, nblk, C, count, gamma, beta, rm, rv, training, momentum, stat);
+        bn_finalize_kernel<<<C, 256, 0, st>>>(partial, nblk, C, count, gamma, beta, rm, rv, training, momentum, stat, zero_p, zero_n);
     } else {
         if (hipMemsetAsync(sums, 0, 2 * C * sizeof(double), st) != hipSuccess) { step_set_error("memset failed"); return STEP_ERR_HIP; }
         bn_sums_sliced_kernel<<<dim3(C, 32), 256, 0, st>>>(partial, nblk, C, sums);
-        bn_finalize_sums_kernel<<<1, 64, 0, st>>>(sums, C, count, gamma, beta, rm, rv, training, momentum, stat);
+        bn_finalize_sums_kernel<<<1, 64, 0, st>>>(sums, C, count, gamma, beta, rm, rv, training, momentum, stat, zero_p, zero_n);
     }
     STEP_LAUNCH_CHECK("bn_stats");
     return STEP_OK;
@@ -747,6 +780,9 @@
     double* own_sums = (double*)(work + part_floats + dgl_conv2_pack_floats());
     float* wp = saved_wp(saved, N, T);
     float* shiftdot = wp + (long)EMB * 16 * T2;
+    const bool fold = cl && all && !shard && !step_chain_unfused();
+    DglBn1Finalize bn1 = {};
+    bool bn1_in_pack = false;
     if (all || phase == 1) {
         int nblk;
         if (cl) {
@@ -759,15 +795,19 @@
             nblk = grid.x * grid.y;
         }
         if (shard) bn_sums_kernel<<<8, 256, 0, st>>>(partial, nblk, 8, sums);
+        else if (fold && nblk < 8192) {
+            bn1 = DglBn1Finalize{partial, nblk, count1, p->bn1_w, p->bn1_b, p->bn1_rm, p->bn1_rv, training, momentum, st1};
+            bn1_in_pack = true;
+        }
         else STEP_TRY(dgl_bn_stats(partial, nblk, 8, count1, p->bn1_w, p->bn1_b, p->bn1_rm, p->bn1_rv, training, momentum, st1, own_sums, st));
         STEP_LAUNCH_CHECK("bn1");
     }
     if (all || phase == 2) {
-        if (shard) bn_finalize_sums_kernel<<<1, 64, 0, st>>>(sums, 8, count1, p->bn1_w, p->bn1_b, p->bn1_rm, p->bn1_rv, training, momentum, st1);
+        if (shard) bn_finalize_sums_kernel<<<1, 64, 0, st>>>(sums, 8, count1, p->bn1_w, p->bn1_b, p->bn1_rm, p->bn1_rv, training, momentum, st1, nullptr, 0);
         int nblk;
         if (cl) {
             STEP_TRY(dgl_conv2_fwd_cl(a1, p->conv2_w, p->conv2_b, st1, st1 + 8, a2, partial, N, T1, &nblk,
-                                      work + part_floats, st));
+                                      fold ? saved_pack(saved, N, T) : work + part_floats, bn1_in_pack ? &bn1 : nullptr, st));
         } else if (p->gemm_bf16) {
             STEP_TRY(dgl_conv2_fwd_mfma(a1, p->conv2_w, p->conv2_b, st1, st1 + 8, a2, partial, N, T1, &nblk, st));
         } else {
@@ -777,15 +817,16 @@
             nblk = grid.x * grid.y;
         }
         if (shard) bn_sums_kernel<<<16, 256, 0, st>>>(partial, nblk, 16, sums + 16);
-        else STEP_TRY(dgl_bn_stats(partial, nblk, 16, count2, p->bn2_w, p->bn2_b, p->bn2_rm, p->bn2_rv, training, momentum, st2, own_sums, st));
+        else STEP_TRY(dgl_bn_stats(partial, nblk, 16, count2, p->bn2_w, p->bn2_b, p->bn2_rm, p->bn2_rv, training, momentum, st2, own_sums, st,
+                                   fold ? shiftdot : nullptr, 128));
         STEP_LAUNCH_CHECK("bn2");
     }
     if (all || phase == 3) {
-        if (shard) bn_finalize_sums_kernel<<<1, 64, 0, st>>>(sums + 16, 16, count2, p->bn2_w, p->bn2_b, p->bn2_rm, p->bn2_rv, training, momentum, st2);
+        if (shard) bn_finalize_sums_kernel<<<1, 64, 0, st>>>(sums + 16, 16, count2, p->bn2_w, p->bn2_b, p->bn2_rm, p->bn2_rv, training, momentum, st2, nullptr, 0);
         const long K = 16L * T2;
         StepGemm gm = gemm_desc(N, EMB, (int)K, a2, K, 1, p->fc_w, 1, K, gpre, EMB);
         if (cl) {
-            if (hipMemsetAsync(shiftdot, 0, 128 * sizeof(float), st) != hipSuccess) { step_set_error("memset failed"); return STEP_ERR_HIP; }
+            if (!fold && hipMemsetAsync(shiftdot, 0, 128 * sizeof(float), st) != hipSuccess) { step_set_error("memset failed"); return STEP_ERR_HIP; }
             fc_prep_kernel<<<dim3(cdiv(T2, 256), EMB), 256, 0, st>>>(p->fc_w, st2, (uint4*)wp, shiftdot, T2);
             gpre_init_kernel<<<cdiv((long)N * EMB, 256), 256, 0, st>>>(gpre, shiftdot, (long)N * EMB);
             STEP_LAUNCH_CHECK("fc_prep");
@@ -891,39 +932,46 @@
         const float* wp = saved_wp((float*)saved, N, T);
         float* dots_o = coef + 256 + 64 + 1344;
         float* colsum = coef + 128;
+        const bool unfused = step_chain_unfused();
+        const bool fold_coef = phase == 0 && !shard && !unfused;
         if (do_fc) {
-            bn3_relu_bwd_kernel<<<EMB, 256, 0, st>>>(dg, gpre, N, p->bn3_w, st3, grads->bn3_w, grads->bn3_b, grads->fc_b, dgpre, dgpreT, colsum);
+            bn3_relu_bwd_kernel<<<EMB, 256, 0, st>>>(dg, gpre, N, p->bn3_w, st3, grads->bn3_w, grads->bn3_b, grads->fc_b, dgpre, dgpreT, colsum,
+                                                     unfused ? nullptr : dots_o);
             STEP_LAUNCH_CHECK("bn3_bwd");
             StepGemm gm = gemm_desc(EMB, (int)K, N, dgpre, 1, EMB, a2, K, 1, wraw, K);
             gm.b_bf16 = 1;
             gm.compute_bf16 = 1;
             STEP_TRY(step_gemm_launch(gm, st));
-            if (hipMemsetAsync(dots_o, 0, EMB * 32 * sizeof(float), st) != hipSuccess) { step_set_error("memset failed"); return STEP_ERR_HIP; }
+            if (unfused && hipMemsetAsync(dots_o, 0, EMB * 32 * sizeof(float), st) != hipSuccess) { step_set_error("memset failed"); return STEP_ERR_HIP; }
             fc_unpermute_kernel<<<dim3(cdiv(T2, 256), EMB), 256, 0, st>>>(wraw, p->fc_w, st2, colsum, grads->fc_w, dots_o, T2, fresh_fc);
-            dots_reduce_kernel<<<1, 64, 0, st>>>(dots_o, dots);
+            if (fold_coef) dots_coef_kernel<<<1, 256, 0, st>>>(dots_o, dots, st2, p->bn2_w, count2, grads->bn2_w, grads->bn2_b, coef, graw, dgl_conv2_wgrad_out_floats());
+            else dots_reduce_kernel<<<1, 64, 0, st>>>(dots_o, dots);
             STEP_LAUNCH_CHECK("fc_unpermute");
         }
         if (do_mid) {
-            bn2_fused_coef_kernel<<<1, 64, 0, st>>>(dots, st2, p->bn2_w, count2, grads->bn2_w, grads->bn2_b, coef);
+            if (!fold_coef) bn2_fused_coef_kernel<<<1, 64, 0, st>>>(dots, st2, p->bn2_w, count2, grads->bn2_w, grads->bn2_b, coef);
             STEP_LAUNCH_CHECK("bn2_fused_coef");
             StepGemm gm = gemm_desc(N, (int)K, EMB, dgpre, EMB, 1, wp, K, 1, d_a2, K);
             gm.b_bf16 = 1;
             gm.compute_bf16 = 1;
             GemmFused fu = {nullptr, nullptr, a2, coef, st2, 16, T2, GEMM_FUSED_INTERLEAVED};
             STEP_TRY(step_gemm_launch_fused(gm, fu, st));
-            STEP_TRY(dgl_conv2_wgrad_cl(d_a2, a1, wg_scratch, graw, N, T1, st));
+            STEP_TRY(dgl_conv2_wgrad_cl(d_a2, a1, wg_scratch, graw, N, T1, fold_coef ? 0 : 1, st));
         }
         if (do_tail) {
             STEP_TRY(dgl_conv2_wgrad_finish(graw, p->conv2_w, st1, p->bn1_w, p->bn1_b, count1, grads->conv2_w, grads->conv2_b, grads->bn1_w,
                                             grads->bn1_b, coef + 64, 1, st));
-            STEP_TRY(dgl_conv2_dgrad_cl(d_a2, p->conv2_w, st1, d_a1, N, T1, a1, coef + 64, st1, shard ? shard->own1 : T1, wraw, st));
+            if (!shard && !unfused)
+                STEP_TRY(dgl_conv2_dgrad_cl(d_a2, p->conv2_w, st1, d_a1, N, T1, a1, coef + 64, st1, T1, saved_pack((float*)saved, N, T), 0, st));
+            else
+                STEP_TRY(dgl_conv2_dgrad_cl(d_a2, p->conv2_w, st1, d_a1, N, T1, a1, coef + 64, st1, shard ? shard->own1 : T1, wraw, 1, st));
             STEP_TRY(dgl_conv1_wgrad_cl(d_a1, series_nt, wg_scratch, grads->conv1_w, grads->conv1_b, N, T, st));
         }
         return STEP_OK;
     }
     if (do_fc) {
         float* colsum = coef + 128;
-        bn3_relu_bwd_kernel<<<EMB, 256, 0, st>>>(dg, gpre, N, p->bn3_w, st3, grads->bn3_w, grads->bn3_b, grads->fc_b, dgpre, dgpreT, colsum);
+        bn3_relu_bwd_kernel<<<EMB, 256, 0, st>>>(dg, gpre, N, p->bn3_w, st3, grads->bn3_w, grads->bn3_b, grads->fc_b, dgpre, dgpreT, colsum, nullptr);
         STEP_LAUNCH_CHECK("bn3_bwd");
         {
             StepGemm gm = gemm_desc(EMB, (int)K, N, dgpre, 1, EMB, a2, K, 1, grads->fc_w, K);
diff --git a/step_amd/csrc/dgl_conv_mfma.hip b/step_amd/csrc/dgl_conv_mfma.hip
--- a/step_amd/csrc/dgl_conv_mfma.hip
+++ b/step_amd/csrc/dgl_conv_mfma.hip
@@ -452,8 +452,8 @@
         partial[((long)blockIdx.y * gridDim.x + blockIdx.x) * (2 * C1_) + tid] = red[0][tid] + red[1][tid] + red[2][tid] + red[3][tid];
 }
 
-__global__ void conv2_pack_kernel(const float* __restrict__ w, const float* __restrict__ b, const float* __restrict__ sc,
-                                  const float* __restrict__ sh, uint4* __restrict__ pack) {
+__device__ __forceinline__ void conv2_pack_body(const float* __restrict__ w, const float* __restrict__ b, const float* sc, const float* sh,
+                                                uint4* __restrict__ pack) {
     const int lane = threadIdx.x & 63, s = threadIdx.x >> 6, ln = lane & 15, q = lane >> 4;
     float v[8];
     if (s < 3) {
@@ -475,6 +475,52 @@
         }
         ((float*)(pack + 8 * 64))[threadIdx.x] = a;
     }
+}
+__global__ void conv2_pack_kernel(const float* __restrict__ w, const float* __restrict__ b, const float* __restrict__ sc,
+                                  const float* __restrict__ sh, uint4* __restrict__ pack) {
+    conv2_pack_body(w, b, sc, sh, pack);
+}
+__global__ __launch_bounds__(512) void conv2_pack_bn1_kernel(const float* __restrict__ w, const float* __restrict__ b, uint4* __restrict__ pack,
+                                                             DglBn1Finalize f) {
+    constexpr int C = C1_;
+    __shared__ double r1[2][256], r2[2][256];
+    __shared__ float scs[C], shs[C];
+    const int half = threadIdx.x >> 8, tid = threadIdx.x & 255;
+    for (int round = 0; round < C / 2; ++round) {
+        const int c = 2 * round + half;
+        double mean, var;
+        if (f.training) {
+            double a = 0.0, q = 0.0;
+            for (int i = tid; i < f.nblk; i += 256) { a += f.partial[(long)i * 2 * C + c]; q += f.partial[(long)i * 2 * C + C + c]; }
+            r1[half][tid] = a; r2[half][tid] = q;
+            __syncthreads();
+            for (int s = 128; s > 0; s >>= 1) {
+                if (tid < s) { r1[half][tid] += r1[half][tid + s]; r2[half][tid] += r2[half][tid + s]; }
+                __syncthreads();
+            }
+            mean = r1[half][0] / f.count;
+            var = fmax(r2[half][0] / f.count - mean * mean, 0.0);
+            if (tid == 0) {
+                f.rmean[c] = (1.f - f.momentum) * f.rmean[c] + f.momentum * (float)mean;
+                f.rvar[c] = (1.f - f.momentum) * f.rvar[c] + f.momentum * (float)(var * f.count / fmax(f.count - 1.0, 1.0));
+            }
+        } else {
+            mean = f.rmean[c];
+            var = f.rvar[c];
+        }
+        if (tid == 0) {
+            float rstd = (float)(1.0 / sqrt(var + 1e-5));
+            float sc = f.gamma[c] * rstd;
+            float sh = f.beta[c] - (float)mean * sc;
+            f.stat[c] = sc;
+            f.stat[C + c] = sh;
+            f.stat[2 * C + c] = (float)mean;
+            f.stat[3 * C + c] = rstd;
+            scs[c] = sc; shs[c] = sh;
+        }
+        __syncthreads();
+    }
+    conv2_pack_body(w, b, scs, shs, pack);
 }
 
 __global__ __launch_bounds__(256) void conv2_fwd_cl_kernel(const uint4* __restrict__ a1h, const uint4* __restrict__ pack,
@@ -830,26 +876,28 @@
 }
 long dgl_conv2_pack_floats() { return 8 * 64 * 4 + 16; }
 int dgl_conv2_fwd_cl(const void* a1h, const float* w, const float* b, const float* sc, const float* sh, void* a2h, float* partial, int N,
-                     int T1, int* nblk, float* pack, hipStream_t st) {
+                     int T1, int* nblk, float* pack, const DglBn1Finalize* bn1, hipStream_t st) {
     const int T2 = T1 - (KW - 1);
     dim3 grid(cdiv(T2, FW_TT), N);
-    conv2_pack_kernel<<<1, 512, 0, st>>>(w, b, sc, sh, (uint4*)pack);
+    if (bn1) conv2_pack_bn1_kernel<<<1, 512, 0, st>>>(w, b, (uint4*)pack, *bn1);
+    else conv2_pack_kernel<<<1, 512, 0, st>>>(w, b, sc, sh, (uint4*)pack);
     conv2_fwd_cl_kernel<<<grid, 256, 0, st>>>((const uint4*)a1h, (const uint4*)pack, (uint2*)a2h, partial, T1);
     STEP_LAUNCH_CHECK("conv2_fwd_cl");
     *nblk = grid.x * grid.y;
     return STEP_OK;
 }
 int dgl_conv2_dgrad_cl(const void* dz2h, const float* w, const float* sc, void* dz1h, int N, int T1, const void* a1h, const float* coef,
-                       const float* stat, int own, float* pack, hipStream_t st) {
-    conv2_pack_kernel<<<1, 512, 0, st>>>(w, w, sc, sc, (uint4*)pack);
+                       const float* stat, int own, float* pack, int build_pack, hipStream_t st) {
+    if (build_pack) conv2_pack_kernel<<<1, 512, 0, st>>>(w, w, sc, sc, (uint4*)pack);
     conv2_dgrad_cl_kernel<<<dim3(cdiv(T1, FW_TT), N), 256, 0, st>>>((const uint4*)dz2h, (const uint4*)pack, (uint2*)dz1h, T1, (const uint2*)a1h, coef, stat, own);
     STEP_LAUNCH_CHECK("conv2_dgrad_cl");
     return STEP_OK;
 }
-int dgl_conv2_wgrad_cl(const void* dz2h, const void* a1h, float* scratch, float* graw, int N, int T1, hipStream_t st) {
+long dgl_conv2_wgrad_out_floats() { return WG_OUT; }
+int dgl_conv2_wgrad_cl(const void* dz2h, const void* a1h, float* scratch, float* graw, int N, int T1, int clear_graw, hipStream_t st) {
     const int T2 = T1 - (KW - 1);
     dim3 grid(cdiv(T2, WG_SC * WG_PASSES), N);
-    if (hipMemsetAsync(graw, 0, WG_OUT * sizeof(float), st) != hipSuccess) { step_set_error("memset failed"); return STEP_ERR_HIP; }
+    if (clear_graw && hipMemsetAsync(graw, 0, WG_OUT * sizeof(float), st) != hipSuccess) { step_set_error("memset failed"); return STEP_ERR_HIP; }
     conv2_wgrad_cl_kernel<<<grid, 256, 0, st>>>((const uint4*)dz2h, (const uint4*)a1h, scratch, T1);
     STEP_LAUNCH_CHECK("conv2_wgrad_cl");
     conv_wgrad_reduce_kernel<<<dim3(cdiv(WG_OUT, 64), wgrad_slices(grid.x * grid.y)), 256, 0, st>>>(scratch, grid.x * grid.y, WG_OUT, CO * CI * KW, graw, graw + CO * CI * KW);
diff --git a/step_amd/csrc/gemm.hip b/step_amd/csrc/gemm.hip
--- a/step_amd/csrc/gemm.hip
+++ b/step_amd/csrc/gemm.hip
@@ -209,7 +209,8 @@
             if (gn >= g.N) continue;
             const float bv = (g.bias != nullptr) ? g.bias[gn] : 0.f;
             const long ni = g.c_nblk ? (long)(gn / g.c_nblk) * g.c_nstride + (gn % g.c_nblk) : (long)gn;
-            gemm_store_tile(acc[i][j], Cb + ni * g.scn, m0 + wr * (TM * 32) + i * 32 + 4 * lk, g.M, g.ldc, g.alpha, g.accumulate, bv, g.relu, gemm_col_affine(g, gn));
+            gemm_store_tile(acc[i][j], Cb + ni * g.scn, m0 + wr * (TM * 32) + i * 32 + 4 * lk, g.M, g.ldc, g.alpha, g.accumulate, bv, g.relu, gemm_col_affine(g, gn),
+                            g.c_relu_mask ? g.c_relu_mask + ((Cb - g.C) + ni * g.scn) : nullptr);
         }
 }
 
@@ -335,7 +336,8 @@
     if (!n_ok) return;
     const float bv = (g.bias != nullptr) ? g.bias[gn] : 0.f;
     const long ni = (long)(gn >> d.cn_sh) * g.c_nstride + (gn & d.cn_mask);
-    gemm_store_tile(acc, Cb + ni * g.scn, m0 + 4 * lk, g.M, g.ldc, g.alpha, g.accumulate, bv, g.relu, gemm_col_affine(g, gn));
+    gemm_store_tile(acc, Cb + ni * g.scn, m0 + 4 * lk, g.M, g.ldc, g.alpha, g.accumulate, bv, g.relu, gemm_col_affine(g, gn),
+                    g.c_relu_mask ? g.c_relu_mask + ((Cb - g.C) + ni * g.scn) : nullptr);
 }
 
 static bool pow2(int x) { return x > 0 && (x & (x - 1)) == 0; }
@@ -404,6 +406,8 @@
         STEP_REQUIRE(g.batch == 1 && g.alpha == 1.f && !g.a_bf16 && !g.a_kscale, "step_gemm: a_rowsum needs batch 1, alpha 1, f32 A without affine");
     if (g.c_nscale)
         STEP_REQUIRE(g.c_nshift && g.c_mvec && g.c_nperiod > 0, "step_gemm: c_nscale needs c_nshift, c_mvec and a positive c_nperiod");
+    if (g.c_relu_mask)
+        STEP_REQUIRE(g.accumulate != 2 && g.splitk <= 1, "step_gemm: c_relu_mask needs a plain store or += (no atomics, no split-K)");
     if (g.compute_bf16) return step_gemm_bf16_launch(g, st);
     {
         const int rc = step_gemm_f32_fast_launch(g, st);
@@ -439,6 +443,7 @@
     STEP_REQUIRE(fused.channels > 0 && fused.period > 0 && (long)fused.channels * fused.period == g.N, "step_gemm(fused): N != channels * period");
     if (g.scn == 0) g.scn = 1;
     if (g.splitk < 1) g.splitk = 1;
+    STEP_REQUIRE(!g.c_relu_mask, "step_gemm(fused): c_relu_mask is not available with the fused epilogues");
     if (g.c_nscale) STEP_REQUIRE(g.c_nshift && g.c_mvec && g.c_nperiod == fused.period, "step_gemm(fused): column affine must use the same period");
     if (g.compute_bf16) return step_gemm_bf16_launch(g, st, &fused);
     const int rc = step_gemm_f32_fast_launch(g, st, &fused);
diff --git a/step_amd/csrc/gemm_bf16.hip b/step_amd/csrc/gemm_bf16.hip
--- a/step_amd/csrc/gemm_bf16.hip
+++ b/step_amd/csrc/gemm_bf16.hip
@@ -208,7 +208,8 @@
             if (gn >= g.N) continue;
             const float bv = (g.bias != nullptr) ? g.bias[gn] : 0.f;
             const long ni = g.c_nblk ? (long)(gn / g.c_nblk) * g.c_nstride + (gn % g.c_nblk) : (long)gn;
-            gemm_store_tile(acc[i][j], Cb + ni * g.scn, m0 + wr * (TM * 32) + i * 32 + 4 * h, g.M, g.ldc, g.alpha, g.accumulate, bv, g.relu, gemm_col_affine(g, gn));
+            gemm_store_tile(acc[i][j], Cb + ni * g.scn, m0 + wr * (TM * 32) + i * 32 + 4 * h, g.M, g.ldc, g.alpha, g.accumulate, bv, g.relu, gemm_col_affine(g, gn),
+                            g.c_relu_mask ? g.c_relu_mask + ((Cb - g.C) + ni * g.scn) : nullptr);
         }
 }
 
@@ -231,7 +232,7 @@
 
 static int wide_store_ok(const StepGemm& g, bool force = false) {
     return g.accumulate != 2 && !g.a_rowsum && g.c_nblk == 0 && g.scn == 1 && g.N % 4 == 0 && g.ldc % 4 == 0 && g.scb % 4 == 0 &&
-           g.scb1 % 4 == 0 && ((uintptr_t)g.C & 15) == 0 && (force || (long)g.M * g.N * g.batch >= (4L << 20));
+           g.scb1 % 4 == 0 && (((uintptr_t)g.C | (uintptr_t)g.c_relu_mask) & 15) == 0 && (force || (long)g.M * g.N * g.batch >= (4L << 20));
 }
 
 __device__ __forceinline__ long remap(int i, int lg, long stride) {
@@ -779,6 +780,13 @@
             float4* dst = (float4*)(Cb + (long)gm * g.ldc + gn);
             if (g.accumulate == 1) { const float4 o = *dst; v.x += o.x; v.y += o.y; v.z += o.z; v.w += o.w; }
             if (g.relu) { v.x = fmaxf(v.x, 0.f); v.y = fmaxf(v.y, 0.f); v.z = fmaxf(v.z, 0.f); v.w = fmaxf(v.w, 0.f); }
+            if (g.c_relu_mask) {
+                const float4 y = *(const float4*)(g.c_relu_mask + ((Cb - g.C) + (long)gm * g.ldc + gn));
+                if (!(y.x > 0.f)) v.x = 0.f;
+                if (!(y.y > 0.f)) v.y = 0.f;
+                if (!(y.z > 0.f)) v.z = 0.f;
+                if (!(y.w > 0.f)) v.w = 0.f;
+            }
             *dst = v;
         }
         return;
@@ -793,7 +801,8 @@
             if (gn >= g.N) continue;
             const float bv = (g.bias != nullptr) ? g.bias[gn] : 0.f;
             const long ni = g.c_nblk ? (long)(gn / g.c_nblk) * g.c_nstride + (gn % g.c_nblk) : (long)gn;
-            gemm_store_tile(acc[i][j], Cb + ni * g.scn, mb, g.M, g.ldc, g.alpha, g.accumulate, bv, g.relu, gemm_col_affine(g, gn));
+            gemm_store_tile(acc[i][j], Cb + ni * g.scn, mb, g.M, g.ldc, g.alpha, g.accumulate, bv, g.relu, gemm_col_affine(g, gn),
+                            g.c_relu_mask ? g.c_relu_mask + ((Cb - g.C) + ni * g.scn) : nullptr);
         }
 }
 
@@ -983,7 +992,7 @@
 int step_gemm_segmented_launch(StepGemm g, const GemmKSeg* ktab, int ktab_per, hipStream_t st) {
     STEP_REQUIRE(g.M > 0 && g.N > 0 && g.K > 0 && g.K % 32 == 0 && g.K / 32 <= GEMM_KSEG_MAX && ktab && g.A && g.B && g.C && g.batch >= 1,
                  "step_gemm(segmented): bad descriptor");
-    STEP_REQUIRE(g.accumulate != 2 && !g.bias && !g.relu && !g.a_rowsum && !g.a_kscale && g.scn <= 1 && !g.c_nblk,
+    STEP_REQUIRE(g.accumulate != 2 && !g.bias && !g.relu && !g.a_rowsum && !g.a_kscale && g.scn <= 1 && !g.c_nblk && !g.c_relu_mask,
                  "step_gemm(segmented): plain store / += only");
     STEP_REQUIRE((((uintptr_t)g.A | (uintptr_t)g.B) & 15) == 0, "step_gemm(segmented): 16-byte aligned bases");
     g.scn = 1; g.splitk = 1;
diff --git a/step_amd/csrc/gwnet.hip b/step_amd/csrc/gwnet.hip
--- a/step_amd/csrc/gwnet.hip
+++ b/step_amd/csrc/gwnet.hip
@@ -76,21 +76,56 @@
     __syncthreads();
     if (w == 0 && j < N) atomicAdd(&cs[(long)b * N + j], red[0][threadIdx.x] + red[1][threadIdx.x] + red[2][threadIdx.x] + red[3][threadIdx.x]);
 }
+__global__ __launch_bounds__(256) void row_col_sums_kernel(const float* __restrict__ A, int N, long BN, int nx, int slices,
+                                                           float* __restrict__ rs, float* __restrict__ cs) {
+    __shared__ float red[4][64];
+    if ((long)blockIdx.x < BN) {
+        const long row = blockIdx.x;
+        float s = 0.f;
+        for (int j = threadIdx.x; j < N; j += 256) s += A[row * N + j];
+        s = wave_sum(s);
+        if ((threadIdx.x & 63) == 0) red[0][threadIdx.x >> 6] = s;
+        __syncthreads();
+        if (threadIdx.x == 0) rs[row] = 1.f + red[0][0] + red[0][1] + red[0][2] + red[0][3];
+        return;
+    }
+    const int blk = (int)(blockIdx.x - BN);
+    const int bx = blk % nx, by = (blk / nx) % slices, b = blk / (nx * slices);
+    const int j = bx * 64 + (threadIdx.x & 63), w = threadIdx.x >> 6;
+    const int per = (N + slices - 1) / slices, ibeg = by * per, iend = min(N, ibeg + per);
+    float s = 0.f;
+    if (j < N)
+        for (int i = ibeg + w; i < iend; i += 4) s += A[((long)b * N + i) * N + j];
+    red[w][threadIdx.x & 63] = s;
+    __syncthreads();
+    if (w == 0 && j < N) atomicAdd(&cs[(long)b * N + j], red[0][threadIdx.x] + red[1][threadIdx.x] + red[2][threadIdx.x] + red[3][threadIdx.x]);
+}
+__device__ __forceinline__ uint16_t stack_bf16(float v) {
+    typedef __attribute__((ext_vector_type(2))) float f2;
+    typedef __attribute__((ext_vector_type(2))) __bf16 b2;
+    const f2 t = {v, 0.f};
+    return (uint16_t)__builtin_bit_cast(uint32_t, __builtin_convertvector(t, b2));
+}
 __global__ __launch_bounds__(256) void rw_build_kernel(const float* __restrict__ A, int N, const float* __restrict__ rs,
                                                        const float* __restrict__ cs, float* __restrict__ Pf, float* __restrict__ Pb,
-                                                       float* __restrict__ PfT, float* __restrict__ PbT) {
+                                                       float* __restrict__ PfT, float* __restrict__ PbT, int N8, uint16_t* __restrict__ Pf16,
+                                                       uint16_t* __restrict__ Pb16, uint16_t* __restrict__ PfT16, uint16_t* __restrict__ PbT16) {
     __shared__ float tile[32][33];
     const int b = blockIdx.z, i0 = blockIdx.y * 32, j0 = blockIdx.x * 32;
     const int tx = threadIdx.x & 31, ty = threadIdx.x >> 5;
-    const long base = (long)b * N * N;
+    const long base = (long)b * N * N, base16 = (long)b * N * N8;
     for (int r = ty; r < 32; r += 8) {
         int i = i0 + r, j = j0 + tx;
         float a = (i < N && j < N) ? A[base + (long)i * N + j] : 0.f;
         tile[r][tx] = a;
         if (i < N && j < N) {
             const float v = a + (i == j ? 1.f : 0.f);
-            Pf[base + (long)i * N + j] = v / rs[(long)b * N + i];
-            PbT[base + (long)i * N + j] = v / cs[(long)b * N + j];
+            const float pf = v / rs[(long)b * N + i], pbt = v / cs[(long)b * N + j];
+            Pf[base + (long)i * N + j] = pf;
+            PbT[base + (long)i * N + j] = pbt;
+            if (Pf16) { Pf16[base16 + (long)i * N8 + j] = stack_bf16(pf); PbT16[base16 + (long)i * N8 + j] = stack_bf16(pbt); }
+        } else if (Pf16 && i < N && j < N8) {
+            Pf16[base16 + (long)i * N8 + j] = 0; PbT16[base16 + (long)i * N8 + j] = 0;
         }
     }
     __syncthreads();
@@ -98,17 +133,30 @@
         int j = j0 + r, i = i0 + tx;
         if (i < N && j < N) {
             const float v = tile[tx][r] + (i == j ? 1.f : 0.f);
-            Pb[base + (long)j * N + i] = v / cs[(long)b * N + j];
-            PfT[base + (long)j * N + i] = v / rs[(long)b * N + i];
-        }
-    }
-}
-__global__ void replicate_adp_kernel(const float* __restrict__ Pa, int N, int B, float* __restrict__ P2, float* __restrict__ PT2) {
+            const float pb = v / cs[(long)b * N + j], pft = v / rs[(long)b * N + i];
+            Pb[base + (long)j * N + i] = pb;
+            PfT[base + (long)j * N + i] = pft;
+            if (Pf16) { Pb16[base16 + (long)j * N8 + i] = stack_bf16(pb); PfT16[base16 + (long)j * N8 + i] = stack_bf16(pft); }
+        } else if (Pf16 && j < N && i < N8) {
+            Pb16[base16 + (long)j * N8 + i] = 0; PfT16[base16 + (long)j * N8 + i] = 0;
+        }
+    }
+}
+__global__ void replicate_adp_kernel(const float* __restrict__ Pa, int N, int B, float* __restrict__ P2, float* __restrict__ PT2, int N8,
+                                     uint16_t* __restrict__ P16, uint16_t* __restrict__ PT16) {
     long idx = (long)blockIdx.x * 256 + threadIdx.x;
     if (idx >= (long)N * N) return;
     int i = idx / N, j = idx % N;
     float v = Pa[idx], vt = Pa[(long)j * N + i];
     for (int b = 0; b < B; ++b) { P2[(long)b * N * N + idx] = v; PT2[(long)b * N * N + idx] = vt; }
+    if (!P16) return;
+    const uint16_t h = stack_bf16(v), ht = stack_bf16(vt);
+    for (int b = 0; b < B; ++b) {
+        const long row = ((long)b * N + i) * N8;
+        P16[row + j] = h; PT16[row + j] = ht;
+        if (j == N - 1)
+            for (int k = N; k < N8; ++k) { P16[row + k] = 0; PT16[row + k] = 0; }
+    }
 }
 __global__ void stacks_to_bf16_kernel(const float* __restrict__ P, const float* __restrict__ PT, long rows, int N, int N8,
                                       uint16_t* __restrict__ P16, uint16_t* __restrict__ PT16) {
@@ -161,6 +209,20 @@
     __syncthreads();
     if (threadIdx.x == 0) out[row] = red[0] + red[1] + red[2] + red[3];
 }
+__global__ __launch_bounds__(256) void row_dot2_kernel(const float* __restrict__ dP, const float* __restrict__ P, int N, long rows0,
+                                                       float* __restrict__ out0, float* __restrict__ out1) {
+    __shared__ float red[4];
+    const long row = blockIdx.x;
+    float s = 0.f;
+    for (int j = threadIdx.x; j < N; j += 256) s += dP[row * N + j] * P[row * N + j];
+    s = wave_sum(s);
+    if ((threadIdx.x & 63) == 0) red[threadIdx.x >> 6] = s;
+    __syncthreads();
+    if (threadIdx.x == 0) {
+        const float v = red[0] + red[1] + red[2] + red[3];
+        if (row < rows0) out0[row] = v; else out1[row - rows0] = v;
+    }
+}
 __global__ __launch_bounds__(256) void rw_bwd_kernel(const float* __restrict__ dPf, const float* __restrict__ dPb, int N,
                                                      const float* __restrict__ rs, const float* __restrict__ cs,
                                                      const float* __restrict__ rf, const float* __restrict__ rb, float* __restrict__ dA) {
@@ -208,10 +270,46 @@
 struct GatePtrs { float *wf[8], *bf[8], *wg[8], *bg[8]; };
 struct SkipPtrs { float *w[8], *b[8]; };
 struct MixPtrs { const float* w[7]; };
+constexpr int ADJ_NSEG = 2 * (12 + 10 + 9 + 7 + 6 + 4 + 3);
+struct AdjOffsets { long cat[NL - 1], dcat[NL - 1]; };
+__device__ __forceinline__ void adj_ktab_entry(const AdjOffsets& o, int N, GemmKSeg* __restrict__ tab, int s, int j) {
+    if (j >= ADJ_NSEG) return;
+    constexpr int tout[NL - 1] = {12, 10, 9, 7, 6, 4, 3};
+    int i = 0, rem = j >> 1;
+    while (rem >= tout[i]) { rem -= tout[i]; ++i; }
+    const int t = rem, pair = j & 1, T = tout[i];
+    GemmKSeg g;
+    g.a_off = o.cat[i] + (long)t * CAT + (pair == 0 ? (1 + 2 * s) * C : 0);
+    g.b_off = o.dcat[i] + (long)t * CAT + (pair == 0 ? (2 + 2 * s) * C : (1 + 2 * s) * C);
+    g.a_rs = g.b_rs = T * CAT;
+    g.a_bs = g.b_bs = (long)N * T * CAT;
+    tab[s * ADJ_NSEG + j] = g;
+}
+__global__ void adj_ktab_kernel(AdjOffsets o, int N, GemmKSeg* __restrict__ tab) { adj_ktab_entry(o, N, tab, blockIdx.x, threadIdx.x); }
+struct PackExtra { float* zero; long zero_n; int nzero; float* ones; long ones_n; int nones; AdjOffsets adj; int N; GemmKSeg* ktab; };
+constexpr int PACK_BLOCKS = 384 + 7 * 28;
 __global__ __launch_bounds__(256) void pack_weights_kernel(GatePtrs P, SkipPtrs K, MixPtrs M, float* __restrict__ wcat_all,
                                                            float* __restrict__ wcatT_all, float* __restrict__ bcat_all,
-                                                           float* __restrict__ wskip, float* __restrict__ bsum, float* __restrict__ wmixT) {
+                                                           float* __restrict__ wskip, float* __restrict__ bsum, float* __restrict__ wmixT,
+                                                           PackExtra X) {
     const int blk = blockIdx.x, tid = threadIdx.x;
+    if (blk >= PACK_BLOCKS) {
+        int e = blk - PACK_BLOCKS;
+        if (e < X.nzero) {
+#pragma unroll
+            for (int k = 0; k < 4; ++k) { const long i = (long)e * 1024 + k * 256 + tid; if (i < X.zero_n) X.zero[i] = 0.f; }
+            return;
+        }
+        e -= X.nzero;
+        if (e < X.nones) {
+#pragma unroll
+            for (int k = 0; k < 4; ++k) { const long i = (long)e * 1024 + k * 256 + tid; if (i < X.ones_n) X.ones[i] = 1.f; }
+            return;
+        }
+        e -= X.nones;
+        if (X.ktab && e < 3) adj_ktab_entry(X.adj, X.N, X.ktab, e, tid);
+        return;
+    }
     if (blk < 128) {
         const int L = blk >> 4;
         const int idx = (blk & 15) * 256 + tid;
@@ -645,23 +743,6 @@
     if ((threadIdx.x & 63) == 0) red[threadIdx.x >> 6] = s;
     __syncthreads();
     if (threadIdx.x == 0) atomicAdd(&out[row % mod], red[0] + red[1] + red[2] + red[3]);
-}
-
-constexpr int ADJ_NSEG = 2 * (12 + 10 + 9 + 7 + 6 + 4 + 3);
-struct AdjOffsets { long cat[NL - 1], dcat[NL - 1]; };
-__global__ void adj_ktab_kernel(AdjOffsets o, int N, GemmKSeg* __restrict__ tab) {
-    const int j = threadIdx.x, s = blockIdx.x;
-    if (j >= ADJ_NSEG) return;
-    constexpr int tout[NL - 1] = {12, 10, 9, 7, 6, 4, 3};
-    int i = 0, rem = j >> 1;
-    while (rem >= tout[i]) { rem -= tout[i]; ++i; }
-    const int t = rem, pair = j & 1, T = tout[i];
-    GemmKSeg g;
-    g.a_off = o.cat[i] + (long)t * CAT + (pair == 0 ? (1 + 2 * s) * C : 0);
-    g.b_off = o.dcat[i] + (long)t * CAT + (pair == 0 ? (2 + 2 * s) * C : (1 + 2 * s) * C);
-    g.a_rs = g.b_rs = T * CAT;
-    g.a_bs = g.b_bs = (long)N * T * CAT;
-    tab[s * ADJ_NSEG + j] = g;
 }
 
 inline dim3 g1(long n) { return dim3((unsigned)((n + 255) / 256)); }
@@ -875,7 +956,7 @@
     return STEP_OK;
 }
 
-static int pack_weights(const StepGwnetParams* p, const Work& W, hipStream_t st) {
+static int pack_weights(const StepGwnetParams* p, const Work& W, PackExtra X, hipStream_t st) {
     GatePtrs gp;
     SkipPtrs sp;
     MixPtrs mp;
@@ -884,7 +965,10 @@
         sp.w[i] = p->skip_w[i]; sp.b[i] = p->skip_b[i];
         if (i < NL - 1) mp.w[i] = p->gconv_w[i];
     }
-    pack_weights_kernel<<<384 + 7 * 28, 256, 0, st>>>(gp, sp, mp, W.wcat, W.wcatT, W.bcat, W.wskip, W.bsum, W.wmixT);
+    X.nzero = X.zero ? (int)cdiv(X.zero_n, 1024) : 0;
+    X.nones = X.ones ? (int)cdiv(X.ones_n, 1024) : 0;
+    pack_weights_kernel<<<PACK_BLOCKS + X.nzero + X.nones + (X.ktab ? 3 : 0), 256, 0, st>>>(gp, sp, mp, W.wcat, W.wcatT, W.bcat, W.wskip, W.bsum,
+                                                                                            W.wmixT, X);
     STEP_LAUNCH_CHECK("pack_weights");
     return STEP_OK;
 }
@@ -922,33 +1006,48 @@
 
     const long NN = (long)N * N;
     const bool dead_bn7 = (training & 2) != 0;
+    const bool unfused = step_chain_unfused();
+    const int N8 = n8(N);
     if (do_prep) {
-        STEP_TRY(zero((float*)W.acc64, 2L * NL * NCOPY * 64, st));
+        if (unfused) STEP_TRY(zero((float*)W.acc64, 2L * NL * NCOPY * 64, st));
         start_conv_kernel<<<g1(BN * 13 * C), 256, 0, st>>>(hist, B, N, Cin, p->start_w, p->start_b, S.x0);
         STEP_LAUNCH_CHECK("start_conv");
         {
             StepGemm g = gemm_desc(N, N, 10, p->nodevec1, 10, 1, p->nodevec2, N, 1, S.Madp, N);
             STEP_TRY(step_gemm_launch(g, st));
             softmax_relu_rows_kernel<<<N, 256, 0, st>>>(S.Madp, N, S.Pa);
-            replicate_adp_kernel<<<g1(NN), 256, 0, st>>>(S.Pa, N, B, S.Pstk + 2 * B * NN, S.PTstk + 2 * B * NN);
+            const bool rows16 = !unfused && p->gemm_bf16;
+            replicate_adp_kernel<<<g1(NN), 256, 0, st>>>(S.Pa, N, B, S.Pstk + 2 * B * NN, S.PTstk + 2 * B * NN, N8,
+                                                         rows16 ? S.P16 + 2L * B * N * N8 : nullptr, rows16 ? S.PT16 + 2L * B * N * N8 : nullptr);
             STEP_LAUNCH_CHECK("adp_softmax");
         }
-        STEP_TRY(pack_weights(p, W, st));
+        {
+            PackExtra X = {};
+            if (!unfused) { X.zero = (float*)W.acc64; X.zero_n = 2L * NL * NCOPY * 64; X.ones = S.cs; X.ones_n = BN; }
+            STEP_TRY(pack_weights(p, W, X, st));
+        }
         if (allbf16) STEP_TRY(gwnet_layers_forward<true>(p, S, W, B, N, train, use_drop ? dropout_p : 0.f, seed, momentum, dead_bn7, dyn, st, true, false));
         else STEP_TRY(gwnet_layers_forward<false>(p, S, W, B, N, train, use_drop ? dropout_p : 0.f, seed, momentum, dead_bn7, dyn, st, true, false));
     }
     if (do_layers) {
-        row_sums_kernel<<<(unsigned)BN, 256, 0, st>>>(adj, N, S.rs, S.cs);
         {
             int slices = cdiv(512, cdiv(N, 64) * B);
             if (slices > cdiv(N, 64)) slices = cdiv(N, 64);
             if (slices < 1) slices = 1;
-            col_sums_kernel<<<dim3(cdiv(N, 64), slices, B), 256, 0, st>>>(adj, N, S.cs);
-        }
+            if (unfused) {
+                row_sums_kernel<<<(unsigned)BN, 256, 0, st>>>(adj, N, S.rs, S.cs);
+                col_sums_kernel<<<dim3(cdiv(N, 64), slices, B), 256, 0, st>>>(adj, N, S.cs);
+            } else {
+                row_col_sums_kernel<<<(unsigned)(BN + (long)cdiv(N, 64) * slices * B), 256, 0, st>>>(adj, N, BN, cdiv(N, 64), slices, S.rs, S.cs);
+            }
+        }
+        const bool rows16 = !unfused && p->gemm_bf16;
+        const long s16 = (long)B * N * N8;
         rw_build_kernel<<<dim3(cdiv(N, 32), cdiv(N, 32), B), 256, 0, st>>>(adj, N, S.rs, S.cs, S.Pstk, S.Pstk + B * NN, S.PTstk,
-                                                                           S.PTstk + B * NN);
+                                                                           S.PTstk + B * NN, N8, rows16 ? S.P16 : nullptr, S.P16 + s16, S.PT16,
+                                                                           S.PT16 + s16);
         STEP_LAUNCH_CHECK("rw_build");
-        if (p->gemm_bf16) {
+        if (p->gemm_bf16 && unfused) {
             const long rows = 3L * B * N;
             stacks_to_bf16_kernel<<<dim3((unsigned)cdiv(rows * (n8(N) / 2), 256), 2), 256, 0, st>>>(S.Pstk, S.PTstk, rows, N, n8(N), S.P16,
                                                                                                    S.PT16);
@@ -985,11 +1084,11 @@
 
 template <bool BF16>
 static int gwnet_layers_backward(const StepGwnetParams* p, const StepGwnetParams* grads, const Saved& S, const Work& W, int B, int N,
-                                 float** dx0, hipStream_t st, AuxLane& lane, AuxLane& leaves, hipEvent_t* adj_done) {
+                                 float** dx0, hipStream_t st, AuxLane& lane, AuxLane& leaves, hipEvent_t* adj_done, bool ktab_ready) {
     const long BN = (long)B * N;
     float* dx_next = nullptr;
     float* dxbuf[2] = {W.dxa, W.dxb};
-    {
+    if (!ktab_ready) {
         AdjOffsets o;
         for (int i = 0; i < NL - 1; ++i) { o.cat[i] = S.cat[i] - S.cat[0]; o.dcat[i] = W.dcat[i] - W.dcat[0]; }
         adj_ktab_kernel<<<3, 128, 0, st>>>(o, N, W.ktab);
@@ -1068,18 +1167,30 @@
     const int allbf16 = p->gemm_bf16;
     auto split_for = [](long) { return -1; };
 
-    STEP_TRY(pack_weights(p, W, st));
-    STEP_TRY(zero(W.dwcat, (long)((float*)W.acc64 - W.dwcat) + 2L * NL * NCOPY * 64, st));
+    const bool unfused = step_chain_unfused();
+    {
+        PackExtra X = {};
+        const long nz = (long)((float*)W.acc64 - W.dwcat) + 2L * NL * NCOPY * 64;
+        if (!unfused) {
+            X.zero = W.dwcat; X.zero_n = nz;
+            for (int i = 0; i < NL - 1; ++i) { X.adj.cat[i] = S.cat[i] - S.cat[0]; X.adj.dcat[i] = W.dcat[i] - W.dcat[0]; }
+            X.N = N; X.ktab = W.ktab;
+        }
+        STEP_TRY(pack_weights(p, W, X, st));
+        if (unfused) STEP_TRY(zero(W.dwcat, nz, st));
+    }
     const long NN = (long)N * N;
 
     {
         StepGemm g = gemm_desc(N, CE, OUT, dpred, 1, N, p->end2_w, CE, 1, W.d_e1, CE);
         g.batch = B; g.sab = (long)OUT * N; g.scb = (long)N * CE;
+        if (!unfused) g.c_relu_mask = S.e1;
         STEP_TRY(step_gemm_launch(g, st));
-        relu_bwd_kernel<<<g1(BN * CE), 256, 0, st>>>(W.d_e1, S.e1, BN * CE);
+        if (unfused) relu_bwd_kernel<<<g1(BN * CE), 256, 0, st>>>(W.d_e1, S.e1, BN * CE);
         StepGemm gx = gemm_desc((int)BN, CS, CE, W.d_e1, CE, 1, p->end1_w, CS, 1, W.d_xh, CS);
+        if (!unfused) gx.c_relu_mask = S.xh;
         gx.compute_bf16 = allbf16; STEP_TRY(step_gemm_launch(gx, st));
-        relu_bwd_kernel<<<g1(BN * CS), 256, 0, st>>>(W.d_xh, S.xh, BN * CS);
+        if (unfused) relu_bwd_kernel<<<g1(BN * CS), 256, 0, st>>>(W.d_xh, S.xh, BN * CS);
         {
             hipStream_t leaf = leaves.fork();
             StepGemm gz = gemm_desc((int)BN, CS, CS, W.d_xh, CS, 1, W.wskip, CS, 1, W.dskip, CS);
@@ -1124,14 +1235,18 @@
 
     float* dx0 = nullptr;
     hipEvent_t adj_done = nullptr;
-    if (allbf16) STEP_TRY(gwnet_layers_backward<true>(p, grads, S, W, B, N, &dx0, st, lane, leaves, &adj_done));
-    else STEP_TRY(gwnet_layers_backward<false>(p, grads, S, W, B, N, &dx0, st, lane, leaves, &adj_done));
+    if (allbf16) STEP_TRY(gwnet_layers_backward<true>(p, grads, S, W, B, N, &dx0, st, lane, leaves, &adj_done, !unfused));
+    else STEP_TRY(gwnet_layers_backward<false>(p, grads, S, W, B, N, &dx0, st, lane, leaves, &adj_done, !unfused));
     STEP_TRY(lane.wait_done(adj_done));
     static const bool tail_leaves = []() { const char* e = getenv("STEP_TAIL_LEAVES"); return !(e && e[0] == '0'); }();
     if (!tail_leaves) STEP_TRY(leaves.join());
     hipStream_t leaf = tail_leaves ? leaves.fork() : st;
-    row_dot_kernel<<<(unsigned)BN, 256, 0, st>>>(W.dPstk, S.Pstk, N, W.rf);
-    row_dot_kernel<<<(unsigned)BN, 256, 0, st>>>(W.dPstk + B * NN, S.Pstk + B * NN, N, W.rb);
+    if (unfused) {
+        row_dot_kernel<<<(unsigned)BN, 256, 0, st>>>(W.dPstk, S.Pstk, N, W.rf);
+        row_dot_kernel<<<(unsigned)BN, 256, 0, st>>>(W.dPstk + B * NN, S.Pstk + B * NN, N, W.rb);
+    } else {
+        row_dot2_kernel<<<(unsigned)(2 * BN), 256, 0, st>>>(W.dPstk, S.Pstk, N, BN, W.rf, W.rb);
+    }
     rw_bwd_kernel<<<dim3(cdiv(N, 32), cdiv(N, 32), B), 256, 0, st>>>(W.dPstk, W.dPstk + B * NN, N, S.rs, S.cs, W.rf, W.rb, dadj);
     STEP_LAUNCH_CHECK("rw_bwd");
     {
diff --git a/step_amd/csrc/step_internal.h b/step_amd/csrc/step_internal.h
--- a/step_amd/csrc/step_internal.h
+++ b/step_amd/csrc/step_internal.h
@@ -1,5 +1,6 @@
 #pragma once
 #include <hip/hip_runtime.h>
+#include <cstdlib>
 #include <vector>
 #include "../../include/step_hip.h"
 
@@ -11,6 +12,11 @@
     int flags;
     const float* ffn_bias; const void* maskx; float p; unsigned seed_lo, seed_hi, site;
 };
+
+static inline bool step_chain_unfused() {
+    const char* e = getenv("STEP_CHAIN_UNFUSED");
+    return e && e[0] == '1';
+}
 
 struct GemmKSeg { long a_off, b_off, a_bs, b_bs; int a_rs, b_rs; };
 constexpr int GEMM_KSEG_MAX = 128;
@@ -45,11 +51,13 @@
 int dgl_conv1_fwd_cl(const float* x, const float* w, const float* b, void* a1h, float* partial, int N, int T, int stat_limit, int* nblk,
                      hipStream_t st);
 long dgl_conv2_pack_floats();
+struct DglBn1Finalize { const float* partial; int nblk; double count; const float *gamma, *beta; float *rmean, *rvar; int training; float momentum; float* stat; };
 int dgl_conv2_fwd_cl(const void* a1h, const float* w, const float* b, const float* sc, const float* sh, void* a2h, float* partial, int N,
-                     int T1, int* nblk, float* pack, hipStream_t st);
+                     int T1, int* nblk, float* pack, const DglBn1Finalize* bn1, hipStream_t st);
 int dgl_conv2_dgrad_cl(const void* dz2h, const float* w, const float* sc, void* dz1h, int N, int T1, const void* a1h, const float* coef,
-                       const float* stat, int own, float* pack, hipStream_t st);
-int dgl_conv2_wgrad_cl(const void* dz2h, const void* a1h, float* scratch, float* graw, int N, int T1, hipStream_t st);
+                       const float* stat, int own, float* pack, int build_pack, hipStream_t st);
+int dgl_conv2_wgrad_cl(const void* dz2h, const void* a1h, float* scratch, float* graw, int N, int T1, int clear_graw, hipStream_t st);
+long dgl_conv2_wgrad_out_floats();
 int dgl_conv1_wgrad_cl(const void* dz1h, const float* x, float* scratch, float* dw, float* db, int N, int T, hipStream_t st);
 long dgl_conv2_wgrad_scratch_floats(int N, int T1);
 int dgl_conv2_wgrad_mfma(const float* dz, const float* a1, const float* sc, const float* sh, float* scratch, float* dw, float* db, int N,
```

Result: no change. 2365 (-0.5%).
